# mmigas/LiverRenderer

Hardware: AMD Instinct MI355X
Metric: Msamples/s (higher is better)
Workload: dtype f32; 1 GPU; C3 Liver-SingleMesh volpath 1920x1080 512 spp max_depth 12 (homogeneous medium, isotropic phase, envmap); width=1920, height=1080, spp=512, parallelism=1 GPU

## Files before the change

### include/liverrt.h

```cpp
#ifndef LIVERRT_H
#define LIVERRT_H

#include <stdint.h>
#include <stddef.h>

#ifdef __cplusplus
extern "C" {
#endif

#define LRT_API __attribute__((visibility("default")))

typedef enum {
    LRT_OK = 0,
    LRT_ERR_INVALID = 1,
    LRT_ERR_IO = 2,
    LRT_ERR_DEVICE = 3,
    LRT_ERR_UNSUPPORTED = 4
} lrt_status;

enum { LRT_INTEGRATOR_PATH = 0, LRT_INTEGRATOR_VOLPATH = 1, LRT_INTEGRATOR_PRBVOLPATH = 2,
       LRT_INTEGRATOR_VOLPATHMIS = 5,
       LRT_INTEGRATOR_BIOVOLPATH = 3,
       LRT_INTEGRATOR_BIOVOLPATH06 = 4    };
enum { LRT_MEDIUM_HOMOGENEOUS = 0, LRT_MEDIUM_LIVER = 1, LRT_MEDIUM_PARENCHYMA = 2, LRT_MEDIUM_GLISSON = 3,
// ... 71 lines not shown
    int32_t type;
    float   radiance[3];
    int32_t shape;
    float   scale;
    float   to_world[16];
    int32_t width, height;
    const float *data;
} lrt_emitter_desc;

enum { LRT_SAMPLER_INDEPENDENT = 0, LRT_SAMPLER_LD = 1 };

typedef struct {
    float   to_world[16];
    float   fov_x;
    float   near_clip, far_clip;
    int32_t medium;
    float   principal_point_offset_x, principal_point_offset_y;
    int32_t pad;
} lrt_sensor_desc;

typedef struct {
    int32_t width, height;
    int32_t crop_offset_x, crop_offset_y, crop_width, crop_height;
    int32_t has_alpha;
    int32_t rfilter;
    float   rfilter_param;
} lrt_film_desc;

typedef struct {
    int32_t type;
    int32_t max_depth;
    int32_t rr_depth;
    int32_t hide_emitters;
} lrt_integrator_desc;

typedef struct {
    uint32_t n_vertices, n_faces, n_shapes, n_bsdfs, n_textures, n_media, n_emitters;
    const float    *positions;
    const float    *normals;
    const float    *texcoords;
    const uint32_t *faces;
    const uint32_t *face_shape;
    const lrt_shape_desc   *shapes;
    const lrt_bsdf_desc    *bsdfs;
    const lrt_texture_desc *textures;
    const lrt_medium_desc  *media;
    const lrt_emitter_desc *emitters;
    lrt_sensor_desc     sensor;
    lrt_film_desc       film;
    lrt_integrator_desc integrator;
    uint32_t sample_count;
    uint32_t sampler_seed;
    uint32_t sampler_type;
    uint32_t samples_per_pass;
    uint32_t use_spectral_mis;
    uint32_t pad;
} lrt_scene_desc;

typedef struct {
    int32_t  integrator;
    int32_t  max_depth;
    int32_t  rr_depth;
    int32_t  hide_emitters;
    uint32_t spp;
    uint32_t seed;
    uint32_t tile_rank, tile_count;
    int32_t  device;
    int32_t  output_on_device;
    int32_t  grad_medium;
    int32_t  pad;
} lrt_render_opts;

typedef struct {
    uint64_t n_samples;
    uint64_t n_iter;
    uint64_t n_shadow;
    uint64_t n_launches;
    uint64_t n_records;
    double   kernel_ms;
    double   total_ms;
    uint64_t lds_resident;
    uint64_t record_bytes;
    uint64_t n_closed_guard;
} lrt_render_stats;

typedef struct {
    float d_sigma_t[3];
    float d_albedo[3];
    float d_g;
} lrt_param_grads;

typedef struct lrt_scene lrt_scene;

LRT_API const char *lrt_last_error(void);
LRT_API int         lrt_version(void);

LRT_API lrt_status lrt_scene_load_xml(const char *path, const char *const *defines,
                                      int n_defines, lrt_scene **out);
LRT_API lrt_status lrt_scene_load_xml_string(const char *xml, const char *base_dir,
                                             const char *const *defines, int n_defines,
                                             lrt_scene **out);
LRT_API lrt_status lrt_scene_from_desc(const lrt_scene_desc *desc, lrt_scene **out);
LRT_API const lrt_scene_desc *lrt_scene_desc_get(const lrt_scene *scene);
LRT_API void       lrt_scene_free(lrt_scene *scene);

LRT_API lrt_status lrt_render(lrt_scene *scene, const lrt_render_opts *opts,
                              float *film_raw, float *image);
LRT_API lrt_status lrt_render_stats_get(const lrt_scene *scene, lrt_render_stats *out);
LRT_API lrt_status lrt_film_develop(lrt_scene *scene, const float *film_raw, float *image,
                                    int on_device);

LRT_API lrt_status lrt_render_samples(lrt_scene *scene, const lrt_render_opts *opts,
                                      uint64_t lane_begin, uint32_t n, float *out);

LRT_API lrt_status lrt_render_backward(lrt_scene *scene, const lrt_render_opts *opts,
                                       const float *grad_image, lrt_param_grads *out);

LRT_API lrt_status lrt_render_backward_grid(lrt_scene *scene, const lrt_render_opts *opts, const float *grad_image,
                                            lrt_param_grads *out, float *d_grid);

LRT_API lrt_status lrt_render_multi(lrt_scene *scene, const lrt_render_opts *opts, int n_devices, const int *device_ids,
                                    float *film_raw, float *image);
LRT_API lrt_status lrt_render_backward_multi(lrt_scene *scene, const lrt_render_opts *opts, int n_devices, const int *device_ids,
                                             const float *grad_image, lrt_param_grads *out);

LRT_API lrt_status lrt_math_eval(int fn, const float *x, const float *y, uint32_t n, float *out, float *out2, int device);

#define LRT_PROBE_FLOATS 20
LRT_API lrt_status lrt_emitter_probe(lrt_scene *scene, const float *ref_p, const float *sample, uint32_t n, float *out, int device);

LRT_API lrt_status lrt_envmap_probe(lrt_scene *scene, const float *dir, uint32_t n, float *out, int device);

#define LRT_BSDF_PROBE_FLOATS 30
LRT_API lrt_status lrt_bsdf_probe(lrt_scene *scene, const float *o, const float *d, const float *sample, const float *wo_query,
                                  uint32_t n, float *out, int device);

typedef struct { const float *ox, *oy, *oz, *dx, *dy, *dz, *tmax; } lrt_rays_soa;
typedef struct { float *t, *u, *v; uint32_t *prim; } lrt_hits_soa;
LRT_API lrt_status lrt_trace(lrt_scene *scene, const lrt_rays_soa *rays,
                             const lrt_hits_soa *hits, uint32_t n, int any_hit);

LRT_API lrt_status lrt_param_set(lrt_scene *scene, const char *key, const float *v, int n);
LRT_API lrt_status lrt_param_get(const lrt_scene *scene, const char *key, float *v, int n);

LRT_API lrt_status lrt_image_read(const char *path, int *width, int *height, int *channels, float **data);
LRT_API void       lrt_image_free(float *data);
LRT_API lrt_status lrt_image_write_exr(const char *path, int width, int height, int channels, const float *data);
LRT_API lrt_status lrt_image_write_png(const char *path, int width, int height, int channels, const float *data);

#define LRT_AOV_MAX_INTEGRATORS 4
#define LRT_AOV_MAX_AOVS        16
#define LRT_AOV_NAME_LEN        64
enum { LRT_AOV_ALBEDO = 0,
       LRT_AOV_DEPTH = 1,
       LRT_AOV_POSITION = 2,
       LRT_AOV_UV = 3,
       LRT_AOV_GEO_NORMAL = 4,
       LRT_AOV_SH_NORMAL = 5,
       LRT_AOV_DP_DU = 6,
       LRT_AOV_DP_DV = 7,
       LRT_AOV_PRIM_INDEX = 8,
       LRT_AOV_SHAPE_INDEX = 9    };

typedef struct {
    int32_t n_integrators;
    lrt_integrator_desc integrators[LRT_AOV_MAX_INTEGRATORS];
// ... 74 lines not shown
```

### liverrenderer_amd/_lib.py

```python
import ctypes as C
import os

_HERE = os.path.dirname(os.path.abspath(__file__))
LIB_PATH = os.environ.get("LRT_LIBRARY") or os.path.join(_HERE, "libliverrt.so")

OK, INVALID, UNSUPPORTED = 0, 1, 4
INTEGRATOR = {"path": 0, "volpath": 1, "prbvolpath": 2, "biovolpath": 3, "biovolpath06": 4, "volpathmis": 5}
MEDIUM = {"homogeneous": 0, "liver": 1, "parenchyma": 2, "glissonCapsule": 3, "heterogeneous": 4}
EMITTER = {"area": 0, "envmap": 1, "constant": 2}
PROBE_FLOATS = 20
BSDF_PROBE_FLOATS = 30


class ShapeDesc(C.Structure):
    _fields_ = [("kind", C.c_int32), ("first_face", C.c_uint32), ("n_faces", C.c_uint32), ("bsdf", C.c_int32),
                ("emitter", C.c_int32), ("interior_medium", C.c_int32), ("exterior_medium", C.c_int32),
                ("has_normals", C.c_int32), ("has_texcoords", C.c_int32), ("flip_normals", C.c_int32),
                ("to_world", C.c_float * 16)]


class TextureDesc(C.Structure):
    _fields_ = [("type", C.c_int32), ("color0", C.c_float * 3), ("color1", C.c_float * 3), ("to_uv", C.c_float * 9),
                ("width", C.c_int32), ("height", C.c_int32), ("channels", C.c_int32), ("data", C.POINTER(C.c_float))]


class BsdfDesc(C.Structure):
    _fields_ = [("type", C.c_int32), ("reflectance", C.c_int32), ("eta", C.c_float), ("nested", C.c_int32),
                ("texture", C.c_int32), ("scale", C.c_float),
                ("alpha_u", C.c_float), ("alpha_v", C.c_float), ("distribution", C.c_int32), ("sample_visible", C.c_int32),
                ("specular_reflectance", C.c_int32), ("specular_transmittance", C.c_int32)]


class MediumDesc(C.Structure):
    _fields_ = [("sigma_t", C.c_float * 3), ("albedo", C.c_float * 3), ("scale", C.c_float),
                ("has_spectral_extinction", C.c_int32), ("sample_emitters", C.c_int32), ("phase", C.c_int32),
                ("g", C.c_float), ("id", C.c_char * 64),
                ("type", C.c_int32), ("layer_limit", C.c_float * 4), ("sigma_collagen", (C.c_float * 3) * 4),
                ("sigma_elastin", (C.c_float * 3) * 4), ("sigma_blood", C.c_float * 3), ("sigma_bile", C.c_float * 3),
                ("sigma_lipid_water", C.c_float * 3), ("sigma_hepatocity", C.c_float),
                ("grid_res", C.c_int32 * 3), ("grid_to_local", C.c_float * 12), ("grid_bbox_min", C.c_float * 3),
                ("grid_bbox_max", C.c_float * 3), ("grid_max", C.c_float), ("grid_data", C.POINTER(C.c_float))]


class EmitterDesc(C.Structure):
    _fields_ = [("type", C.c_int32), ("radiance", C.c_float * 3), ("shape", C.c_int32), ("scale", C.c_float),
                ("to_world", C.c_float * 16), ("width", C.c_int32), ("height", C.c_int32), ("data", C.POINTER(C.c_float))]


class SensorDesc(C.Structure):
    _fields_ = [("to_world", C.c_float * 16), ("fov_x", C.c_float), ("near_clip", C.c_float), ("far_clip", C.c_float),
                ("medium", C.c_int32), ("principal_point_offset_x", C.c_float), ("principal_point_offset_y", C.c_float), ("pad", C.c_int32)]


class FilmDesc(C.Structure):
    _fields_ = [("width", C.c_int32), ("height", C.c_int32), ("crop_offset_x", C.c_int32), ("crop_offset_y", C.c_int32),
                ("crop_width", C.c_int32), ("crop_height", C.c_int32), ("has_alpha", C.c_int32), ("rfilter", C.c_int32),
                ("rfilter_param", C.c_float)]


class IntegratorDesc(C.Structure):
    _fields_ = [("type", C.c_int32), ("max_depth", C.c_int32), ("rr_depth", C.c_int32), ("hide_emitters", C.c_int32)]


class SceneDesc(C.Structure):
    _fields_ = [("n_vertices", C.c_uint32), ("n_faces", C.c_uint32), ("n_shapes", C.c_uint32), ("n_bsdfs", C.c_uint32),
                ("n_textures", C.c_uint32), ("n_media", C.c_uint32), ("n_emitters", C.c_uint32),
                ("positions", C.POINTER(C.c_float)), ("normals", C.POINTER(C.c_float)), ("texcoords", C.POINTER(C.c_float)),
                ("faces", C.POINTER(C.c_uint32)), ("face_shape", C.POINTER(C.c_uint32)),
                ("shapes", C.POINTER(ShapeDesc)), ("bsdfs", C.POINTER(BsdfDesc)), ("textures", C.POINTER(TextureDesc)),
                ("media", C.POINTER(MediumDesc)), ("emitters", C.POINTER(EmitterDesc)),
                ("sensor", SensorDesc), ("film", FilmDesc), ("integrator", IntegratorDesc),
                ("sample_count", C.c_uint32), ("sampler_seed", C.c_uint32),
                ("sampler_type", C.c_uint32), ("samples_per_pass", C.c_uint32), ("use_spectral_mis", C.c_uint32), ("pad", C.c_uint32)]


AOV_MAX_INTEGRATORS, AOV_MAX_AOVS, AOV_NAME_LEN = 4, 16, 64
AOV_TYPES = {"albedo": 0, "depth": 1, "position": 2, "uv": 3, "geo_normal": 4, "sh_normal": 5, "dp_du": 6, "dp_dv": 7,
             "prim_index": 8, "shape_index": 9}


class AovDesc(C.Structure):
    _fields_ = [("n_integrators", C.c_int32), ("integrators", IntegratorDesc * AOV_MAX_INTEGRATORS),
                ("integrator_names", (C.c_char * AOV_NAME_LEN) * AOV_MAX_INTEGRATORS),
                ("n_aovs", C.c_int32), ("aov_types", C.c_int32 * AOV_MAX_AOVS), ("aov_names", (C.c_char * AOV_NAME_LEN) * AOV_MAX_AOVS),
                ("n_aov_channels", C.c_int32), ("n_channels", C.c_int32)]


class MomentDesc(C.Structure):
    _fields_ = [("integrator", IntegratorDesc), ("name", C.c_char * AOV_NAME_LEN), ("n_channels", C.c_int32), ("n_raw_channels", C.c_int32)]


class RenderOpts(C.Structure):
    _fields_ = [("integrator", C.c_int32), ("max_depth", C.c_int32), ("rr_depth", C.c_int32), ("hide_emitters", C.c_int32),
                ("spp", C.c_uint32), ("seed", C.c_uint32), ("tile_rank", C.c_uint32), ("tile_count", C.c_uint32),
                ("device", C.c_int32), ("output_on_device", C.c_int32), ("grad_medium", C.c_int32), ("pad", C.c_int32)]


class RenderStats(C.Structure):
    _fields_ = [("n_samples", C.c_uint64), ("n_iter", C.c_uint64), ("n_shadow", C.c_uint64), ("n_launches", C.c_uint64),
                ("n_records", C.c_uint64), ("kernel_ms", C.c_double), ("total_ms", C.c_double), ("lds_resident", C.c_uint64),
                ("record_bytes", C.c_uint64), ("n_closed_guard", C.c_uint64)]


class ParamGrads(C.Structure):
    _fields_ = [("d_sigma_t", C.c_float * 3), ("d_albedo", C.c_float * 3), ("d_g", C.c_float)]


class DenoiseParams(C.Structure):
    _fields_ = [("iterations", C.c_int32), ("sigma_color", C.c_float), ("sigma_normal", C.c_float), ("sigma_albedo", C.c_float), ("eps_a", C.c_float)]


class RaysSoA(C.Structure):
    _fields_ = [(n, C.POINTER(C.c_float)) for n in ("ox", "oy", "oz", "dx", "dy", "dz", "tmax")]


class HitsSoA(C.Structure):
    _fields_ = [("t", C.POINTER(C.c_float)), ("u", C.POINTER(C.c_float)), ("v", C.POINTER(C.c_float)), ("prim", C.POINTER(C.c_uint32))]


def make_opts(integrator=None, max_depth=None, rr_depth=None, hide_emitters=None, spp=0, seed=0,
              tile_rank=0, tile_count=1, device=0, output_on_device=False, grad_medium=0):
    o = RenderOpts()
    o.integrator = -1 if integrator is None else (INTEGRATOR[integrator] if isinstance(integrator, str) else int(integrator))
    o.max_depth = -2 if max_depth is None else int(max_depth)
    o.rr_depth = -1 if rr_depth is None else int(rr_depth)
    o.hide_emitters = -1 if hide_emitters is None else int(bool(hide_emitters))
    o.spp, o.seed, o.tile_rank, o.tile_count = int(spp), int(seed) & 0xffffffff, int(tile_rank), int(tile_count)
    o.device, o.output_on_device = int(device), int(bool(output_on_device))
    o.grad_medium = int(grad_medium)
    return o


_lib = None


def _pytorch_context_first():
    import importlib.util
    import sys
    if os.environ.get("LRT_NO_TORCH_INIT"):
        return "skipped"
    if "torch" not in sys.modules and importlib.util.find_spec("torch") is None:
        return "no torch"
    import torch
    if not torch.cuda.is_available():
        return "no device"
    if not torch.cuda.is_initialized():
        lr = os.environ.get("LOCAL_RANK")
        if lr is not None and lr.isdigit() and torch.cuda.device_count() > 0:
            torch.cuda.set_device(int(lr) % torch.cuda.device_count())
        torch.zeros(1, device="cuda")
    if not torch.cuda.is_initialized():
        raise RuntimeError("PyTorch is importable but its HIP context could not be created before libliverrt.so was loaded; "
                           "set LRT_NO_TORCH_INIT=1 if this process does not use PyTorch")
    return "initialised"


def lib():
    global _lib
    if _lib is not None:
        return _lib
    _pytorch_context_first()
    if not os.path.exists(LIB_PATH):
        raise RuntimeError(f"{LIB_PATH} is missing: build it with `python -c 'import __graft_entry__ as g; g.build()'` "
                           "(the hip_ad_rgb back-end has no CPU fallback)")
    L = C.CDLL(LIB_PATH)
    P = C.POINTER
    L.lrt_last_error.restype = C.c_char_p
    L.lrt_version.restype = C.c_int
    L.lrt_scene_load_xml.argtypes = [C.c_char_p, P(C.c_char_p), C.c_int, P(C.c_void_p)]
    L.lrt_scene_load_xml_string.argtypes = [C.c_char_p, C.c_char_p, P(C.c_char_p), C.c_int, P(C.c_void_p)]
    L.lrt_scene_from_desc.argtypes = [P(SceneDesc), P(C.c_void_p)]
    L.lrt_scene_desc_get.argtypes = [C.c_void_p]
    L.lrt_scene_desc_get.restype = P(SceneDesc)
    L.lrt_scene_free.argtypes = [C.c_void_p]
    L.lrt_scene_free.restype = None
    L.lrt_render.argtypes = [C.c_void_p, P(RenderOpts), C.c_void_p, C.c_void_p]
    L.lrt_render_multi.argtypes = [C.c_void_p, P(RenderOpts), C.c_int, P(C.c_int), C.c_void_p, C.c_void_p]
    L.lrt_render_backward_multi.argtypes = [C.c_void_p, P(RenderOpts), C.c_int, P(C.c_int), C.c_void_p, P(ParamGrads)]
    L.lrt_math_eval.argtypes = [C.c_int, P(C.c_float), P(C.c_float), C.c_uint32, P(C.c_float), P(C.c_float), C.c_int]
    L.lrt_render_stats_get.argtypes = [C.c_void_p, P(RenderStats)]
    L.lrt_film_develop.argtypes = [C.c_void_p, C.c_void_p, C.c_void_p, C.c_int]
    L.lrt_render_samples.argtypes = [C.c_void_p, P(RenderOpts), C.c_uint64, C.c_uint32, C.c_void_p]
    L.lrt_render_backward.argtypes = [C.c_void_p, P(RenderOpts), C.c_void_p, P(ParamGrads)]
    L.lrt_render_backward_grid.argtypes = [C.c_void_p, P(RenderOpts), C.c_void_p, P(ParamGrads), C.c_void_p]
# ... 63 lines not shown
```

### liverrenderer_amd/csrc/capi.cpp

```cpp
#include "host_scene.h"
#include "device_scene.h"
#include "image_io.h"
#include <algorithm>
#include <cmath>
#include <cstring>
#include <cstdio>
#include <fstream>
#include <sstream>
#include <stdexcept>

using namespace lrt;

static thread_local std::string g_error;
static lrt_status fail(lrt_status st, const std::string &msg) { g_error = msg; return st; }

#define LRT_TRY try {
#define LRT_CATCH } catch (const std::exception &e) { \
        std::string m = e.what(); \
        lrt_status st = LRT_ERR_INVALID; \
        if (m.find("hip") != std::string::npos || m.find("HIP") != std::string::npos) st = LRT_ERR_DEVICE; \
        if (m.find("cannot open") != std::string::npos || m.find("file not found") != std::string::npos) st = LRT_ERR_IO; \
        if (m.find("unsupported") != std::string::npos || m.find("not supported") != std::string::npos) st = LRT_ERR_UNSUPPORTED; \
        return fail(st, m); \
    } catch (...) { return fail(LRT_ERR_INVALID, "unknown error"); }

extern "C" {

const char *lrt_last_error(void) { return g_error.c_str(); }
int lrt_version(void) { return 114; }

static std::vector<std::pair<std::string, std::string>> parse_defines(const char *const *defines, int n) {
    std::vector<std::pair<std::string, std::string>> r;
    for (int i = 0; i < n; ++i) {
        std::string s = defines[i]; size_t eq = s.find('=');
        if (eq == std::string::npos) throw std::runtime_error("define \"" + s + "\" must have the form key=value");
        r.emplace_back(s.substr(0, eq), s.substr(eq + 1));
    }
    return r;
}

lrt_status lrt_scene_load_xml_string(const char *xml, const char *base_dir, const char *const *defines, int n_defines, lrt_scene **out) {
    if (!xml || !out) return fail(LRT_ERR_INVALID, "lrt_scene_load_xml_string: null argument");
    *out = nullptr;
    LRT_TRY
        std::unique_ptr<lrt_scene> s(new lrt_scene());
        load_scene_xml(xml, base_dir ? base_dir : "", parse_defines(defines, n_defines), s->st);
        *out = s.release();
        return LRT_OK;
    LRT_CATCH
}

lrt_status lrt_scene_load_xml(const char *path, const char *const *defines, int n_defines, lrt_scene **out) {
    if (!path || !out) return fail(LRT_ERR_INVALID, "lrt_scene_load_xml: null argument");
    *out = nullptr;
    std::ifstream f(path, std::ios::binary);
    if (!f) return fail(LRT_ERR_IO, std::string("cannot open \"") + path + "\"");
    std::stringstream ss; ss << f.rdbuf();
    std::string p = path, dir; size_t sl = p.rfind('/'); dir = sl == std::string::npos ? "." : p.substr(0, sl);
    return lrt_scene_load_xml_string(ss.str().c_str(), dir.c_str(), defines, n_defines, out);
}

static void validate_desc(const lrt_scene_desc &d) {
    auto bad = [](const std::string &m) { throw std::runtime_error("lrt_scene_from_desc: " + m); };
    if ((d.n_vertices && (!d.positions || !d.normals || !d.texcoords)) || (d.n_faces && (!d.faces || !d.face_shape))) bad("null geometry array");
    if ((d.n_shapes && !d.shapes) || (d.n_bsdfs && !d.bsdfs) || (d.n_textures && !d.textures) || (d.n_media && !d.media) || (d.n_emitters && !d.emitters)) bad("null object array");
    for (uint32_t f = 0; f < 3 * d.n_faces; ++f) if (d.faces[f] >= d.n_vertices) bad("face references an invalid vertex");
    for (uint32_t f = 0; f < d.n_faces; ++f) if (d.face_shape[f] >= d.n_shapes) bad("face references an invalid shape");
    for (uint32_t i = 0; i < d.n_textures; ++i) {
        const lrt_texture_desc &T = d.textures[i];
        if (T.type < LRT_TEX_RGB || T.type > LRT_TEX_BITMAP) bad("invalid texture type");
        if (T.type == LRT_TEX_BITMAP && (!T.data || T.width < 1 || T.height < 1 || (T.channels != 1 && T.channels != 3))) bad("bitmap texture without texels or with invalid dimensions");
    }
    for (uint32_t i = 0; i < d.n_bsdfs; ++i) {
        const lrt_bsdf_desc &B = d.bsdfs[i];
        if (B.type < LRT_BSDF_DIFFUSE || B.type > LRT_BSDF_ROUGHDIELECTRIC) bad("invalid bsdf type");
        if (B.type == LRT_BSDF_DIFFUSE) {
            if (B.reflectance < 0 || (uint32_t) B.reflectance >= d.n_textures) bad("diffuse bsdf references an invalid texture");
            if (d.textures[B.reflectance].type == LRT_TEX_BITMAP) throw std::runtime_error("unsupported: a bitmap texture as diffuse reflectance (bitmaps are supported as bump-map heights only)");
        }
        if (B.type == LRT_BSDF_BUMPMAP) {
            if (B.nested < 0 || (uint32_t) B.nested >= d.n_bsdfs || d.bsdfs[B.nested].type == LRT_BSDF_BUMPMAP) bad("bumpmap references an invalid nested bsdf");
            if (B.texture < 0 || (uint32_t) B.texture >= d.n_textures) bad("bumpmap references an invalid texture");
        }
        if (B.type == LRT_BSDF_DIELECTRIC && !(B.eta > 0.f)) bad("dielectric with a non-positive relative index of refraction");
        if (B.type == LRT_BSDF_ROUGHDIELECTRIC) {
            if (!(B.eta > 0.f) || B.eta == 1.f) bad("roughdielectric: the interior and exterior indices of refraction must be positive and differ");
            if (!(B.alpha_u >= 0.f) || !(B.alpha_v >= 0.f) || !std::isfinite(B.alpha_u) || !std::isfinite(B.alpha_v)) bad("roughdielectric with an invalid roughness");
            if (B.distribution != 0 && B.distribution != 1) bad("roughdielectric with an invalid distribution (0: beckmann, 1: ggx)");
            for (int32_t t : { B.specular_reflectance, B.specular_transmittance }) {
                if (t < -1 || t >= (int32_t) d.n_textures) bad("roughdielectric references an invalid texture");
                if (t >= 0 && d.textures[t].type == LRT_TEX_BITMAP) throw std::runtime_error("unsupported: a bitmap texture as roughdielectric specular_reflectance / specular_transmittance");
            }
        }
    }
    for (uint32_t i = 0; i < d.n_media; ++i) {
        const lrt_medium_desc &M = d.media[i];
        if (M.type < LRT_MEDIUM_HOMOGENEOUS || M.type > LRT_MEDIUM_HETEROGENEOUS) bad("invalid medium type");
        if (M.type == LRT_MEDIUM_HETEROGENEOUS && (!M.grid_data || M.grid_res[0] < 1 || M.grid_res[1] < 1 || M.grid_res[2] < 1)) bad("heterogeneous medium without grid data");
        if (M.phase != LRT_PHASE_ISOTROPIC && M.phase != LRT_PHASE_HG) bad("invalid phase function");
        if (M.phase == LRT_PHASE_HG && !(M.g > -1.f && M.g < 1.f)) bad("The asymmetry parameter must lie in the interval (-1, 1)!");
    }
    for (uint32_t i = 0; i < d.n_shapes; ++i) {
        const lrt_shape_desc &s = d.shapes[i];
        if (s.bsdf < 0 || (uint32_t) s.bsdf >= d.n_bsdfs) bad("shape references an invalid bsdf");
        if (s.emitter < -1 || s.emitter >= (int) d.n_emitters || s.interior_medium < -1 || s.interior_medium >= (int) d.n_media || s.exterior_medium < -1 || s.exterior_medium >= (int) d.n_media)
            bad("shape references an invalid emitter/medium");
        if ((uint64_t) s.first_face + s.n_faces > d.n_faces) bad("shape face range exceeds the face array");
        if (s.kind < LRT_SHAPE_MESH || s.kind > LRT_SHAPE_SPHERE) bad("invalid shape kind");
        if (s.kind == LRT_SHAPE_SPHERE && s.n_faces != 0) bad("a sphere shape has no faces");
        if (s.emitter >= 0 && (d.emitters[s.emitter].type != LRT_EMITTER_AREA || d.emitters[s.emitter].shape != (int) i)) bad("shape and area emitter do not reference each other");
    }
    uint32_t n_env = 0;
// ... 488 lines not shown
```

### liverrenderer_amd/csrc/device.hip

```cpp
#include "host_scene.h"
#include "device_scene.h"
#include "kernels_prb.h"
#include "kernels_vae.h"
#include "kernels_aov.h"
#include "kernels_denoise.h"
#include "kernels_moment.h"
#include <functional>
#include "scene_prep.h"
#include <cmath>
#include <array>
#include <cstring>
#include <algorithm>
#include <stdexcept>
#include <string>
#include <cstdio>
#include <cstdlib>
#include <thread>
#include <chrono>
#include <exception>
#include <dlfcn.h>
#include <rccl/rccl.h>

namespace lrt {

#define HIP_CHECK(expr) do { hipError_t e_ = (expr); if (e_ != hipSuccess) throw std::runtime_error(std::string(#expr) + ": " + hipGetErrorString(e_)); } while (0)

template <typename T> static T *dev_upload(const T *src, size_t n, hipStream_t st) {
    T *p = nullptr; size_t bytes = std::max<size_t>(n, 1) * sizeof(T);
    HIP_CHECK(hipMalloc((void **) &p, bytes));
    if (n) HIP_CHECK(hipMemcpyAsync(p, src, n * sizeof(T), hipMemcpyHostToDevice, st));
    return p;
}

struct DevTmp {
    float *p = nullptr;
    DevTmp() = default;
    explicit DevTmp(size_t floats) { alloc(floats); }
    DevTmp(const DevTmp &) = delete; DevTmp &operator=(const DevTmp &) = delete;
    void alloc(size_t floats) { HIP_CHECK(hipMalloc((void **) &p, std::max<size_t>(floats, 1) * sizeof(float))); }
    void upload(const float *src, size_t floats, hipStream_t st) { alloc(floats); HIP_CHECK(hipMemcpyAsync(p, src, floats * sizeof(float), hipMemcpyHostToDevice, st)); }
    ~DevTmp() { if (p) (void) hipFree(p); }
};

static void select_device(int device) {
    int count = 0;
    if (hipGetDeviceCount(&count) != hipSuccess || count == 0) throw std::runtime_error("no HIP device available: the hip_ad_rgb back-end has no CPU fallback");
    if (device < 0 || device >= count) throw std::runtime_error("invalid HIP device ordinal " + std::to_string(device));
    HIP_CHECK(hipSetDevice(device));
}

static lrt_render_opts default_opts() { return lrt_render_opts{ -1, -2, -1, -1, 0, 0, 0, 1, 0, 0, 0, 0 }; }

static void add_stats(lrt_render_stats &total, const lrt_render_stats &s) {
    total.n_samples += s.n_samples; total.n_iter += s.n_iter; total.n_shadow += s.n_shadow; total.n_launches += s.n_launches;
    total.n_records += s.n_records; total.kernel_ms += s.kernel_ms; total.total_ms += s.total_ms;
    total.record_bytes = s.record_bytes; total.n_closed_guard += s.n_closed_guard;
}

#define LRT_LAUNCH_SLOTS 64
#define LRT_WIDE_BLOCK 768

struct DeviceScene {
    int device = 0;
    hipStream_t stream = nullptr;
    DScene sc{};
    DScene *d_sc = nullptr;
    DLaunch *d_launch = nullptr, *h_launch = nullptr; uint32_t launch_next = 0;
    std::vector<void *> allocs;
    uint32_t capacity = 0;
    DPathStreams q[2]{};
    float4 *dl[2] = { nullptr, nullptr }; size_t dl_records[2] = { 0, 0 }; float4 *L_buf = nullptr; size_t l_buf_lanes = 0;
    double *d_grads = nullptr; float *wfilm = nullptr; size_t wfilm_floats = 0; float *grad_image = nullptr; size_t grad_floats = 0;
    DCounters *counters = nullptr;
    DCounters *h_counters = nullptr;
    float *film = nullptr; size_t film_floats = 0;
    float *image = nullptr; size_t image_floats = 0;
    unsigned long long *pass_state[2] = { nullptr, nullptr }; size_t pass_state_lanes[2] = { 0, 0 };
    const unsigned long long *cur_pass_in = nullptr; unsigned long long *cur_pass_out = nullptr;
    uint32_t *pixel_slot = nullptr;
    uint32_t *pixel_list = nullptr; uint32_t pixel_list_rank = 0xffffffffu, pixel_list_count = 0, n_owned_pixels = 0;
    uint32_t *halo_list = nullptr; uint32_t halo_rank = 0xffffffffu, halo_count = 0, halo_width = 0, n_halo_pixels = 0;
    std::vector<hipEvent_t> ev_pool;
    std::vector<DMedium> h_media; DMedium *d_media = nullptr;
    std::vector<DBioMedium> h_bio; DBioMedium *d_bio = nullptr;
    std::vector<DHetMedium> h_het; DHetMedium *d_het = nullptr; std::vector<float *> het_data; bool has_het = false, has_non_bio = false, need_mis = false; uint32_t ws_layouts = 0;
    bool ext = false;
    bool has_area_emitter = false;
    float *dgrid = nullptr; size_t dgrid_floats = 0;
    bool prb_null = false;
    DLdsInfo lds{}; bool use_lds = false; int n_cus = 256; int bvh_leaf = 4;
    DAovSpec *d_aov_spec = nullptr; uint32_t *d_first_face = nullptr;
    float *aov_film = nullptr; size_t aov_film_floats = 0; float *aov_image = nullptr; size_t aov_image_floats = 0; float *aov_inner = nullptr; size_t aov_inner_floats = 0;

    template <typename T> T *track(T *p) { allocs.push_back((void *) p); return p; }
    void release(void *p) {
        if (!p) return;
        for (auto it = allocs.begin(); it != allocs.end(); ++it) if (*it == p) { allocs.erase(it); break; }
        (void) hipFree(p);
    }
    template <typename T> T *grow(T *&p, size_t &have, size_t want) {
        if (have >= want) return p;
        HIP_CHECK(hipStreamSynchronize(stream));
        release(p); p = nullptr; have = 0;
        HIP_CHECK(hipMalloc((void **) &p, std::max<size_t>(want, 1) * sizeof(T))); track(p);
        have = want;
        return p;
    }
    ~DeviceScene() {
        for (void *p : allocs) (void) hipFree(p);
        for (auto e : ev_pool) (void) hipEventDestroy(e);
        if (h_counters) (void) hipHostFree(h_counters);
        if (h_launch) (void) hipHostFree(h_launch);
        if (stream) (void) hipStreamDestroy(stream);
    }
};

void device_scene_destroy(DeviceScene *d) { delete d; }

static_assert(PREP_F_DELTA == F_DELTA && PREP_F_SMOOTH == F_SMOOTH && PREP_F_NULL == F_NULL, "scene_prep.h restates the BSDF leaf flags of dshade.h");

__global__ void k_bio_prepare(DBioMedium *bio, uint32_t n) {
    const uint32_t i = blockIdx.x * blockDim.x + threadIdx.x;
    if (i < n) bio[i].log10_hep = m_log2(bio[i].hepatocity + 1.f) / m_log2(10.f);
}

__global__ void k_medium_prepare(DMedium *media, uint32_t n) {
    const uint32_t i = blockIdx.x * blockDim.x + threadIdx.x;
    if (i >= n) return;
    DMedium &M = media[i];
    const V3 st(M.sigma_t[0], M.sigma_t[1], M.sigma_t[2]), ss = st * V3(M.albedo[0], M.albedo[1], M.albedo[2]);
    const V3 ws = ss / mean3(st / st), wp = ss / st;
    M.w_spec[0] = ws.x; M.w_spec[1] = ws.y; M.w_spec[2] = ws.z; M.w_plain[0] = wp.x; M.w_plain[1] = wp.y; M.w_plain[2] = wp.z;
}

static void upload_media(DeviceScene *D, const lrt_scene_desc &d) {
    prepare_media(d, D->sc.env.bsphere_r, D->h_media, D->h_bio, D->h_het);
    for (size_t i = 0; i < D->h_het.size(); ++i) D->h_het[i].data = D->het_data[i];
    HIP_CHECK(hipMemcpyAsync(D->d_bio, D->h_bio.data(), D->h_bio.size() * sizeof(DBioMedium), hipMemcpyHostToDevice, D->stream));
    k_bio_prepare<<<1, 64, 0, D->stream>>>(D->d_bio, (uint32_t) std::min<size_t>(D->h_bio.size(), 64));
// ... 59 lines not shown
typedef void (*AovFn)(ScenePtr, LaunchPtr, AovSpecPtr);
static AovFn aov_kernel(bool lds, bool ld, bool ext) {
    static const AovFn t[2][2][2] = { { { k_aov<false, false, false>, k_aov<false, false, true> }, { k_aov<false, true, false>, k_aov<false, true, true> } },
                                      { { k_aov<true, false, false>, k_aov<true, false, true> }, { k_aov<true, true, false>, k_aov<true, true, true> } } };
    return t[lds][ld][ext];
}
typedef decltype(&k_trace<false, false>) TraceFn;
typedef decltype(&k_trace_lds<false, false>) TraceLdsFn;
static TraceFn trace_kernel(bool any_hit, bool ext) {
    static const TraceFn t[2][2] = { { k_trace<false, false>, k_trace<false, true> }, { k_trace<true, false>, k_trace<true, true> } };
    return t[any_hit][ext];
}
static TraceLdsFn trace_lds_kernel(bool any_hit, bool ext) {
    static const TraceLdsFn t[2][2] = { { k_trace_lds<false, false>, k_trace_lds<false, true> }, { k_trace_lds<true, false>, k_trace_lds<true, true> } };
    return t[any_hit][ext];
}
static RenderFn moment_splat_kernel(bool wide, bool alpha) {
    static const RenderFn t[2][2] = { { k_moment_splat<false, false>, k_moment_splat<false, true> }, { k_moment_splat<true, false>, k_moment_splat<true, true> } };
    return t[wide][alpha];
}

DeviceScene *device_scene_create(const lrt_scene_desc &d, int device) {
    select_device(device);
    std::unique_ptr<DeviceScene> D(new DeviceScene());
    D->device = device;
    HIP_CHECK(hipStreamCreateWithFlags(&D->stream, hipStreamNonBlocking));
    hipStream_t st = D->stream;
    PrepOptions opt = PrepOptions::from_env();
    hipDeviceProp_t prop; HIP_CHECK(hipGetDeviceProperties(&prop, device)); opt.n_cus = prop.multiProcessorCount > 0 ? prop.multiProcessorCount : 256;
    int optin = 0; if (hipDeviceGetAttribute(&optin, hipDeviceAttributeSharedMemPerBlockOptin, device) != hipSuccess || optin <= 0) optin = (int) prop.sharedMemPerBlock;
    (void) hipGetLastError();
    opt.lds_limit = std::min<size_t>((size_t) std::max(optin, 0), 160 * 1024) - 512;
    PreparedScene P; DScene &sc = P.sc;
    prepare_geometry(d, opt, P);
    D->n_cus = opt.n_cus; D->bvh_leaf = P.bvh_leaf; D->ext = P.ext;
    auto up = [&](const auto &v) { return D->track(dev_upload(v.data(), v.size(), st)); };
    sc.spheres = P.spheres.empty() ? nullptr : up(P.spheres);
    sc.nodes = (const float4 *) up(P.bvh.nodes);
    sc.tris = (const float4 *) up(P.bvh.tris);
    if (P.use_lds) {
        D->lds = P.lds; D->lds.blob = (const uint4 *) up(P.lds_blob);
        const size_t lds_limit = opt.lds_limit;
        auto raise_lds = [&](const void *k) { if (k) HIP_CHECK(hipFuncSetAttribute(k, hipFuncAttributeMaxDynamicSharedMemorySize, (int) lds_limit)); };
        const KernelTable &K = kernels();
        for (const RenderRow &r : K.render) if (r.lds && (!r.ext || D->ext)) raise_lds((const void *) r.fn);
        for (const auto &adjoint : K.prb) for (const auto &ld : adjoint[1]) for (RenderFn fn : ld) raise_lds((const void *) fn);
        for (RenderFn fn : K.prb_grid[1]) raise_lds((const void *) fn);
        for (int i = 0; i < 2; ++i) for (int ext = 0; ext <= (D->ext ? 1 : 0); ++ext) {
            raise_lds((const void *) aov_kernel(true, i, ext)); raise_lds((const void *) trace_lds_kernel(i, ext));
        }
        D->use_lds = true;
    }
    if (sc.grid.enabled) {
        const size_t n_cells = (size_t) sc.grid.n[0] * sc.grid.n[1] * sc.grid.n[2];
        uint16_t *buf = nullptr; HIP_CHECK(hipMalloc((void **) &buf, n_cells * sizeof(uint16_t))); D->track(buf);
        k_build_dist_grid<<<(uint32_t) ((n_cells + LRT_BLOCK - 1) / LRT_BLOCK), LRT_BLOCK, 0, st>>>(sc.tris, d.n_faces ? (uint32_t) (P.bvh.tris.size() / 12) : 0u, sc.grid, buf, P.grid_abs_margin,
                                                                                             sc.spheres, sc.n_spheres);
        HIP_CHECK(hipGetLastError());
        sc.grid.d = buf;
    }
    prepare_shading(d, opt, P);
    D->has_area_emitter = P.has_area_emitter; D->has_het = P.has_het; D->has_non_bio = P.has_non_bio; D->prb_null = P.prb_null;
    sc.positions = D->track(dev_upload(d.positions, 3 * (size_t) d.n_vertices, st));
    sc.vattr = (const float4 *) up(P.vattr);
    sc.faces = D->track(dev_upload(d.faces, 3 * (size_t) d.n_faces, st));
    sc.face_shape = D->track(dev_upload(d.face_shape, d.n_faces, st));
    sc.shapes = up(P.shapes);
    sc.textures = up(P.textures);
    sc.tex_data = up(P.tex_data);
    sc.bsdfs = up(P.bsdfs);
    HIP_CHECK(hipMalloc((void **) &D->d_media, std::max<uint32_t>(d.n_media, 1) * sizeof(DMedium))); D->track(D->d_media);
    HIP_CHECK(hipMalloc((void **) &D->d_bio, std::max<uint32_t>(d.n_media, 1) * sizeof(DBioMedium))); D->track(D->d_bio);
    HIP_CHECK(hipMalloc((void **) &D->d_het, std::max<uint32_t>(d.n_media, 1) * sizeof(DHetMedium))); D->track(D->d_het);
    D->het_data.assign(std::max<uint32_t>(d.n_media, 1), nullptr);
    for (uint32_t i = 0; i < d.n_media; ++i) {
        const lrt_medium_desc &M = d.media[i];
        if (M.type == LRT_MEDIUM_HETEROGENEOUS) D->het_data[i] = D->track(dev_upload(M.grid_data, (size_t) M.grid_res[0] * M.grid_res[1] * M.grid_res[2], st));
    }
    D->sc = sc;
    upload_media(D.get(), d); sc.media = D->d_media; sc.bio = D->d_bio; sc.het = D->d_het;
    sc.emitters = up(P.emitters);
    sc.mesh_emitters = up(P.mesh_emitters);
    sc.mesh_emitter_tab = up(P.mesh_emitter_tab);
    sc.env_data = (const float4 *) up(P.env_data);
    sc.env_hier = up(P.env_hier);
    HIP_CHECK(hipMalloc((void **) &D->d_sc, sizeof(DScene))); D->track(D->d_sc);
    D->sc = sc;
    HIP_CHECK(hipMemcpyAsync(D->d_sc, &D->sc, sizeof(DScene), hipMemcpyHostToDevice, st));
    HIP_CHECK(hipMalloc((void **) &D->d_launch, LRT_LAUNCH_SLOTS * sizeof(DLaunch))); D->track(D->d_launch);
    HIP_CHECK(hipHostMalloc((void **) &D->h_launch, LRT_LAUNCH_SLOTS * sizeof(DLaunch)));
    HIP_CHECK(hipMalloc((void **) &D->counters, sizeof(DCounters))); D->track(D->counters);
    HIP_CHECK(hipHostMalloc((void **) &D->h_counters, sizeof(DCounters)));
    HIP_CHECK(hipStreamSynchronize(st));
    return D.release();
}

void device_scene_update_params(DeviceScene *D, const lrt_scene_desc &d, bool grids) {
    HIP_CHECK(hipSetDevice(D->device));
    if (grids) for (uint32_t i = 0; i < d.n_media; ++i) {
        const lrt_medium_desc &M = d.media[i];
        if (M.type == LRT_MEDIUM_HETEROGENEOUS && D->het_data[i])
            HIP_CHECK(hipMemcpyAsync(D->het_data[i], M.grid_data, (size_t) M.grid_res[0] * M.grid_res[1] * M.grid_res[2] * sizeof(float), hipMemcpyHostToDevice, D->stream));
    }
    upload_media(D, d);
    HIP_CHECK(hipStreamSynchronize(D->stream));
}

static void ensure_workspace(DeviceScene *D, uint32_t capacity) {
    const uint32_t layouts = workspace_layouts(D->has_het, D->need_mis);
    if (D->capacity >= capacity && D->ws_layouts == layouts) return;
    HIP_CHECK(hipStreamSynchronize(D->stream));
    D->capacity = 0;
    auto get = [](const DPathStreams *q, const RecordStream &r) { void *p; memcpy(&p, (const char *) q + r.member, sizeof p); return p; };
    auto set = [](DPathStreams *q, const RecordStream &r, void *p) { memcpy((char *) q + r.member, &p, sizeof p); };
    for (DPathStreams *q : { &D->q[0], &D->q[1] })
        for (const RecordStream &r : kRecordStreams) if (r.member != kNoMember) { D->release(get(q, r)); set(q, r, nullptr); }
    for (DPathStreams *q : { &D->q[0], &D->q[1] })
        for (size_t k = 0; k < std::size(kRecordStreams); ++k) if (const uint32_t bytes = workspace_stream_bytes(k, layouts)) {
            void *p = nullptr; HIP_CHECK(hipMalloc(&p, (size_t) capacity * bytes)); D->track(p); set(q, kRecordStreams[k], p);
        }
    D->capacity = capacity; D->ws_layouts = layouts;
}

static hipEvent_t get_event(DeviceScene *D, size_t i) {
    while (D->ev_pool.size() <= i) { hipEvent_t e; HIP_CHECK(hipEventCreate(&e)); D->ev_pool.push_back(e); }
    return D->ev_pool[i];
}

static void ensure_pixel_list(DeviceScene *D, const ResolvedOpts &O) {
    const DFilm &F = D->sc.film;
    if (O.tile_count == 1) { D->n_owned_pixels = (uint32_t) F.width * F.height; return; }
    if (D->pixel_list && D->pixel_list_rank == O.tile_rank && D->pixel_list_count == O.tile_count) return;
    const TilePixels T = tile_pixel_list(F, O.tile_rank, O.tile_count);
    D->release(D->pixel_list); D->release(D->pixel_slot); D->pixel_list = nullptr; D->pixel_slot = nullptr;
    D->pixel_list = D->track(dev_upload(T.list.data(), T.list.size(), D->stream));
    D->pixel_slot = D->track(dev_upload(T.slot.data(), T.slot.size(), D->stream));
    D->pixel_list_rank = O.tile_rank; D->pixel_list_count = O.tile_count; D->n_owned_pixels = (uint32_t) T.list.size();
}

static void ensure_halo_list(DeviceScene *D, const ResolvedOpts &O, uint32_t halo) {
    const DFilm &F = D->sc.film;
    if (D->halo_list && D->halo_rank == O.tile_rank && D->halo_count == O.tile_count && D->halo_width == halo) return;
    const std::vector<uint32_t> px = halo_pixel_list(F, O.tile_rank, O.tile_count, halo);
    D->release(D->halo_list); D->halo_list = nullptr;
    D->halo_list = D->track(dev_upload(px.data(), px.size(), D->stream));
    D->halo_rank = O.tile_rank; D->halo_count = O.tile_count; D->halo_width = halo; D->n_halo_pixels = (uint32_t) px.size();
}

static void ensure_prb_workspace(DeviceScene *D, uint32_t records, uint64_t l_buf_lanes) {
    for (int k = 0; k < 2; ++k) D->grow(D->dl[k], D->dl_records[k], records);
    D->grow(D->L_buf, D->l_buf_lanes, l_buf_lanes);
    if (!D->d_grads) { HIP_CHECK(hipMalloc((void **) &D->d_grads, 7 * sizeof(double))); D->track(D->d_grads); }
}

static DRenderParams make_params(const lrt_scene_desc &d, const ResolvedOpts &O, uint64_t n_lanes) {
    DRenderParams rp{};
    rp.integrator = O.integrator; rp.max_depth = O.max_depth; rp.rr_depth = O.rr_depth; rp.hide_emitters = O.hide_emitters;
    rp.spp = O.spp; rp.log2_spp = ((O.spp & (O.spp - 1)) == 0) ? (uint32_t) __builtin_ctz(O.spp) : 0xffffffffu;
    rp.profile = getenv("LRT_DEBUG_LAUNCH") ? 1u : 0u;
#ifdef LRT_EXPERIMENT
    if (getenv("LRT_EXP")) rp.profile |= (uint32_t) atoi(getenv("LRT_EXP"));
    if (getenv("LRT_PRB_DEBUG_LANE")) rp.pad1 = (uint32_t) atoi(getenv("LRT_PRB_DEBUG_LANE")) + 1u;
#endif
    rp.seed_value = d.sampler_seed + O.seed; rp.base_seed = d.sampler_seed; rp.seed = O.seed;
    rp.ld_count = d.sampler_type == LRT_SAMPLER_LD ? O.spp_total : 0u; rp.pass_index = O.pass; rp.spp_total = O.spp_total; rp.tile_rank = O.tile_rank; rp.tile_count = O.tile_count; rp.n_lanes = n_lanes;
    return rp;
// ... 49 lines not shown
    HIP_CHECK(hipMemcpyAsync(&D->d_launch[slot], &D->h_launch[slot], sizeof(DLaunch), hipMemcpyHostToDevice, D->stream));
    return (LaunchPtr) &D->d_launch[slot];
}

template <bool ADJOINT>
static void launch_prb(DeviceScene *D, const DRenderParams &rp, const PoolGeometry &g, const uint32_t *pixel_list, uint64_t lane_begin,
                       float4 *L_buf, const float *grad_image, double *grads, float *film, float *sample_out, float *dgrid = nullptr) {
    hipStream_t st = D->stream;
    HIP_CHECK(hipMemsetAsync(&D->counters->next_lane, 0, sizeof(unsigned long long), st));
    DLaunch a{}; a.rp = rp; a.li = D->lds; a.q0 = D->q[0]; a.q1 = D->q[1]; a.dl0 = D->dl[0]; a.dl1 = D->dl[1]; a.P = g.P; a.cnt = D->counters;
    a.pixel_list = pixel_list; a.lane_begin = lane_begin; a.n = rp.n_lanes; a.L_buf = L_buf; a.grad_image = grad_image; a.wfilm = D->wfilm; a.grads = grads;
    a.film = film; a.sample_out = sample_out; a.sample_base = lane_begin; a.dgrid = dgrid;
    const LaunchPtr lp = push_launch(D, a);
    const bool ld = rp.ld_count != 0;
    const RenderFn fn = (ADJOINT && dgrid) ? kernels().prb_grid[D->use_lds][ld] : kernels().prb[ADJOINT][D->use_lds][ld][D->prb_null];
    if (!fn) throw std::runtime_error("developer build: volpath only");
    fn<<<g.n_wg, D->use_lds ? 1024 : LRT_BLOCK, g.smem, st>>>((ScenePtr) D->d_sc, lp);
    HIP_CHECK(hipGetLastError());
}

static void check_integrator_media(DeviceScene *D, int integrator) {
    if ((integrator == LRT_INTEGRATOR_BIOVOLPATH || integrator == LRT_INTEGRATOR_BIOVOLPATH06) && D->has_non_bio)
        throw std::runtime_error("NotImplementedError: sample_interaction (the bio integrators need liver / parenchyma / glissonCapsule media)");
    if (integrator == LRT_INTEGRATOR_PRBVOLPATH && D->ext)
        throw std::runtime_error("unsupported: prbvolpath on a scene with sphere shapes, point emitters, area emitters on meshes or a roughdielectric BSDF (its adjoint is built for triangles, rectangle / infinite emitters and the diffuse / dielectric / null BSDFs)");
    if (integrator == LRT_INTEGRATOR_VOLPATHMIS) D->need_mis = true;
}

static const RenderRow &select_render_kernel(int integrator, bool has_het, bool spectral_mis, bool lds, bool ld, bool ext, bool compact, bool closed) {
    int mode;
    switch (integrator) {
        case LRT_INTEGRATOR_PATH: case LRT_INTEGRATOR_BIOVOLPATH: case LRT_INTEGRATOR_BIOVOLPATH06: mode = integrator; break;
        case LRT_INTEGRATOR_VOLPATHMIS: mode = spectral_mis ? LRT_INTEGRATOR_VOLPATHMIS : LRT_INTEGRATOR_VOLPATHMIS_PLAIN; break;
        default: mode = closed ? LRT_INTEGRATOR_VOLPATH_CLOSED : (has_het ? LRT_INTEGRATOR_VOLPATH_HET : LRT_INTEGRATOR_VOLPATH);
    }
    for (const RenderRow &r : kernels().render) if (r.mode == mode && r.lds == lds && r.ld == ld && r.compact == compact && r.ext == ext) return r;
    throw std::runtime_error("no render-kernel instance for mode " + std::to_string(mode) + (lds ? ", LDS BVH" : ", global BVH") + (ld ? ", ld sampler" : ", independent sampler") +
                             (compact ? ", compact records" : ", wide records") + (ext ? ", EXT" : ""));
}

static void run_wavefront(DeviceScene *D, const lrt_scene_desc &d, const ResolvedOpts &O, uint64_t lane_begin, uint64_t n_lanes,
                          const uint32_t *pixel_list, float *film, float *sample_out, lrt_render_stats &stats) {
    hipStream_t st = D->stream;
    DRenderParams rp = make_params(d, O, n_lanes);
    rp.pixel_slot = pixel_list ? D->pixel_slot : nullptr;
    rp.pass_in = D->cur_pass_in; rp.pass_out = D->cur_pass_out;
    const bool prb = O.integrator == LRT_INTEGRATOR_PRBVOLPATH;
    check_integrator_media(D, O.integrator);
    PoolGeometry g = pool_geometry(D, n_lanes);
    const uint32_t records = (uint32_t) std::min<uint64_t>((uint64_t) g.n_wg * 2u * g.P, 0xffffffffull);
    ensure_workspace(D, records);
    if (prb) ensure_prb_workspace(D, records, 0);
    HIP_CHECK(hipMemsetAsync(D->counters, 0, sizeof(DCounters), st));
    LaunchLog log;
    hipEvent_t e_begin = get_event(D, log.ev++), e_end = get_event(D, log.ev++);
    HIP_CHECK(hipEventRecord(e_begin, st));
    const bool count_iter = !(O.integrator == LRT_INTEGRATOR_PATH && O.max_depth == 0);
    hipEvent_t a = get_event(D, log.ev++), b = get_event(D, log.ev++);
    HIP_CHECK(hipEventRecord(a, st));
    if (prb) { stats.record_bytes = 0; launch_prb<false>(D, rp, g, pixel_list, lane_begin, nullptr, nullptr, nullptr, film, sample_out); }
    else {
        DLaunch a{}; a.rp = rp; a.li = D->lds; a.q0 = D->q[0]; a.q1 = D->q[1]; a.P = g.P; a.cnt = D->counters; a.pixel_list = pixel_list;
        a.lane_begin = lane_begin; a.n = n_lanes; a.film = film; a.sample_out = sample_out; a.sample_base = lane_begin;
        const bool compact = D->use_lds && !D->has_area_emitter && !D->ext && !getenv("LRT_WIDE_RECORDS") && O.integrator != LRT_INTEGRATOR_VOLPATHMIS && !(O.integrator == LRT_INTEGRATOR_VOLPATH && D->has_het);
        const bool closed = compact && O.integrator == LRT_INTEGRATOR_VOLPATH && closed_records(d, D->sc.cam.medium) && !getenv("LRT_NO_CLOSED_RECORDS");
#ifdef LRT_DEV_VOLPATH_ONLY
        if (D->ext) throw std::runtime_error("developer build: no EXT instances (spheres / point emitters)");
        if (!(D->use_lds && (O.integrator == LRT_DEV_INTEGRATOR || (LRT_DEV_INTEGRATOR == LRT_INTEGRATOR_VOLPATH_HET && D->has_het)) && (rp.ld_count != 0) == LRT_DEV_LD)) throw std::runtime_error("developer build: one integrator / sampler / LDS BVH only");
#endif
        const RenderRow &row = select_render_kernel(O.integrator, D->has_het, d.use_spectral_mis != 0, D->use_lds, rp.ld_count != 0, D->ext, compact, closed);
        stats.record_bytes = row.record_bytes;
        const LaunchPtr lp = push_launch(D, a);
        row.fn<<<g.n_wg, row.block, g.smem, st>>>((ScenePtr) D->d_sc, lp);
        HIP_CHECK(hipGetLastError());
    }
    HIP_CHECK(hipEventRecord(b, st));
    log.launches.emplace_back(a, b); log.sizes.push_back(0);
    HIP_CHECK(hipMemcpyAsync(D->h_counters, D->counters, sizeof(DCounters), hipMemcpyDeviceToHost, st));
    HIP_CHECK(hipStreamSynchronize(st));
    log.n_iter = count_iter ? D->h_counters->n_iter : 0;
    log.n_records = D->h_counters->n_records;
    finish_stats(D, log, e_begin, e_end, n_lanes, stats);
    stats.n_closed_guard = D->h_counters->n_closed_guard;
    if (stats.n_closed_guard)
        throw std::runtime_error("64-byte path records: " + std::to_string(stats.n_closed_guard) + " trips broke the premise of the layout (radiance before a path's last trip, "
                                 "or an emitter hit that needs its MIS weight); the scene test in closed_records() is wrong for this scene: LRT_NO_CLOSED_RECORDS=1 renders it with 80-byte records");
}

static void render_passes(DeviceScene *D, const lrt_scene_desc &d, const lrt_render_opts *opts, float *film_raw, float *image, lrt_render_stats &stats,
                          const std::function<void(const ResolvedOpts &)> &after_pass, bool moment = false);

void device_render(DeviceScene *D, const lrt_scene_desc &d, const lrt_render_opts *opts, float *film_raw, float *image, lrt_render_stats &stats) {
    render_passes(D, d, opts, film_raw, image, stats, nullptr);
}

static void develop_and_download(DeviceScene *D, const float *film, float *film_raw, float *image, size_t film_floats, size_t image_floats, bool on_device, bool moment = false) {
    const DFilm &F = D->sc.film; const size_t np = (size_t) F.width * F.height;
    if (image) {
        float *img = on_device ? image : D->grow(D->image, D->image_floats, image_floats);
        if (!moment) k_develop<<<(uint32_t) ((np + 255) / 256), 256, 0, D->stream>>>(F, film, img, (uint32_t) np);
        else if (F.has_alpha) k_moment_develop<true><<<(uint32_t) ((np + 255) / 256), 256, 0, D->stream>>>(film, img, (uint32_t) np);
        else k_moment_develop<false><<<(uint32_t) ((np + 255) / 256), 256, 0, D->stream>>>(film, img, (uint32_t) np);
        if (!on_device) HIP_CHECK(hipMemcpyAsync(image, img, image_floats * 4, hipMemcpyDeviceToHost, D->stream));
    }
    if (film_raw && !on_device) HIP_CHECK(hipMemcpyAsync(film_raw, film, film_floats * 4, hipMemcpyDeviceToHost, D->stream));
    HIP_CHECK(hipStreamSynchronize(D->stream));
    HIP_CHECK(hipGetLastError());
}

static void render_passes(DeviceScene *D, const lrt_scene_desc &d, const lrt_render_opts *opts, float *film_raw, float *image, lrt_render_stats &stats,
                          const std::function<void(const ResolvedOpts &)> &after_pass, bool moment) {
    HIP_CHECK(hipSetDevice(D->device));
    ResolvedOpts O = resolve(d, opts);
    const DFilm &F = D->sc.film;
    bool on_device = opts && opts->output_on_device;
    const size_t film_channels = moment ? (F.has_alpha ? 11 : 10) : (size_t) F.channels, image_channels = moment ? film_channels - 1 : (F.has_alpha ? 4 : 3);
    size_t np = (size_t) F.width * F.height, film_floats = np * film_channels, image_floats = np * image_channels;
    ensure_pixel_list(D, O);
    const uint64_t n_lanes = (uint64_t) D->n_owned_pixels * O.spp;
    float *film = (on_device && film_raw) ? film_raw : D->grow(D->film, D->film_floats, film_floats);
    HIP_CHECK(hipMemsetAsync(film, 0, film_floats * 4, D->stream));
    const uint32_t *pixel_list = O.tile_count > 1 ? D->pixel_list : nullptr;
    const bool carry = O.n_passes > 1 && d.sampler_type != LRT_SAMPLER_LD;
    if (carry) for (int k = 0; k < 2; ++k) D->grow(D->pass_state[k], D->pass_state_lanes[k], n_lanes);
    const bool lane_splat = moment || (F.rfilter != LRT_RFILTER_BOX && (O.n_passes > 1 || !getenv("LRT_NO_LANE_SPLAT")));
    lrt_render_stats total{};
    for (uint32_t pass = 0; pass < O.n_passes; ++pass) {
        O.pass = pass;
        D->cur_pass_in = carry ? D->pass_state[pass & 1] : nullptr;
        D->cur_pass_out = (carry && pass + 1 < O.n_passes) ? D->pass_state[(pass & 1) ^ 1] : nullptr;
        if (!lane_splat) {
            lrt_render_stats st1{};
            run_wavefront(D, d, O, 0, n_lanes, pixel_list, film, nullptr, st1);
            add_stats(total, st1);
            if (after_pass) after_pass(O);
            continue;
        }
        const uint64_t chunk = std::min<uint64_t>(std::max<uint64_t>(n_lanes, 1), 1ull << 28);
        ensure_prb_workspace(D, 0, chunk);
        for (uint64_t base = 0; base < n_lanes; base += chunk) {
            const uint64_t n = std::min<uint64_t>(chunk, n_lanes - base);
            lrt_render_stats st1{};
            run_wavefront(D, d, O, base, n, pixel_list, nullptr, reinterpret_cast<float *>(D->L_buf), st1);
            DRenderParams rp = make_params(d, O, n); rp.pass_in = D->cur_pass_in;
            DLaunch a{}; a.rp = rp; a.L_buf = D->L_buf; a.pixel_list = pixel_list; a.lane_begin = base; a.n = n; a.film = film;
            const uint32_t grid = (uint32_t) ((n + LRT_BLOCK - 1) / LRT_BLOCK);
            const LaunchPtr lp = push_launch(D, a);
            if (!moment) k_splat_lanes<false><<<grid, LRT_BLOCK, 0, D->stream>>>((ScenePtr) D->d_sc, lp);
            else moment_splat_kernel(F.rfilter != LRT_RFILTER_BOX, F.has_alpha != 0)<<<grid, LRT_BLOCK, 0, D->stream>>>((ScenePtr) D->d_sc, lp);
            HIP_CHECK(hipGetLastError());
            add_stats(total, st1);
        }
        if (after_pass) after_pass(O);
    }
    D->cur_pass_in = nullptr; D->cur_pass_out = nullptr;
    total.lds_resident = D->use_lds ? 1 : 0;
    stats = total;
    develop_and_download(D, film, film_raw, image, film_floats, image_floats, on_device, moment);
}

void device_render_moment(DeviceScene *D, const lrt_scene_desc &d, const lrt_render_opts *opts, float *film_raw, float *image, lrt_render_stats &stats) {
    render_passes(D, d, opts, film_raw, image, stats, nullptr, true);
}

void device_render_moment_samples(DeviceScene *D, const lrt_scene_desc &d, const lrt_render_opts *opts, uint64_t lane_begin, uint32_t n, float *out, lrt_render_stats &stats) {
    HIP_CHECK(hipSetDevice(D->device));
// ... 295 lines not shown
        for (const char *name : { env ? env : "/opt/rocm/lib/librccl.so", "librccl.so.1", "librccl.so" }) { h = dlopen(name, RTLD_NOW | RTLD_LOCAL); if (h) break; }
        if (!h) throw std::runtime_error(std::string("hip: cannot load librccl.so (") + (dlerror() ? dlerror() : "?") + "); lrt_render_multi on distinct devices needs RCCL");
        auto sym = [&](const char *n) { void *p = dlsym(h, n); if (!p) throw std::runtime_error(std::string("hip: librccl.so lacks ") + n); return p; };
        CommInitAll = (decltype(CommInitAll)) sym("ncclCommInitAll"); AllReduce = (decltype(AllReduce)) sym("ncclAllReduce");
        GroupStart = (decltype(GroupStart)) sym("ncclGroupStart"); GroupEnd = (decltype(GroupEnd)) sym("ncclGroupEnd");
        CommDestroy = (decltype(CommDestroy)) sym("ncclCommDestroy"); GetErrorString = (decltype(GetErrorString)) sym("ncclGetErrorString");
    }
    void check(ncclResult_t r, const char *what) { if (r != ncclSuccess) throw std::runtime_error(std::string("hip: rccl ") + what + ": " + (GetErrorString ? GetErrorString(r) : "error")); }
};
static Rccl g_rccl;

struct MultiContext {
    std::vector<int> devices; std::vector<ncclComm_t> comms;
    ~MultiContext() { for (auto c : comms) if (c && g_rccl.CommDestroy) (void) g_rccl.CommDestroy(c); }
};
void multi_context_destroy(MultiContext *m) { delete m; }

__global__ void k_film_add(float *__restrict__ dst, const float *__restrict__ src, size_t n) {
    const size_t i = (size_t) blockIdx.x * blockDim.x + threadIdx.x;
    if (i < n) dst[i] += src[i];
}

template <typename T>
static void reduce_across(std::vector<DeviceScene *> &devs, MultiContext *&ctx, std::vector<T *> &buf, size_t count) {
    const int N = (int) devs.size();
    bool distinct = true;
    for (int i = 0; i < N; ++i) for (int j = 0; j < i; ++j) if (devs[i]->device == devs[j]->device) distinct = false;
    for (auto *D : devs) { HIP_CHECK(hipSetDevice(D->device)); HIP_CHECK(hipStreamSynchronize(D->stream)); }
    if (distinct) {
        g_rccl.load();
        std::vector<int> ids; for (auto *D : devs) ids.push_back(D->device);
        if (!ctx || ctx->devices != ids) {
            delete ctx; ctx = new MultiContext(); ctx->devices = ids; ctx->comms.assign(N, nullptr);
            g_rccl.check(g_rccl.CommInitAll(ctx->comms.data(), N, ids.data()), "ncclCommInitAll");
        }
        g_rccl.check(g_rccl.GroupStart(), "ncclGroupStart");
        for (int i = 0; i < N; ++i) {
            HIP_CHECK(hipSetDevice(devs[i]->device));
            g_rccl.check(g_rccl.AllReduce(buf[i], buf[i], count, sizeof(T) == 8 ? ncclDouble : ncclFloat, ncclSum, ctx->comms[i], devs[i]->stream), "ncclAllReduce");
        }
        g_rccl.check(g_rccl.GroupEnd(), "ncclGroupEnd");
        for (auto *D : devs) { HIP_CHECK(hipSetDevice(D->device)); HIP_CHECK(hipStreamSynchronize(D->stream)); }
    } else {
        for (int i = 1; i < N; ++i) if (devs[i]->device != devs[0]->device) throw std::runtime_error("lrt_render_multi: a device list is either all distinct or one device repeated");
        static_assert(sizeof(T) == 4 || sizeof(T) == 8, "float or double");
        HIP_CHECK(hipSetDevice(devs[0]->device));
        for (int i = 1; i < N; ++i) {
            if (sizeof(T) == 4) k_film_add<<<(uint32_t) ((count + 255) / 256), 256, 0, devs[0]->stream>>>((float *) buf[0], (const float *) buf[i], count);
            else { std::vector<double> a(count), b(count); HIP_CHECK(hipMemcpy(a.data(), buf[0], count * 8, hipMemcpyDeviceToHost)); HIP_CHECK(hipMemcpy(b.data(), buf[i], count * 8, hipMemcpyDeviceToHost));
                   for (size_t k = 0; k < count; ++k) a[k] += b[k]; HIP_CHECK(hipMemcpy(buf[0], a.data(), count * 8, hipMemcpyHostToDevice)); }
        }
        HIP_CHECK(hipGetLastError()); HIP_CHECK(hipStreamSynchronize(devs[0]->stream));
    }
}

template <typename F> static void on_every_device(size_t n, F fn) {
    std::vector<std::exception_ptr> err(n);
    std::vector<std::thread> th;
    for (size_t i = 0; i < n; ++i) th.emplace_back([&, i]() { try { fn(i); } catch (...) { err[i] = std::current_exception(); } });
    for (auto &t : th) t.join();
    for (auto &e : err) if (e) std::rethrow_exception(e);
}

void device_render_multi(std::vector<DeviceScene *> &devs, MultiContext *&ctx, const lrt_scene_desc &d, const lrt_render_opts *opts, float *film_raw, float *image, lrt_render_stats &stats) {
    const int N = (int) devs.size();
    const DFilm &F = devs[0]->sc.film;
    const size_t np = (size_t) F.width * F.height, film_floats = np * F.channels, image_floats = np * (F.has_alpha ? 4 : 3);
    const bool on_device = opts && opts->output_on_device;
    std::vector<float *> films(N); std::vector<lrt_render_stats> st(N);
    const auto t0 = std::chrono::steady_clock::now();
    on_every_device(N, [&](size_t i) {
        HIP_CHECK(hipSetDevice(devs[i]->device));
        films[i] = (i == 0 && on_device && film_raw) ? film_raw : devs[i]->grow(devs[i]->film, devs[i]->film_floats, film_floats);
        lrt_render_opts o = opts ? *opts : default_opts();
        o.tile_rank = (uint32_t) i; o.tile_count = (uint32_t) N; o.device = devs[i]->device; o.output_on_device = 1;
        device_render(devs[i], d, &o, films[i], nullptr, st[i]);
    });
    if (N > 1 || getenv("LRT_MULTI_ALWAYS_REDUCE")) reduce_across(devs, ctx, films, film_floats);
    DeviceScene *D0 = devs[0];
    HIP_CHECK(hipSetDevice(D0->device));
    develop_and_download(D0, films[0], film_raw, image, film_floats, image_floats, on_device);
    lrt_render_stats total{};
    for (auto &x : st) { total.n_samples += x.n_samples; total.n_iter += x.n_iter; total.n_shadow += x.n_shadow; total.n_launches += x.n_launches; total.n_records += x.n_records;
                         total.kernel_ms = std::max(total.kernel_ms, x.kernel_ms); total.lds_resident = x.lds_resident; total.record_bytes = x.record_bytes; total.n_closed_guard += x.n_closed_guard; }
    total.total_ms = std::chrono::duration<double, std::milli>(std::chrono::steady_clock::now() - t0).count();
    stats = total;
}

void device_render_backward_multi(std::vector<DeviceScene *> &devs, MultiContext *&ctx, const lrt_scene_desc &d, const lrt_render_opts *opts, const float *grad_image, lrt_param_grads *out, lrt_render_stats &stats) {
    const int N = (int) devs.size();
    if (opts && opts->output_on_device) throw std::runtime_error("lrt_render_backward_multi: grad_image is a host buffer (every device takes its own copy)");
    std::vector<lrt_param_grads> g(N); std::vector<lrt_render_stats> st(N);
    on_every_device(N, [&](size_t i) {
        lrt_render_opts o = opts ? *opts : default_opts();
        o.tile_rank = (uint32_t) i; o.tile_count = (uint32_t) N; o.device = devs[i]->device; o.output_on_device = 0;
        device_render_backward(devs[i], d, &o, grad_image, &g[i], st[i]);
    });
    std::vector<double *> bufs; for (auto *D : devs) bufs.push_back(D->d_grads);
    if (N > 1) reduce_across(devs, ctx, bufs, 7);
    double h[7]; HIP_CHECK(hipSetDevice(devs[0]->device)); HIP_CHECK(hipMemcpy(h, devs[0]->d_grads, sizeof(h), hipMemcpyDeviceToHost));
    for (int k = 0; k < 3; ++k) { out->d_sigma_t[k] = (float) h[k]; out->d_albedo[k] = (float) h[3 + k]; }
    out->d_g = (float) h[6];
    lrt_render_stats total{};
    for (auto &x : st) { total.n_samples += x.n_samples; total.n_iter += x.n_iter; total.n_shadow += x.n_shadow; total.n_launches += x.n_launches; total.n_records += x.n_records;
                         total.kernel_ms = std::max(total.kernel_ms, x.kernel_ms); total.total_ms = std::max(total.total_ms, x.total_ms); total.lds_resident = x.lds_resident; }
    stats = total;
}

void device_emitter_probe(DeviceScene *D, const float *ref_p, const float *sample, uint32_t n, float *out) {
    HIP_CHECK(hipSetDevice(D->device));
    if (!n) return;
    hipStream_t st = D->stream;
    DevTmp dr, ds, dout((size_t) n * LRT_PROBE_FLOATS);
    dr.upload(ref_p, (size_t) n * 3, st); ds.upload(sample, (size_t) n * 2, st);
    k_emitter_probe<<<(n + LRT_BLOCK - 1) / LRT_BLOCK, LRT_BLOCK, 0, st>>>((ScenePtr) D->d_sc, dr.p, ds.p, n, dout.p);
    HIP_CHECK(hipGetLastError());
    HIP_CHECK(hipMemcpyAsync(out, dout.p, (size_t) n * LRT_PROBE_FLOATS * 4, hipMemcpyDeviceToHost, st));
    HIP_CHECK(hipStreamSynchronize(st));
}

void device_envmap_probe(DeviceScene *D, const float *dir, uint32_t n, float *out) {
    HIP_CHECK(hipSetDevice(D->device));
    if (D->sc.env.emitter < 0) throw std::runtime_error("lrt_envmap_probe: the scene has no environment emitter");
    if (!n) return;
    hipStream_t st = D->stream;
    DevTmp dd, dout((size_t) n * 4);
    dd.upload(dir, (size_t) n * 3, st);
    k_envmap_probe<<<(n + LRT_BLOCK - 1) / LRT_BLOCK, LRT_BLOCK, 0, st>>>((ScenePtr) D->d_sc, dd.p, n, dout.p);
    HIP_CHECK(hipGetLastError());
    HIP_CHECK(hipMemcpyAsync(out, dout.p, (size_t) n * 4 * 4, hipMemcpyDeviceToHost, st));
    HIP_CHECK(hipStreamSynchronize(st));
}

void device_bsdf_probe(DeviceScene *D, const float *o, const float *d, const float *sample, const float *wo_query, uint32_t n, float *out) {
    HIP_CHECK(hipSetDevice(D->device));
    if (!n) return;
    hipStream_t st = D->stream;
    DevTmp in[4], dout((size_t) n * LRT_BSDF_PROBE_FLOATS);
    const float *src[4] = { o, d, sample, wo_query };
    for (int k = 0; k < 4; ++k) in[k].upload(src[k], (size_t) n * 3, st);
    k_bsdf_probe<<<(n + LRT_BLOCK - 1) / LRT_BLOCK, LRT_BLOCK, 0, st>>>((ScenePtr) D->d_sc, in[0].p, in[1].p, in[2].p, in[3].p, n, dout.p);
    HIP_CHECK(hipGetLastError());
    HIP_CHECK(hipMemcpyAsync(out, dout.p, (size_t) n * LRT_BSDF_PROBE_FLOATS * 4, hipMemcpyDeviceToHost, st));
    HIP_CHECK(hipStreamSynchronize(st));
}

__global__ void k_math_eval(int fn, const float *__restrict__ x, const float *__restrict__ y, uint32_t n, float *__restrict__ out, float *__restrict__ out2) {
    const uint32_t i = blockIdx.x * blockDim.x + threadIdx.x;
    if (i >= n) return;
    float a = 0.f, b = 0.f;
    switch (fn) {
        case 0: a = m_log(x[i]); break;
        case 1: a = m_exp(x[i]); break;
        case 2: m_sincos(x[i], &a, &b); break;
        case 3: a = m_atan2(y[i], x[i]); break;
        case 4: a = m_acos(x[i]); break;
        case 5: a = m_log2(x[i]); break;
        case 6: a = x[i] / y[i]; break;
        case 7: a = __builtin_sqrtf(x[i]); break;
        case 8: a = rcp(x[i]); break;
        case 9: a = m_erf(x[i]); break;
        case 10: a = m_erfinv(x[i]); break;
        default: break;
    }
    out[i] = a; out2[i] = b;
}
void device_math_eval(int fn, const float *x, const float *y, uint32_t n, float *out, float *out2, int device) {
// ... 85 lines not shown
```

### liverrenderer_amd/csrc/device_types.h

```cpp
#pragma once
#include <stdint.h>
#include <hip/hip_vector_types.h>

namespace lrt {

struct DShape {
    int32_t bsdf, emitter, interior_medium, exterior_medium;
    int32_t has_normals, has_texcoords, flip_normals, kind;
};

#define LRT_MICRO_GGX 1
#define LRT_MICRO_VISIBLE 2
struct DBsdf {
    int32_t type;
    union { int32_t reflectance; int32_t specular_reflectance; };
    union { int32_t nested; int32_t micro; };
    union { int32_t texture; int32_t specular_transmittance; };
    float eta;
    union { float scale; float alpha_u; };
    int32_t flags;
    union { int32_t pad; float alpha_v; };
};
static_assert(sizeof(DBsdf) == 32, "DBsdf stride");

// ... 36 lines not shown
    int32_t type, shape; float radiance[3]; float scale;
    float n[3]; float inv_area;
    float to_world[12];
};

struct DSphere {
    float center[3], radius;
    float to_world[9];
    float to_object[12];
    uint32_t shape; int32_t flip_normals;
    float pad[2];
};

struct DMeshEmitter {
    uint32_t first_face, n_faces, pmf_offset, cdf_offset;
    float sum, normalization;
    int32_t has_normals, flip_normals;
    int32_t mesh, pad[3];
};

#define LRT_MAX_HIER_LEVELS 16

struct DCamera {
    float s2c[16];
    float to_world[12];
    float near_clip, far_clip;
    int32_t medium, pad;
    float ppo_x, ppo_y;
};

struct DFilm {
    int32_t width, height;
    int32_t crop_offset_x, crop_offset_y;
    float scale_x, scale_y, offset_x, offset_y;
    int32_t channels, has_alpha, rfilter, fcount;
    float rf_radius, rf_inv_radius; int32_t fn, pad;
    float rf_coeff[10];
    int32_t pad2[2];
};

struct DEnv {
    int32_t type;
    int32_t emitter;
    uint32_t w, h;
    float scale;
    float bsphere_c[3]; float bsphere_r;
    float to_world[9];
    float to_local[9];
    float patch_size[2], inv_patch_size[2];
    uint32_t max_patch[2];
    int32_t n_levels;
    uint32_t level_offset[LRT_MAX_HIER_LEVELS];
    uint32_t level_width[LRT_MAX_HIER_LEVELS];
    float radiance[3];
};

struct DDistGrid {
    const uint16_t *d;
    float lo[3]; float cell, inv_cell;
    int32_t n[3]; int32_t enabled;
};

struct DScene {
    const float4 *nodes;
    const float4 *tris;
    const float *positions;
    const float4 *vattr;
    const uint32_t *faces, *face_shape;
    const DShape *shapes; const DBsdf *bsdfs; const DTexture *textures; const DMedium *media; const DBioMedium *bio; const DHetMedium *het; const DEmitter *emitters;
    const float *tex_data;
    const float4 *env_data;
    const float *env_hier;
    uint32_t n_faces, n_emitters;
    int32_t root_is_leaf, has_null_bsdf;
    int32_t nee_fast_reject;
    int32_t one_shape;
    uint32_t root_leaf_first, root_leaf_count;
    DCamera cam; DFilm film; DEnv env;
    DDistGrid grid;
    const DSphere *spheres;
    uint32_t n_spheres, pad_sph;
    const DMeshEmitter *mesh_emitters;
    const float *mesh_emitter_tab;
};

#define LRT_CONST __attribute__((address_space(4)))
typedef const LRT_CONST DScene &SceneRef;
typedef const LRT_CONST DFilm &FilmRef;
typedef const LRT_CONST DEnv &EnvRef;
typedef const LRT_CONST DDistGrid &GridRef;
typedef const LRT_CONST DScene *ScenePtr;

struct DRenderParams {
    int32_t integrator, max_depth, rr_depth, hide_emitters;
    uint32_t spp, log2_spp;
    uint32_t seed_value;
    uint32_t base_seed, seed;
    uint32_t ld_count, pad1;
    uint32_t tile_rank, tile_count;
    int32_t grad_medium;
    uint32_t tiles_x, tiles_y, profile;
    uint32_t pad2;
    uint64_t n_lanes;
    const uint32_t *pixel_slot;
    uint32_t pass_index, spp_total;
    const unsigned long long *pass_in;
    unsigned long long *pass_out;
};

struct DPathStreams {
    float4 *o_maxt;
    float4 *d_eta;
    float4 *tp_pdf;
    float4 *res_flags;
    float4 *lp_lane;
    uint2  *rng;
    float2 *tdepth;
    float4 *hit;
    float4 *w1, *w2, *w3, *w4;
};

#define LRT_INTEGRATOR_VOLPATHMIS_PLAIN 102
#define LRT_INTEGRATOR_VOLPATH_HET 101
#define LRT_INTEGRATOR_VOLPATH_CLOSED 103

#define PF_DEPTH_MASK   0x0000ffffu
#define PF_MEDIUM_SHIFT 16
#define PF_MEDIUM_MASK  0x00ff0000u
#define PF_CHANNEL_SHIFT 24
#define PF_SPECULAR     (1u << 26)
#define PF_VALID        (1u << 27)
#define PF_NOHIT        (1u << 28)
#define PF_BIO_SCATTERED (1u << 29)
#define PF_LONG_QUERY   (1u << 29)
#define PF_HAVE_SI      (1u << 29)
#define PF_LAST_NULL    (1u << 30)
#define PF_BIO_EMIT     (1u << 30)
#define PF_BIO_FULL     (1u << 31)

struct DCounters {
    uint32_t pad[4];
    unsigned long long n_shadow;
    unsigned long long n_iter;
    unsigned long long next_lane;
    unsigned long long n_records;
    unsigned long long prof_cycles[4], prof_tiles[4];
    unsigned long long prof_wg[6];
    unsigned long long n_closed_guard;
};

struct DLdsInfo {
    const uint4 *blob;
    uint32_t blob_bytes, nodes_off, verts_off, tris_off, stack_off, total_bytes;
};

struct DLaunch {
    DRenderParams rp; DLdsInfo li; DPathStreams q0, q1;
    float4 *dl0, *dl1;
    uint32_t P, pad; DCounters *cnt; const uint32_t *pixel_list; uint64_t lane_begin, n;
    float4 *L_buf; const float *grad_image; const float *wfilm; double *grads;
    float *film; float *sample_out; uint64_t sample_base;
    float *dgrid;
};
typedef const LRT_CONST DRenderParams &RpRef;
typedef const LRT_CONST DLaunch *LaunchPtr;

}
```

### liverrenderer_amd/csrc/dshade.h

```cpp
#pragma once
#include "device_types.h"
#include "dmath.h"
#include "../../include/liverrt.h"

namespace lrt {

#define LRT_BLOCK 256
#define LRT_STACK 32

template <class T> DEV T tab(const T *table, uint32_t i, bool worth_a_look = true) {
    if (!worth_a_look) return table[i];
    const uint32_t i0 = (uint32_t) __builtin_amdgcn_readfirstlane((int) i);
    if (__builtin_amdgcn_ballot_w64(true) != 0ull && __builtin_amdgcn_ballot_w64(i != i0) == 0ull)
    { T out; __builtin_memcpy(&out, reinterpret_cast<const LRT_CONST T *>((uintptr_t) table) + i0, sizeof(T)); return out; }
    return table[i];
}

struct Ray { V3 o, d; float maxt; };
struct Hit { float t, u, v; uint32_t prim; uint32_t slot = 0xffffffffu; };
struct SI { bool valid; float t; V3 p, n; Frame sh; V2 uv; V3 dp_du, dp_dv, wi; uint32_t prim, shape; };

DEV float slab_rcp(float x) { return fmin_(fmax_(__builtin_amdgcn_rcpf(x), -1e20f), 1e20f); }
DEV void test_tri(const float4 *__restrict__ tris, uint32_t slot, V3 o, V3 d, float maxt, Hit &best) {
    float4 a = tris[3 * slot], b = tris[3 * slot + 1], c = tris[3 * slot + 2];
// ... 114 lines not shown
    const f32x2 vix = { ix, ix }, viy = { iy, iy }, viz = { iz, iz }, vox = { ox, ox }, voy = { oy, oy }, voz = { oz, oz };
    const uint32_t DONE = 0x10000u;
    int sp = 0; uint32_t cur = 0;
    for (;;) {
        while (cur < 0x8000u) {
            LRT_TRAV_COUNT(0)
            const float4 *nd = L.nodes + 4 * cur;
            float4 n0 = nd[0], n1 = nd[1], n2 = nd[2], n3 = nd[3];
            float limit = fmin_(best.t, r.maxt);
            const f32x2 vax = pk_fma(f32x2{ n0.x, n0.y }, vix, vox), vay = pk_fma(f32x2{ n0.z, n0.w }, viy, voy), vaz = pk_fma(f32x2{ n2.x, n2.y }, viz, voz);
            const f32x2 vbx = pk_fma(f32x2{ n1.x, n1.y }, vix, vox), vby = pk_fma(f32x2{ n1.z, n1.w }, viy, voy), vbz = pk_fma(f32x2{ n2.z, n2.w }, viz, voz);
            const float ax0 = vax.x, ax1 = vax.y, ay0 = vay.x, ay1 = vay.y, az0 = vaz.x, az1 = vaz.y;
            const float bx0 = vbx.x, bx1 = vbx.y, by0 = vby.x, by1 = vby.y, bz0 = vbz.x, bz1 = vbz.y;
            float tmin0 = fmax_(fmax_(fmin_(ax0, ax1), fmin_(ay0, ay1)), fmax_(fmin_(az0, az1), 0.f));
            float tmax0 = fmin_(fmin_(fmax_(ax0, ax1), fmax_(ay0, ay1)), fmin_(fmax_(az0, az1), limit));
            float tmin1 = fmax_(fmax_(fmin_(bx0, bx1), fmin_(by0, by1)), fmax_(fmin_(bz0, bz1), 0.f));
            float tmax1 = fmin_(fmin_(fmax_(bx0, bx1), fmax_(by0, by1)), fmin_(fmax_(bz0, bz1), limit));
            bool h0 = tmin0 <= tmax0 * 1.000002f, h1 = tmin1 <= tmax1 * 1.000002f;
            const uint32_t c0 = f2u(n3.x), c1 = f2u(n3.y);
            if (h0 && h1) {
                bool swap = tmin1 < tmin0;
                stack[sp * STRIDE] = (uint16_t) (swap ? c0 : c1); ++sp;
                cur = swap ? c1 : c0;
            } else if (h0 || h1) cur = h0 ? c0 : c1;
            else if (sp == 0) cur = DONE;
            else { --sp; cur = stack[sp * STRIDE]; }
        }
        if (cur == DONE) break;
        uint32_t slot = cur & 0x7fffu, last;
        do {
            LRT_TRAV_COUNT(2)
            const uint2 ix = L.tris[slot];
            last = (ix.y >> 16) & 1u;
            test_tri_lds(L, ix, slot, o, d, r.maxt, best);
            ++slot;
        } while (!last);
        if (ANY_HIT && best.prim != 0xffffffffu) return best;
        if (sp == 0) break;
        --sp; cur = stack[sp * STRIDE];
    }
    if (best.prim != 0xffffffffu) { best.slot = best.prim >> 16; best.prim &= 0x7fffu; }
    return best;
}

template <int STRIDE>
struct LdsTracer {
    static constexpr bool kExt = false;
    const LdsScene &L; uint16_t *stack;
    DEV Hit closest(const Ray &r) const { return trace_lds<false, STRIDE>(L, r, stack); }
    DEV Hit any(const Ray &r) const { return trace_lds<true, STRIDE>(L, r, stack); }
    DEV SI surface(SceneRef s, const Ray &r, const Hit &h) const;
};

DEV float dist_grid_lower_bound(GridRef g, V3 p) {
    float fx = (p.x - g.lo[0]) * g.inv_cell, fy = (p.y - g.lo[1]) * g.inv_cell, fz = (p.z - g.lo[2]) * g.inv_cell;
    int ix = min(max((int) fx, 0), g.n[0] - 1), iy = min(max((int) fy, 0), g.n[1] - 1), iz = min(max((int) fz, 0), g.n[2] - 1);
    union { uint16_t u; _Float16 h; } cv; cv.u = g.d[(uint32_t) ((iz * g.n[1] + iy) * g.n[0] + ix)];
    float D = (float) cv.h;
    float cx = fx - ((float) ix + .5f), cy = fy - ((float) iy + .5f), cz = fz - ((float) iz + .5f);
    return D - __builtin_amdgcn_sqrtf(cx * cx + cy * cy + cz * cz) * (g.cell * 1.001f);
}

#ifndef LRT_GRID_STEPS
#define LRT_GRID_STEPS 3
#endif
template <int STEPS = LRT_GRID_STEPS>
DEV bool segment_proven_empty(GridRef g, V3 o, V3 d, float maxt) {
    if (!g.enabled || !(maxt < 1e30f)) return false;
    float len = __builtin_amdgcn_sqrtf(dot(d, d));
    float remaining = maxt * len * 1.01f, inv_len = __builtin_amdgcn_rcpf(len);
    V3 p = o;
    for (int k = 0; k < STEPS; ++k) {
        float lb = dist_grid_lower_bound(g, p);
        if (remaining < lb) return true;
        if (!(lb > .5f * g.cell)) return false;
        float adv = lb * .99f;
        p = p + d * (adv * inv_len);
        remaining -= adv * .995f;
    }
    return false;
}

template <int K>
DEV bool segment_covered_by_balls(GridRef g, V3 o, V3 d, float maxt) {
    if (!g.enabled || !(maxt < 1e30f)) return false;
    const float len = __builtin_amdgcn_sqrtf(dot(d, d));
    const float L = maxt * len * 1.01f;
#define LRT_FRAC(k) (((float) (k) + .5f) / (float) K)
    float lb[K];
#pragma unroll
    for (int k = 0; k < K; ++k) lb[k] = dist_grid_lower_bound(g, fma3(d, maxt * LRT_FRAC(k), o)) * .995f;
    float covered = 0.f; bool ok = true;
#pragma unroll
    for (int k = 0; k < K; ++k) {
        const float c = L * LRT_FRAC(k);
        ok = ok && (lb[k] > 0.f) && (c - lb[k] <= covered);
        covered = fmax_(covered, c + lb[k]);
    }
    return ok && covered >= L;
#undef LRT_FRAC
}

DEV bool segment_free_of_surfaces(GridRef g, V3 o, V3 d, float maxt) {
#ifdef LRT_SPHERE_TRACE
    return segment_proven_empty(g, o, d, maxt);
#else
    return segment_covered_by_balls<2>(g, o, d, maxt);
#endif
}

DEV SI compute_si(SceneRef sc, const Ray &r, const Hit &h, const LdsScene *L = nullptr) {
    const bool valid = h.prim != 0xffffffffu;
    float t = kInf; V3 p(0.f), n(0.f), shn(0.f), shs(0.f), sht(0.f), dp_du(0.f), dp_dv(0.f), wi = -r.d;
    V2 uv = { 0.f, 0.f }; uint32_t f = 0xffffffffu, shp = 0xffffffffu;
    if (valid) {
        f = h.prim; shp = 0u; if (!sc.one_shape) shp = sc.face_shape[f];
        const DShape sd = tab(sc.shapes, shp, sc.one_shape);
        uint32_t i0, i1, i2; V3 p0, p1, p2;
        if (L && h.slot != 0xffffffffu) {
            const uint2 ix = L->tris[h.slot];
            i0 = ix.x & 0xffffu; i1 = ix.x >> 16; i2 = ix.y & 0xffffu;
            const float4 a = L->verts[i0], b = L->verts[i1], c = L->verts[i2];
            p0 = V3(a.x, a.y, a.z); p1 = V3(b.x, b.y, b.z); p2 = V3(c.x, c.y, c.z);
        } else {
            i0 = sc.faces[3 * f]; i1 = sc.faces[3 * f + 1]; i2 = sc.faces[3 * f + 2];
            p0 = V3(sc.positions[3 * i0], sc.positions[3 * i0 + 1], sc.positions[3 * i0 + 2]);
            p1 = V3(sc.positions[3 * i1], sc.positions[3 * i1 + 1], sc.positions[3 * i1 + 2]);
            p2 = V3(sc.positions[3 * i2], sc.positions[3 * i2 + 1], sc.positions[3 * i2 + 2]);
        }
        float b1 = h.u, b2 = h.v, b0 = 1.f - b1 - b2;
        t = h.t;
        p = V3(fma_(p0.x, b0, fma_(p1.x, b1, p2.x * b2)), fma_(p0.y, b0, fma_(p1.y, b1, p2.y * b2)), fma_(p0.z, b0, fma_(p1.z, b1, p2.z * b2)));
        V3 dp0 = p1 - p0, dp1 = p2 - p0;
        n = normalize(cross(dp0, dp1));
        uv = { b1, b2 };
        Basis bs = coordinate_system(n);
        dp_du = bs.s; dp_dv = bs.t;
        if (sd.has_texcoords) {
            const float2 t0 = *reinterpret_cast<const float2 *>(sc.vattr + 2 * (size_t) i0 + 1), t1 = *reinterpret_cast<const float2 *>(sc.vattr + 2 * (size_t) i1 + 1),
                         t2 = *reinterpret_cast<const float2 *>(sc.vattr + 2 * (size_t) i2 + 1);
            V2 uv0 = { t0.x, t0.y }, uv1 = { t1.x, t1.y }, uv2 = { t2.x, t2.y };
            uv = { fma_(uv2.x, b2, fma_(uv1.x, b1, uv0.x * b0)), fma_(uv2.y, b2, fma_(uv1.y, b1, uv0.y * b0)) };
            V2 duv0 = { uv1.x - uv0.x, uv1.y - uv0.y }, duv1 = { uv2.x - uv0.x, uv2.y - uv0.y };
            float det = fma_(duv0.x, duv1.y, -(duv0.y * duv1.x)), inv_det = rcp(det);
            if (det != 0.f) {
                dp_du = V3(fma_(duv1.y, dp0.x, -(duv0.y * dp1.x)), fma_(duv1.y, dp0.y, -(duv0.y * dp1.y)), fma_(duv1.y, dp0.z, -(duv0.y * dp1.z))) * inv_det;
                dp_dv = V3(fma_(-duv1.x, dp0.x, duv0.x * dp1.x), fma_(-duv1.x, dp0.y, duv0.x * dp1.y), fma_(-duv1.x, dp0.z, duv0.x * dp1.z)) * inv_det;
            }
        }
        if (sd.has_normals) {
            const float4 a0 = sc.vattr[2 * (size_t) i0], a1 = sc.vattr[2 * (size_t) i1], a2 = sc.vattr[2 * (size_t) i2];
            V3 n0(a0.x, a0.y, a0.z), n1(a1.x, a1.y, a1.z), n2(a2.x, a2.y, a2.z);
            V3 ni(fma_(n2.x, b2, fma_(n1.x, b1, n0.x * b0)), fma_(n2.y, b2, fma_(n1.y, b1, n0.y * b0)), fma_(n2.z, b2, fma_(n1.z, b1, n0.z * b0)));
            float il = rsqrt_(squared_norm(ni));
            shn = ni * il;
        } else shn = n;
        if (sd.flip_normals) { n = V3(-n.x, -n.y, -n.z); shn = V3(-shn.x, -shn.y, -shn.z); }
        shs = normalize(fma3(shn, -dot(shn, dp_du), dp_du));
        if (dp_du.x == 0.f && dp_du.y == 0.f && dp_du.z == 0.f) shs = coordinate_system(shn).s;
        sht = cross(shn, shs);
        V3 md(-r.d.x, -r.d.y, -r.d.z);
        wi = V3(dot(md, shs), dot(md, sht), dot(md, shn));
    }
    SI si;
    si.valid = valid; si.t = t; si.p = p; si.n = n; si.sh.s = shs; si.sh.t = sht; si.sh.n = shn; si.uv = uv;
    si.dp_du = dp_du; si.dp_dv = dp_dv; si.wi = wi; si.prim = f; si.shape = shp;
    return si;
}

DEV SI GlobalTracer::surface(SceneRef s, const Ray &r, const Hit &h) const { return compute_si(s, r, h); }
template <int STRIDE> DEV SI LdsTracer<STRIDE>::surface(SceneRef s, const Ray &r, const Hit &h) const { return compute_si(s, r, h, &L); }


DEV bool solve_quadratic(float a, float b, float c, float &x0, float &x1) {
    const bool linear_case = a == 0.f, valid_linear = linear_case && b != 0.f;
    x0 = x1 = -c / b;
    const float discrim = fma_(b, b, -(4.f * a * c));
    const bool valid_quadratic = !linear_case && discrim >= 0.f;
    const float sqrt_discrim = __builtin_sqrtf(discrim);
    const float temp = -0.5f * (b + __builtin_copysignf(sqrt_discrim, b));
    const float x0p = temp / a, x1p = c / temp;
    const float x0m = fmin_(x0p, x1p), x1m = fmax_(x0p, x1p);
    if (!linear_case) { x0 = x0m; x1 = x1m; }
    return valid_linear || valid_quadratic;
}
DEV float sphere_intersect(V3 center, float radius, const Ray &r) {
    const V3 l = r.o - center, d = r.d;
    const float plane_t = dot(-l, d) / norm(d);
    const V3 o = fma3(d, plane_t, r.o) - center;
    const float A = squared_norm(d), B = 2.f * dot(o, d), C = squared_norm(o) - sqr(radius);
    float near_t, far_t;
// ... 866 lines not shown
```

### liverrenderer_amd/csrc/kernels.h

```cpp
#pragma once
#include "dshade.h"
#include "record.h"

namespace lrt {

#ifndef LRT_STAMP_KIND
#define LRT_STAMP_KIND 0
#endif
struct StampClock {
    unsigned long long *acc; unsigned long long t; bool on;
    DEV void start(unsigned long long *a, bool enable) { acc = a; on = enable; t = on ? __builtin_amdgcn_s_memtime() : 0ull; }
    DEV void at(int k) { if (on) { const unsigned long long now = __builtin_amdgcn_s_memtime(); if ((threadIdx.x & 63u) == 0) atomicAdd(&acc[k], now - t); t = now; } }
};

template <bool LD>
DEV uint64_t lane_rng_inc(RpRef rp, uint32_t lane) {
    if (LD) {
        const uint32_t pixel = (rp.log2_spp != 0xffffffffu) ? (lane >> rp.log2_spp) : (lane / rp.spp);
        uint32_t v0, v1; tea32(rp.base_seed, rp.spp * pixel + rp.seed, &v0, &v1);
        return (uint64_t) v0 | ((uint64_t) (rp.pass_index * rp.spp + (lane - pixel * rp.spp)) << 32);
    }
    uint32_t v0, v1; tea32(rp.seed_value, lane, &v0, &v1);
    return ((uint64_t) v1 << 1) | 1u;
}
// ... 124 lines not shown
                else { si.valid = false; si.t = kInf; }
            }
            if (si.t < mei.t) mei.t = kInf;
            needs_intersection = false;
            bool spectral = M.has_spectral_extinction;
            if (spectral) {
                float t = fmin_(remaining_dist, fmin_(mei.t, si.t)) - mei.mint;
                V3 tr = exp_neg(t, mei.combined);
                V3 ffp = (si.t < mei.t || mei.t > remaining_dist) ? tr : tr * mei.combined;
                float tr_pdf = idx3(ffp, channel);
                transmittance = transmittance * ((tr_pdf > 0.f) ? div_uniform(tr, tr_pdf) : V3(0.f));
            }
            if ((mei.t > remaining_dist) && mei.valid()) total_dist = ds.dist;
            if (mei.t > remaining_dist) mei.t = kInf;
            escaped_medium = !mei.valid();
            active_medium = mei.valid();
            if (active_medium) {
                total_dist += mei.t;
                ray.o = mei.p;
                si.t = si.t - mei.t;
                if (spectral) transmittance = transmittance * mei.sigma_n;
                else transmittance = transmittance * (mei.sigma_n / mei.combined);
            }
        }
        bool intersect = active_surface && needs_intersection;
        if (intersect) { n_shadow++; Hit h = tr.closest(ray); si = tr.surface(sc, ray, h); needs_intersection = false; }
        active_surface = active_surface || escaped_medium;
        if (active_surface) total_dist += si.t;
        active_surface = active_surface && si.valid && !active_medium;
        if (active_surface) {
            transmittance = transmittance * bsdf_null_transmission(sc, tab(sc.shapes, si.shape, sc.one_shape).bsdf);
            ray = spawn_ray(si.p, si.n, ray.d);
        }
        ray.maxt = remaining_dist;
        needs_intersection = needs_intersection || active_surface;
        active = (active_medium || active_surface) && any_nonzero(transmittance);
        if (active_surface) { const DShape sd = tab(sc.shapes, si.shape, sc.one_shape); if (is_medium_transition(sd)) medium = target_medium(sd, ray.d, si.n); }
    }
    return transmittance * emitter_val;
}

struct WaveCount {
    unsigned long long *c;
    DEV void operator++(int) {
        const unsigned long long m = __ballot(true);
        if ((threadIdx.x & 63u) == (uint32_t) (__ffsll((long long) m) - 1)) atomicAdd(c, (unsigned long long) __popcll(m));
    }
};

template <bool HET, bool CLOSED = false, typename SMP, typename TR, typename CNT>
DEV bool volpath_iteration(SceneRef sc, RpRef rp, PathState &s, SMP &rng, const TR &tr, CNT &n_shadow, CNT &n_extra, bool fresh = false, StampClock *clk = nullptr,
                           unsigned long long *guard = nullptr) {
    constexpr bool PRE = !HET;
    uint32_t depth = s.flags & PF_DEPTH_MASK;
    bool proven_empty = (s.flags & PF_NOHIT) != 0;
    float ff_t = s.ff_t;
    const bool needs_intersection = !(HET && (s.flags & PF_HAVE_SI));
    bool act_null_scatter = false;
    Hit hkeep; hkeep.t = s.hit.x; hkeep.u = s.hit.y; hkeep.v = s.hit.z; hkeep.prim = f2u(s.hit.w);
    if (PRE) { hkeep.t = kInf; hkeep.u = hkeep.v = 0.f; hkeep.prim = 0xffffffffu; }
    int medium = (int) ((s.flags & PF_MEDIUM_MASK) >> PF_MEDIUM_SHIFT) - 1;
    const uint32_t channel = (s.flags >> PF_CHANNEL_SHIFT) & 3u;
    bool specular_chain = (s.flags & PF_SPECULAR) != 0, valid_ray = (s.flags & PF_VALID) != 0;
    const uint32_t max_depth = (uint32_t) rp.max_depth;
    V3 throughput = s.tp, result = CLOSED ? V3(0.f) : s.res;
    bool broken = false;
    float eta = s.eta;
    Ray ray; ray.o = s.o; ray.d = s.d; ray.maxt = s.maxt;
    auto commit = [&]() {
        s.tp = throughput; s.res = result; s.eta = eta; s.o = ray.o; s.d = ray.d; s.maxt = ray.maxt;
        s.flags = (depth & PF_DEPTH_MASK) | ((uint32_t) (medium + 1) << PF_MEDIUM_SHIFT) | (channel << PF_CHANNEL_SHIFT) |
                  (specular_chain ? PF_SPECULAR : 0u) | (valid_ray ? PF_VALID : 0u);
    };
    auto termination_stage = [&]() -> bool {
        bool a = any_nonzero(throughput);
        const float q = fmin_(max3(throughput) * sqr(eta), .95f);
        const bool perform_rr = depth > (uint32_t) rp.rr_depth;
        if (a) { const float u = rng.next(); a = (u < q) || !perform_rr; }
        if (perform_rr) throughput = throughput * rcp(q);
        return a && depth < max_depth;
    };
    uint32_t nohit = 0;
    float cache_t = u2f(0x7fc00000u);
    auto free_flight_stage = [&]() {
        if (medium < 0) return;
        const DMedium M = tab(sc.media, medium);
        cache_t = medium_sampled_t(M, rng.next(), channel);
        if (sc.grid.enabled) { const MI m2 = medium_interaction_at(M, ray, cache_t); if (m2.valid() && segment_free_of_surfaces(sc.grid, ray.o, ray.d, m2.t)) nohit = PF_NOHIT; }
    };
    bool active = true;
    if (!PRE) active = termination_stage();
    else if (fresh) { active = termination_stage(); if (active) { free_flight_stage(); ff_t = cache_t; proven_empty = nohit != 0; nohit = 0; cache_t = u2f(0x7fc00000u); } }
    if (!active) { commit(); return false; }

    bool active_medium = medium >= 0, active_surface = !active_medium;
    bool act_medium_scatter = false, escaped_medium = false;
    MI mei; mei.t = kInf;
    SI si; si.valid = false; si.t = kInf;
    if (!active_medium) rng.skip(2);
    if (active_medium) {
        const DMedium M = tab(sc.media, medium);
        const bool het = HET && M.het;
        if (PRE) mei = medium_interaction_at(M, ray, ff_t);
        else { const float sample = rng.next(); mei = het ? het_sample_interaction(M, tab(sc.het, medium), ray, sample) : medium_sample_interaction(M, ray, sample, channel); }
        if (mei.valid() && !het) ray.maxt = mei.t;
        if (!needs_intersection) si = surface_of(tr, sc, ray, hkeep);
        else if (!proven_empty) {
            hkeep = tr.closest(ray);
            if (PRE) { si.valid = hkeep.prim != 0xffffffffu; si.t = si.valid ? hkeep.t : kInf; }
            else si = tr.surface(sc, ray, hkeep);
        }
        if (si.t < mei.t) mei.t = kInf;
        if (M.has_spectral_extinction) {
            float t = fmin_(mei.t, si.t) - mei.mint;
            V3 tr = exp_neg(t, mei.combined);
            V3 pdf = (si.t < mei.t) ? tr : tr * mei.combined;
            float tr_pdf = idx3(pdf, channel);
            throughput = throughput * ((tr_pdf > 0.f) ? div_uniform(tr, tr_pdf) : V3(0.f));
        }
        escaped_medium = !mei.valid();
        active_medium = mei.valid();
        if (!active_medium) rng.skip(1);
        if (active_medium) {
            const float u_null = rng.next();
            if (HET) {
                const float null_scatter_prob = mean3(mei.sigma_n / mei.combined);
                act_null_scatter = u_null < null_scatter_prob;
                if (M.has_spectral_extinction && act_null_scatter) throughput = throughput * (mei.sigma_n / null_scatter_prob);
            }
            act_medium_scatter = !act_null_scatter;
            if (act_medium_scatter) { depth += 1; s.lp = mei.p; }
        }
    }
    active = active && depth < max_depth;
    act_medium_scatter = act_medium_scatter && active;
    if (HET && act_null_scatter) { ray.o = mei.p; hkeep.t = si.t - mei.t; }
    if (clk) clk->at(2);
    if (!act_medium_scatter) rng.skip(3);
    if (act_medium_scatter) {
        const DMedium M = tab(sc.media, medium);
        if (HET && M.het) {
            if (M.has_spectral_extinction) throughput = throughput * (mei.sigma_s / mean3(mei.sigma_t / mei.combined));
            else throughput = throughput * (mei.sigma_s / mei.sigma_t);
        } else if (M.has_spectral_extinction) throughput = throughput * V3(M.w_spec[0], M.w_spec[1], M.w_spec[2]);
        else throughput = throughput * V3(M.w_plain[0], M.w_plain[1], M.w_plain[2]);
        bool sample_emitters = M.sample_emitters != 0;
        valid_ray = true;
        specular_chain = !sample_emitters;
        if (!sample_emitters) rng.skip(1);
        if (sample_emitters) {
            bool rejected = false;
            if (sc.nee_fast_reject) {
                SMP saved = rng;
                float sx, sy; rng.next2(sx, sy);
                float u3 = rng.next();
                const float lo = 9.5367431640625e-7f, hi = 1.f - 9.5367431640625e-7f;
                bool interior = sc.env.type == LRT_EMITTER_CONSTANT || (sx > lo && sx < hi && sy > lo && sy < hi);
                rejected = interior;
                if (!(1.f - u3 >= idx3(V3(M.nee_vmin[0], M.nee_vmin[1], M.nee_vmin[2]), channel))) {
                    float sampled_t = 0.f + (-m_log(1.f - u3) / idx3(V3(M.sigma_t[0], M.sigma_t[1], M.sigma_t[2]), channel));
                    V3 cc(sc.env.bsphere_c[0], sc.env.bsphere_c[1], sc.env.bsphere_c[2]);
                    float dist = 2.f * fmax_(sc.env.bsphere_r, norm(mei.p - cc));
                    rejected = interior && sampled_t <= dist * 0.998f - 1e-3f;
                }
                if (!rejected) rng = saved;
            }
            if (!rejected && CLOSED) {
                float sx, sy; rng.next2(sx, sy);
                DirSample ds; (void) sample_emitter_direction<TR::kExt>(sc, mei.p, sx, sy, &ds);
                if (ds.pdf != 0.f) {
                    const Ray r2 = spawn_ray_to(mei.p, V3(0.f), ds.p);
                    if (!(r2.maxt > 0.f)) rng.skip(1);
                    else { const MI m2 = medium_sample_interaction(M, r2, rng.next(), channel); if (!m2.valid()) n_shadow++; }
                }
            } else if (!rejected) {
                DirSample ds;
                V3 emitted = volpath_sample_emitter<HET>(sc, rng, mei.p, V3(0.f), false, 0, V3(0.f), medium, channel, &ds, tr, n_shadow);
                float phase_val = phase_eval(M, mei.wi, ds.d);
                V3 c = throughput * phase_val * emitted * mis_weight(ds.pdf, ds.delta ? 0.f : phase_val);
                result = result + c;
            }
        }
        (void) rng.next();
        float s2x, s2y; rng.next2(s2x, s2y);
        V3 wo; float phase_pdf; phase_sample(M, mei.wi, s2x, s2y, &wo, &phase_pdf);
        if (phase_pdf > 0.f) {
            ray = spawn_ray(mei.p, V3(0.f), wo);
            s.last_pdf = phase_pdf;
        }
    }
    active_surface = active_surface || escaped_medium;
    bool intersect = active_surface && !escaped_medium;
    if (PRE) {
        Hit h = hkeep;
        if (intersect) h = tr.closest(ray);
        if (active_surface) si = tr.surface(sc, ray, h);
    } else if (intersect) { Hit h = tr.closest(ray); si = tr.surface(sc, ray, h); }
    if (active_surface) {
        if (!CLOSED && rp.hide_emitters && depth == 0 && intersect) {
            bool skip = si.valid && tab(sc.shapes, si.shape, sc.one_shape).emitter >= 0;
            if (skip) {
                Ray r2 = spawn_ray(si.p, si.n, ray.d);
                bool a = true; Hit h; h.prim = 0xffffffffu; h.t = kInf; h.u = h.v = 0.f;
                while (a) {
                    h = tr.closest(r2);
                    a = hit_on_emitter(tr, sc, h);
                    if (a) { SI s2 = surface_of(tr, sc, r2, h); r2 = spawn_ray(s2.p, s2.n, r2.d); }
                }
                si = surface_of(tr, sc, r2, h);
            }
        }
        bool count_direct = (depth == 0) || specular_chain;
        int emitter = CLOSED ? (si.valid ? -1 : sc.env.emitter) : si_emitter(sc, si);
        bool active_e = emitter >= 0 && !(depth == 0 && rp.hide_emitters);
        if (active_e) {
            if (CLOSED) { broken = broken || !count_direct; result = result + throughput * emitter_eval_env(sc, -si.wi); }
            else {
                float emitter_pdf = 1.f;
                if (!count_direct) emitter_pdf = pdf_emitter_direction<TR::kExt>(sc, s.lp, si, emitter);
                V3 emitted = emitter_eval(sc, emitter, si);
                V3 contrib = count_direct ? throughput * emitted : throughput * mis_weight(s.last_pdf, emitter_pdf) * emitted;
                result = result + contrib;
            }
        }
    }
    active_surface = active_surface && si.valid;
    if (!active_surface) rng.skip(3);
    if (active_surface) {
        const DShape sd = tab(sc.shapes, si.shape, sc.one_shape);
        int b = sd.bsdf;
        int flags = tab(sc.bsdfs, b, sc.one_shape).flags;
        bool active_e = !CLOSED && (flags & F_SMOOTH) && (depth + 1 < max_depth);
        if (!active_e) rng.skip(1);
        if (active_e) {
            DirSample ds;
            V3 emitted = volpath_sample_emitter<HET>(sc, rng, si.p, si.n, true, si.shape, si.n, medium, channel, &ds, tr, n_shadow);
            V3 wo = si.sh.to_local(ds.d);
            V3 bsdf_val = bsdf_eval<TR::kExt>(sc, b, si, wo);
            float bpdf = bsdf_pdf<TR::kExt>(sc, b, si, wo);
            V3 c = throughput * bsdf_val * mis_weight(ds.pdf, ds.delta ? 0.f : bpdf) * emitted;
            result = result + c;
        }
        float s1 = rng.next(), s2x, s2y; rng.next2(s2x, s2y);
        const BSDFSample bs = bsdf_sample<CLOSED, TR::kExt>(sc, b, si, s1, s2x, s2y);
        throughput = throughput * bs.weight;
        eta *= bs.eta;
        ray = spawn_ray(si.p, si.n, si.sh.to_world(bs.wo));
        bool non_null = !(bs.type & F_NULL);
        if (non_null) { depth += 1; s.lp = si.p; s.last_pdf = bs.pdf; valid_ray = true; }
        specular_chain = specular_chain || (non_null && (bs.type & F_DELTA));
        specular_chain = specular_chain && !(bs.type & F_SMOOTH);
        if (is_medium_transition(sd)) medium = target_medium(sd, ray.d, si.n);
    }
    active = active && (active_surface || active_medium);
    if (clk) clk->at(3);
    if (PRE) {
        if (active) { if (!termination_stage()) { active = false; n_extra++; } else free_flight_stage(); }
        if (clk) clk->at(4);
    } else if (active) {
        SMP pk = rng;
        bool a2 = any_nonzero(throughput);
        float q2 = fmin_(max3(throughput) * sqr(eta), .95f);
        if (a2) { float u = pk.next(); a2 = (u < q2) || !(depth > (uint32_t) rp.rr_depth); }
        a2 = a2 && depth < max_depth;
        if (!a2) { active = false; n_extra++; rng = pk; }
        else if (medium >= 0 && sc.grid.enabled && !(HET && act_null_scatter)) {
            const DMedium M = tab(sc.media, medium);
            if (!(HET && M.het)) {
                const float t2 = medium_sampled_t(M, pk.next(), channel);
                const MI m2 = medium_interaction_at(M, ray, t2);
                if (m2.valid() && segment_free_of_surfaces(sc.grid, ray.o, ray.d, m2.t)) nohit = PF_NOHIT;
            }
        }
    }
    commit();
    s.flags |= nohit; s.ff_t = cache_t;
#ifndef LRT_CLOSED_NO_GUARD
    if (CLOSED && (broken || (active && !(result.x == 0.f && result.y == 0.f && result.z == 0.f)))) atomicAdd(guard, 1ull);
#endif
    if (HET && act_null_scatter && active) { s.flags |= PF_HAVE_SI; s.hit = make_float4(hkeep.t, hkeep.u, hkeep.v, u2f(hkeep.prim)); }
    return active;
}

template <typename SMP, typename TR>
DEV bool path_iteration(SceneRef sc, RpRef rp, PathState &s, SMP &rng, const TR &tr, uint32_t &n_shadow) {
    uint32_t depth = s.flags & PF_DEPTH_MASK;
    bool prev_bsdf_delta = (s.flags & PF_SPECULAR) != 0, valid_ray = (s.flags & PF_VALID) != 0;
    const uint32_t max_depth = (uint32_t) rp.max_depth;
    V3 throughput = s.tp, result = s.res;
    float eta = s.eta;
    Ray ray; ray.o = s.o; ray.d = s.d; ray.maxt = s.maxt;
    auto commit = [&]() {
        s.tp = throughput; s.res = result; s.eta = eta; s.o = ray.o; s.d = ray.d; s.maxt = ray.maxt;
        s.flags = (depth & PF_DEPTH_MASK) | (prev_bsdf_delta ? PF_SPECULAR : 0u) | (valid_ray ? PF_VALID : 0u);
    };
    if (max_depth == 0) { commit(); return false; }
    Hit pi = tr.closest(ray);
    if (rp.hide_emitters && depth == 0) {
        bool skip = hit_on_emitter(tr, sc, pi);
        if (skip) {
            SI s0 = surface_of(tr, sc, ray, pi);
            Ray r2 = spawn_ray(s0.p, s0.n, ray.d);
            bool a = true; Hit h; h.prim = 0xffffffffu; h.t = kInf; h.u = h.v = 0.f;
            while (a) {
                h = tr.closest(r2);
                a = hit_on_emitter(tr, sc, h);
                if (a) { SI s2 = surface_of(tr, sc, r2, h); r2 = spawn_ray(s2.p, s2.n, r2.d); }
            }
            pi = h; ray = r2;
        }
    }
    SI si = surface_of(tr, sc, ray, pi);
    int emitter = si_emitter(sc, si);
    if (emitter >= 0) {
        float em_pdf = 0.f;
        if (!prev_bsdf_delta) em_pdf = pdf_emitter_direction<TR::kExt>(sc, s.lp, si, emitter);
        float mis_bsdf = mis_weight(s.last_pdf, em_pdf);
        V3 em = (s.last_pdf > 0.f) ? emitter_eval(sc, emitter, si) : V3(0.f);
        em = em * mis_bsdf;
        result = V3(fma_(throughput.x, em.x, result.x), fma_(throughput.y, em.y, result.y), fma_(throughput.z, em.z, result.z));
    }
    bool active_next = (depth + 1 < max_depth) && si.valid;
    if (!active_next) {
        float a0, a1; rng.next2(a0, a1); (void) rng.next(); rng.next2(a0, a1); (void) rng.next();
        if (si.valid && !(tab(sc.bsdfs, tab(sc.shapes, si.shape, sc.one_shape).bsdf, sc.one_shape).flags & F_NULL)) valid_ray = true;
        commit(); return false;
    }
    const DShape sd = tab(sc.shapes, si.shape, sc.one_shape);
    int b = sd.bsdf;
    bool active_em = (tab(sc.bsdfs, b, sc.one_shape).flags & F_SMOOTH) != 0;
    DirSample ds; ds.pdf = 0.f; ds.delta = false; ds.d = V3(0.f);
    V3 em_weight(0.f), wo(0.f);
    float sx, sy; rng.next2(sx, sy);
    if (active_em) {
        em_weight = sample_emitter_direction<TR::kExt>(sc, si.p, sx, sy, &ds);
// ... 32 lines not shown
}

}
#include "kernels_bio.h"
#include "kernels_mis.h"
namespace lrt {

template <RecordLayout LAYOUT = RecordLayout::Wide, bool READLANE = true, bool COMPACT = false, bool LONGQ = false>
DEV void retire_and_compact_wave(SceneRef sc, RpRef rp, bool had_path, bool alive, const PathState &s,
                                 float *__restrict__ film, float *__restrict__ sample_out, uint64_t sample_base,
                                 const LRT_CONST DPathStreams &qout, size_t pool, uint32_t P, uint32_t *s_out , StampClock *clk = nullptr) {
    const uint32_t lane_in_wave = threadIdx.x & 63u;
    const int region = !(s.flags & PF_MEDIUM_MASK) ? 2 : ((s.flags & PF_NOHIT) ? 0 : ((LONGQ && (s.flags & PF_LONG_QUERY)) ? 3 : 1));
    const unsigned long long m0 = __ballot(alive && region == 0), m1 = __ballot(alive && region == 1), m2 = __ballot(alive && region == 2);
    const unsigned long long m3 = LONGQ ? __ballot(alive && region == 3) : 0ull;
    uint32_t base = 0;
    if (lane_in_wave < (LONGQ ? 4u : 3u)) {
        const uint32_t c = (uint32_t) __popcll(lane_in_wave == 0 ? m0 : (lane_in_wave == 1 ? m1 : ((!LONGQ || lane_in_wave == 2) ? m2 : m3)));
        if (c) base = atomicAdd(&s_out[lane_in_wave], c);
    }
    uint32_t b;
    if (READLANE) {
        const uint32_t b0 = (uint32_t) __builtin_amdgcn_readlane((int) base, 0), b1 = (uint32_t) __builtin_amdgcn_readlane((int) base, 1), b2 = (uint32_t) __builtin_amdgcn_readlane((int) base, 2);
        b = region == 0 ? b0 : (region == 1 ? b1 : b2);
        if (LONGQ) { const uint32_t b3 = (uint32_t) __builtin_amdgcn_readlane((int) base, 3); if (region == 3) b = b3; }
    } else b = __shfl(base, region);
    if (clk) clk->at(5);
    if (alive) {
        const unsigned long long mine = region == 0 ? m0 : (region == 1 ? m1 : ((!LONGQ || region == 2) ? m2 : m3));
        const uint32_t slot = b + (uint32_t) __popcll(mine & ((1ull << lane_in_wave) - 1ull));
        store_state<LAYOUT, COMPACT>(qout, pool + (region == 0 ? slot : (region == 1 ? P + slot : ((!LONGQ || region == 2) ? 2u * P - 1u - slot : P - 1u - slot))), s);
    }
    if (clk) clk->at(6);
    if (rp.pass_out && had_path && !alive) rp.pass_out[lane_local_index(rp, s.lane)] = s.rng_state;
    finish_paths_wave(sc, rp, film, sample_out, sample_base, had_path && !alive, s.lane, s.res, (s.flags & PF_VALID) != 0);
}

template <int INTEGRATOR, int BLOCK, bool LDS_BVH, bool LD, bool COMPACT = false, bool EXT = false>
__global__ void __launch_bounds__(BLOCK, BLOCK == 512 ? 2 : (BLOCK == 768 ? 3 : 4))
k_render(ScenePtr scp, LaunchPtr lp) {
    SceneRef sc = *scp;
    const LRT_CONST DLaunch &A = *lp;
    RpRef rp = A.rp;
    const LRT_CONST DLdsInfo &li = A.li;
    const uint32_t P = A.P;
    extern __shared__ __align__(16) unsigned char smem[];
    __shared__ uint32_t s_in[4], s_out[4], s_ticket, s_fresh;
    __shared__ unsigned long long s_fresh_base, s_prof[8];
#ifdef LRT_STAMP
    __shared__ unsigned long long s_stamp[16];
    if (threadIdx.x < 16) s_stamp[threadIdx.x] = 0;
#endif
    const uint32_t tid = threadIdx.x, lane_in_wave = tid & 63u;
    constexpr bool READLANE = INTEGRATOR != LRT_INTEGRATOR_PATH && INTEGRATOR != LRT_INTEGRATOR_BIOVOLPATH06;
    constexpr bool LONGQ = INTEGRATOR == LRT_INTEGRATOR_BIOVOLPATH;
    constexpr bool CLOSED = INTEGRATOR == LRT_INTEGRATOR_VOLPATH_CLOSED;
    constexpr RecordLayout LAYOUT = record_layout(INTEGRATOR);
    if (tid < 8) s_prof[tid] = 0;
    const unsigned long long t_wg_start = (rp.profile & 1u) ? wall_clock64() : 0ull;
    unsigned long long t_loop_start = 0ull, t_barrier = 0ull;
    LdsScene L{};
    if (LDS_BVH) {
        const uint4 *src = li.blob; uint4 *dst = reinterpret_cast<uint4 *>(smem);
        for (uint32_t k = tid; k < li.blob_bytes / 16u; k += BLOCK) dst[k] = src[k];
        L.nodes = reinterpret_cast<const float4 *>(smem + li.nodes_off); L.verts = reinterpret_cast<const float4 *>(smem + li.verts_off);
        L.tris = reinterpret_cast<const uint2 *>(smem + li.tris_off);
        L.n_faces = sc.n_faces; L.root_is_leaf = (uint32_t) sc.root_is_leaf; L.root_first = sc.root_leaf_first; L.root_count = sc.root_leaf_count;
    }
    const LdsTracer<BLOCK> tr_lds_tri{ L, reinterpret_cast<uint16_t *>(smem + li.stack_off) + tid };
    const GlobalTracer tr_glb_tri{ sc, reinterpret_cast<int *>(smem) + tid };
    const ExtTracer<LdsTracer<BLOCK>> tr_lds_ext{ tr_lds_tri, sc };
    const ExtTracer<GlobalTracer> tr_glb_ext{ tr_glb_tri, sc };
    const auto &tr_lds = pick<EXT>(tr_lds_tri, tr_lds_ext);
    const auto &tr_glb = pick<EXT>(tr_glb_tri, tr_glb_ext);
    const size_t pool = (size_t) blockIdx.x * 2u * P;
    uint32_t parity = 0;
    if (tid == 0) { s_in[0] = s_in[1] = s_in[2] = 0; if (LONGQ) s_in[3] = 0; }
    bool lanes_left = true;
    constexpr bool VP_LDS_COUNT = INTEGRATOR == LRT_INTEGRATOR_VOLPATH || CLOSED;
    __shared__ unsigned long long s_cnt[2];
    if (VP_LDS_COUNT && tid < 2) s_cnt[tid] = 0;
    WaveCount wc_shadow{ &s_cnt[0] }, wc_extra{ &s_cnt[1] };
    uint32_t n_shadow = 0, n_extra = 0, n_trips = 0, n_loaded = 0;
    if (rp.profile & 1u) t_loop_start = wall_clock64();
    for (;;) {
        if (tid == 0) {
            const uint32_t want = P - (s_in[0] + s_in[1] + s_in[2] + (LONGQ ? s_in[3] : 0u));
            uint32_t got = 0; unsigned long long base = 0;
            if (want && lanes_left) {
                base = atomicAdd(&A.cnt->next_lane, (unsigned long long) want);
                if (base < rp.n_lanes) got = (uint32_t) (rp.n_lanes - base < (unsigned long long) want ? rp.n_lanes - base : (unsigned long long) want);
                lanes_left = base + want < rp.n_lanes;
            }
            s_fresh = got; s_fresh_base = base; s_ticket = 0; s_out[0] = s_out[1] = s_out[2] = 0; if (LONGQ) s_out[3] = 0;
        }
        __syncthreads();
        const uint32_t n_a = s_in[0], n_c = s_in[1], n_b = s_in[2], n_l = LONGQ ? s_in[3] : 0u, fresh = s_fresh;
        const unsigned long long fresh_base = s_fresh_base;
        if (n_a + n_c + n_b + n_l + fresh == 0) break;
        const uint32_t ta = (n_a + 63u) >> 6, tc = (n_c + 63u) >> 6, tb = (n_b + 63u) >> 6, tf = (fresh + 63u) >> 6;
        const uint32_t tcl = tc + (LONGQ ? (n_l + 63u) >> 6 : 0u);
        const uint32_t n_tiles = ta + tcl + tb + tf;
        for (;;) {
            uint32_t t = 0;
            if (lane_in_wave == 0) t = atomicAdd(&s_ticket, 1u);
            t = (uint32_t) __builtin_amdgcn_readfirstlane((int) t);
            if (t >= n_tiles) break;
            const unsigned long long t_begin = (rp.profile & 1u) ? wall_clock64() : 0ull;
#ifdef LRT_STAMP
            StampClock clk; clk.start(s_stamp, LRT_STAMP_KIND == 0 ? t < ta : (LRT_STAMP_KIND == 1 ? (t >= ta && t < ta + tcl) : (LRT_STAMP_KIND == 2 ? (t >= ta + tcl && t < ta + tcl + tb) : t >= ta + tcl + tb)));
#endif
            bool had_path = false, alive = false;
            PathState s; s.flags = 0; s.lane = 0; s.res = V3(0.f);
            if (t < ta + tcl + tb) {
                uint32_t i;
                if (t < ta) { i = (t << 6) + lane_in_wave; had_path = i < n_a; }
                else if (t < ta + tc) { i = ((t - ta) << 6) + lane_in_wave; had_path = i < n_c; i += P; }
                else if (LONGQ && t < ta + tcl) { i = ((t - ta - tc) << 6) + lane_in_wave; had_path = i < n_l; i = P - 1u - i; }
                else { i = ((t - ta - tcl) << 6) + lane_in_wave; had_path = i < n_b; i = 2u * P - 1u - i; }
                if (had_path) { load_state<LAYOUT, COMPACT>(parity ? A.q1 : A.q0, pool + i, s); if (!VP_LDS_COUNT) n_loaded += 1; }
            } else {
                const uint32_t i = ((t - ta - tcl - tb) << 6) + lane_in_wave;
                had_path = i < fresh;
                if (had_path) s = generate_camera_path<LD>(sc, rp, A.pixel_list, A.lane_begin + fresh_base + i);
            }
            if (VP_LDS_COUNT) {
                const uint32_t n_had = (uint32_t) __popcll(__ballot(had_path));
                n_trips += n_had;
                if (t < ta + tcl + tb) n_loaded += n_had;
            }
#ifdef LRT_STAMP
            clk.at(0);
#endif
            if (had_path) {
                SamplerT<LD> rng = COMPACT ? lane_rng_resume_word<LD>(rp, s.lane, s.rng_state, s.rng_word) : lane_rng_resume<LD>(rp, s.lane, s.rng_state);
#ifdef LRT_STAMP
                clk.at(1);
#endif
                if (INTEGRATOR == LRT_INTEGRATOR_PATH) alive = LDS_BVH ? path_iteration(sc, rp, s, rng, tr_lds, n_shadow) : path_iteration(sc, rp, s, rng, tr_glb, n_shadow);
                else if (INTEGRATOR == LRT_INTEGRATOR_BIOVOLPATH) { const bool fresh_tile = t >= ta + tcl + tb; alive = LDS_BVH ? biovolpath_iteration(sc, rp, s, rng, tr_lds, n_shadow, n_extra, fresh_tile) : biovolpath_iteration(sc, rp, s, rng, tr_glb, n_shadow, n_extra, fresh_tile); }
                else if (INTEGRATOR == LRT_INTEGRATOR_BIOVOLPATH06) alive = LDS_BVH ? biovolpath06_iteration(sc, rp, s, rng, tr_lds) : biovolpath06_iteration(sc, rp, s, rng, tr_glb);
                else if (INTEGRATOR == LRT_INTEGRATOR_VOLPATHMIS) alive = LDS_BVH ? volpathmis_iteration<true>(sc, rp, s, rng, tr_lds, n_shadow) : volpathmis_iteration<true>(sc, rp, s, rng, tr_glb, n_shadow);
                else if (INTEGRATOR == LRT_INTEGRATOR_VOLPATHMIS_PLAIN) alive = LDS_BVH ? volpathmis_iteration<false>(sc, rp, s, rng, tr_lds, n_shadow) : volpathmis_iteration<false>(sc, rp, s, rng, tr_glb, n_shadow);
                else if (INTEGRATOR == LRT_INTEGRATOR_VOLPATH_HET) alive = LDS_BVH ? volpath_iteration<true>(sc, rp, s, rng, tr_lds, n_shadow, n_extra) : volpath_iteration<true>(sc, rp, s, rng, tr_glb, n_shadow, n_extra);
                else {
                    const bool fresh_tile = t >= ta + tcl + tb;
#ifdef LRT_STAMP
                    StampClock *const pclk = &clk;
#else
                    StampClock *const pclk = nullptr;
#endif
                    unsigned long long *const guard = CLOSED ? &A.cnt->n_closed_guard : nullptr;
                    alive = LDS_BVH ? volpath_iteration<false, CLOSED>(sc, rp, s, rng, tr_lds, wc_shadow, wc_extra, fresh_tile, pclk, guard) : volpath_iteration<false, CLOSED>(sc, rp, s, rng, tr_glb, wc_shadow, wc_extra, fresh_tile, pclk, guard);
                }
                s.rng_state = rng.state;
                if (!VP_LDS_COUNT) n_trips += 1;
            }
#ifdef LRT_STAMP
            retire_and_compact_wave<LAYOUT, READLANE, COMPACT, LONGQ>(sc, rp, had_path, alive, s, A.film, A.sample_out, A.sample_base, parity ? A.q0 : A.q1, pool, P, s_out, &clk);
            clk.at(7);
            if (clk.on && lane_in_wave == 0) atomicAdd(&s_stamp[15], 1ull);
#else
            retire_and_compact_wave<LAYOUT, READLANE, COMPACT, LONGQ>(sc, rp, had_path, alive, s, A.film, A.sample_out, A.sample_base, parity ? A.q0 : A.q1, pool, P, s_out);
#endif
            if ((rp.profile & 1u) && lane_in_wave == 0) {
                const int region = t < ta ? 0 : (t < ta + tcl ? 1 : (t < ta + tcl + tb ? 2 : 3));
                atomicAdd(&s_prof[region], wall_clock64() - t_begin); atomicAdd(&s_prof[4 + region], 1ull);
            }
        }
        { const unsigned long long tb0 = (rp.profile & 1u) ? wall_clock64() : 0ull;
        __syncthreads();
        if (rp.profile & 1u) t_barrier += wall_clock64() - tb0; }
        if (tid == 0) { s_in[0] = s_out[0]; s_in[1] = s_out[1]; s_in[2] = s_out[2]; if (LONGQ) s_in[3] = s_out[3]; }
        parity ^= 1u;
    }
    if ((rp.profile & 1u) && (tid & 63u) == 0) {
        const unsigned long long t_end = wall_clock64();
        if (tid == 0) { atomicAdd(&A.cnt->prof_wg[0], t_loop_start - t_wg_start); atomicMax(&A.cnt->prof_wg[1], t_end); atomicMax(&A.cnt->prof_wg[2], ~t_wg_start); atomicAdd(&A.cnt->prof_wg[3], t_end - t_wg_start); atomicMax(&A.cnt->prof_wg[5], t_wg_start); }
        atomicAdd(&A.cnt->prof_wg[4], t_barrier);
    }
    if ((rp.profile & 1u) && tid < 8) { if (tid < 4) atomicAdd(&A.cnt->prof_cycles[tid], s_prof[tid]); else atomicAdd(&A.cnt->prof_tiles[tid - 4], s_prof[tid]); }
#ifdef LRT_TRAV_STATS
    if (tid == 0 && blockIdx.x == 0) printf("[trav, so far] closest: node steps %llu (lanes %.1f), leaf steps %llu (lanes %.1f); any-hit: node steps %llu (lanes %.1f), leaf steps %llu (lanes %.1f)\n", g_trav[0], (double) g_trav[1] / g_trav[0], g_trav[2], (double) g_trav[3] / g_trav[2], g_trav[4], (double) g_trav[5] / g_trav[4], g_trav[6], (double) g_trav[7] / g_trav[6]);
#endif
#ifdef LRT_STAMP
    __syncthreads();
    if (tid == 0 && blockIdx.x == 7) printf("[stamp] tiles of kind %d in workgroup 7: %llu; cycles per tile: ticket+load issue %.0f, record wait+TEA %.0f, to the end of the medium interaction / ray query %.0f, scatter + surface %.0f, termination+free flight %.0f, ballots+slots %.0f, stores %.0f, film %.0f\n", LRT_STAMP_KIND, s_stamp[15],
        (double) s_stamp[0] / s_stamp[15], (double) s_stamp[1] / s_stamp[15], (double) s_stamp[2] / s_stamp[15], (double) s_stamp[3] / s_stamp[15], (double) s_stamp[4] / s_stamp[15], (double) s_stamp[5] / s_stamp[15], (double) s_stamp[6] / s_stamp[15], (double) s_stamp[7] / s_stamp[15]);
#endif
    if (!VP_LDS_COUNT) {
        n_trips += n_extra;
        for (int off = 32; off > 0; off >>= 1) {
            n_shadow += __shfl_down(n_shadow, off); n_trips += __shfl_down(n_trips, off); n_loaded += __shfl_down(n_loaded, off);
        }
    }
    if (lane_in_wave == 0) {
        if (!VP_LDS_COUNT && n_shadow) atomicAdd(&A.cnt->n_shadow, (unsigned long long) n_shadow);
        if (n_trips) atomicAdd(&A.cnt->n_iter, (unsigned long long) n_trips);
        if (n_loaded) atomicAdd(&A.cnt->n_records, (unsigned long long) n_loaded);
    }
    if (VP_LDS_COUNT) {
        __syncthreads();
        if (tid == 0) {
            if (s_cnt[0]) atomicAdd(&A.cnt->n_shadow, s_cnt[0]);
            if (s_cnt[1]) atomicAdd(&A.cnt->n_iter, s_cnt[1]);
        }
    }
}

DEV float point_triangle_dist2(V3 p, V3 a, V3 ab, V3 ac) {
    V3 ap = p - a;
    float d1 = dot(ab, ap), d2 = dot(ac, ap);
    if (d1 <= 0.f && d2 <= 0.f) return dot(ap, ap);
    V3 bp = ap - ab;
    float d3 = dot(ab, bp), d4 = dot(ac, bp);
    if (d3 >= 0.f && d4 <= d3) return dot(bp, bp);
    float vc = d1 * d4 - d3 * d2;
    if (vc <= 0.f && d1 >= 0.f && d3 <= 0.f) { V3 r = ap - ab * (d1 / (d1 - d3)); return dot(r, r); }
    V3 cp = ap - ac;
    float d5 = dot(ab, cp), d6 = dot(ac, cp);
    if (d6 >= 0.f && d5 <= d6) return dot(cp, cp);
    float vb = d5 * d2 - d1 * d6;
    if (vb <= 0.f && d2 >= 0.f && d6 <= 0.f) { V3 r = ap - ac * (d2 / (d2 - d6)); return dot(r, r); }
    float va = d3 * d6 - d5 * d4;
    if (va <= 0.f && (d4 - d3) >= 0.f && (d5 - d6) >= 0.f) { V3 r = bp - (ac - ab) * ((d4 - d3) / ((d4 - d3) + (d5 - d6))); return dot(r, r); }
    float denom = 1.f / (va + vb + vc);
    V3 r = ap - ab * (vb * denom) - ac * (vc * denom);
    return dot(r, r);
}

__global__ void __launch_bounds__(LRT_BLOCK)
k_build_dist_grid(const float4 *__restrict__ tris, uint32_t n_slots, DDistGrid g, uint16_t *__restrict__ out, float abs_margin,
                  const DSphere *__restrict__ spheres, uint32_t n_spheres) {
    const size_t n_cells = (size_t) g.n[0] * g.n[1] * g.n[2];
    const size_t c = (size_t) blockIdx.x * LRT_BLOCK + threadIdx.x;
    if (c >= n_cells) return;
    const int ix = (int) (c % g.n[0]), iy = (int) ((c / g.n[0]) % g.n[1]), iz = (int) (c / ((size_t) g.n[0] * g.n[1]));
    const V3 p(g.lo[0] + ((float) ix + .5f) * g.cell, g.lo[1] + ((float) iy + .5f) * g.cell, g.lo[2] + ((float) iz + .5f) * g.cell);
    float best = kInf;
    for (uint32_t sl = 0; sl < n_slots; ++sl) {
        const float4 a = tris[3 * sl], b = tris[3 * sl + 1], cc = tris[3 * sl + 2];
        float d2 = point_triangle_dist2(p, V3(a.x, a.y, a.z), V3(b.x, b.y, b.z), V3(cc.x, cc.y, cc.z));
        if (!(d2 >= 0.f)) d2 = 0.f;
        best = fmin_(best, d2);
    }
    for (uint32_t k = 0; k < n_spheres; ++k) {
        const DSphere &S = spheres[k];
        const float ds = __builtin_fabsf(norm(p - V3(S.center[0], S.center[1], S.center[2])) - S.radius);
        best = fmin_(best, ds * ds);
    }
    float d = __builtin_sqrtf(best) * .999f - abs_margin;
    d = d > 0.f ? fmin_(d, 60000.f) : 0.f;
    union { uint16_t u; _Float16 h; } cv; cv.h = (_Float16) d;
    if ((float) cv.h > d) cv.u -= 1;
    out[c] = cv.u;
}

template <bool WEIGHTS_ONLY>
__global__ void __launch_bounds__(LRT_BLOCK)
k_splat_lanes(ScenePtr scp, LaunchPtr lp) {
    RpRef rp = lp->rp;
    const float4 *__restrict__ lane_L = lp->L_buf; const uint32_t *__restrict__ pixel_list = lp->pixel_list;
    const uint64_t slot_base = lp->lane_begin, n = lp->n;
    float *__restrict__ film = lp->film;
    SceneRef sc = *scp;
    FilmRef F = sc.film;
    const uint64_t i = (uint64_t) blockIdx.x * LRT_BLOCK + threadIdx.x;
    const uint32_t me = threadIdx.x & 63u;
    const bool have = i < n;
    V3 L(0.f); float alpha = 0.f; FilmFootprint fp{}; uint32_t key = 0xffffffffu;
    if (have) {
        const uint64_t j = slot_base + i;
        const uint32_t lane = slot_to_lane(rp, pixel_list, j);
        if (!WEIGHTS_ONLY) {
            const float4 v = lane_L[i];
            L = V3(v.x, v.y, v.z); alpha = v.w;
            if (rp.integrator == LRT_INTEGRATOR_PATH && alpha == 0.f) L = V3(0.f);
        }
        int px, py; lane_to_pixel(sc, rp, lane, &px, &py);
        float jx, jy; lane_jitter(rp, lane, j, jx, jy);
        fp = film_footprint(F, px, py, jx, jy);
        key = fp.key();
// ... 160 lines not shown
```

### liverrenderer_amd/csrc/scene_prep.cpp

```cpp
#include "scene_prep.h"
#include <cmath>
#include <cstring>
#include <cstdlib>
#include <algorithm>
#include <stdexcept>
#include <string>

namespace lrt {

PrepOptions PrepOptions::from_env() {
    PrepOptions o;
    if (getenv("LRT_BVH_LEAF")) o.bvh_leaf = std::max(1, atoi(getenv("LRT_BVH_LEAF")));
    o.no_lds_bvh = getenv("LRT_NO_LDS_BVH") != nullptr;
    o.no_dist_grid = getenv("LRT_NO_DIST_GRID") != nullptr;
    if (getenv("LRT_DIST_GRID_RES")) o.dist_grid_res = std::max(8, std::min(256, atoi(getenv("LRT_DIST_GRID_RES"))));
    o.no_nee_reject = getenv("LRT_NO_NEE_REJECT") != nullptr;
    return o;
}

static void m4_mul(const float *a, const float *b, float *r) {
    for (int i = 0; i < 4; ++i) for (int j = 0; j < 4; ++j) { float s = a[4 * i] * b[j]; for (int k = 1; k < 4; ++k) s = fmaf(a[4 * i + k], b[4 * k + j], s); r[4 * i + j] = s; }
}
static void m4_ident(float *m) { for (int i = 0; i < 16; ++i) m[i] = (i % 5 == 0) ? 1.f : 0.f; }

static void build_camera(const lrt_scene_desc &d, DCamera &cam, DFilm &film) {
    const lrt_film_desc &F = d.film; const lrt_sensor_desc &C = d.sensor;
    float fw = (float) F.width, fh = (float) F.height;
    float rsx = (float) F.crop_width / fw, rsy = (float) F.crop_height / fh, rox = (float) F.crop_offset_x / fw, roy = (float) F.crop_offset_y / fh;
    float aspect = fw / fh, recip = 1.f / (C.far_clip - C.near_clip);
    float tn = (float) tan((double) (C.fov_x * .5f) * (3.14159265358979323846 / 180.0));
    (void) recip;
    float S1i[16], T1i[16], S2i[16], T2i[16], Pit[16], t0[16], t1[16], t2[16], it[16];
    m4_ident(S1i); S1i[0] = 1.f / (1.f / rsx); S1i[5] = 1.f / (1.f / rsy); S1i[10] = 1.f / 1.f;
    m4_ident(T1i); T1i[12] = rox; T1i[13] = roy; T1i[14] = -0.f;
    m4_ident(S2i); S2i[0] = 1.f / -0.5f; S2i[5] = 1.f / (-0.5f * aspect); S2i[10] = 1.f;
    m4_ident(T2i); T2i[12] = 1.f; T2i[13] = 1.f / aspect; T2i[14] = -0.f;
    float Pinv[16]; m4_ident(Pinv); Pinv[0] = tn; Pinv[5] = tn; Pinv[10] = 0.f; Pinv[15] = 1.f / C.near_clip; Pinv[11] = 1.f;
    Pinv[14] = (C.near_clip - C.far_clip) / (C.far_clip * C.near_clip);
    for (int i = 0; i < 4; ++i) for (int j = 0; j < 4; ++j) Pit[4 * i + j] = Pinv[4 * j + i];
    m4_mul(S1i, T1i, t0); m4_mul(t0, S2i, t1); m4_mul(t1, T2i, t2); m4_mul(t2, Pit, it);
    for (int i = 0; i < 4; ++i) for (int j = 0; j < 4; ++j) cam.s2c[4 * i + j] = it[4 * j + i];
    memcpy(cam.to_world, C.to_world, sizeof(float) * 12);
    cam.near_clip = C.near_clip; cam.far_clip = C.far_clip; cam.medium = C.medium;
    cam.ppo_x = fw * C.principal_point_offset_x / (float) F.crop_width; cam.ppo_y = fh * C.principal_point_offset_y / (float) F.crop_height;

    film.width = F.crop_width; film.height = F.crop_height; film.crop_offset_x = F.crop_offset_x; film.crop_offset_y = F.crop_offset_y;
    film.scale_x = 1.f / (float) F.crop_width; film.scale_y = 1.f / (float) F.crop_height;
    film.offset_x = -(float) F.crop_offset_x * film.scale_x; film.offset_y = -(float) F.crop_offset_y * film.scale_y;
    film.has_alpha = F.has_alpha; film.channels = F.has_alpha ? 5 : 4; film.rfilter = F.rfilter;
    film.rf_radius = 0.5f; film.rf_inv_radius = 1.f;
    if (F.rfilter == LRT_RFILTER_GAUSSIAN) {
        float stddev = F.rfilter_param; film.rf_radius = 4.f * stddev;
        static const double coeff[10] = { 9.992604880e-1, -4.977025247e-1, 1.222248550e-1, -1.932406282e-2, 2.136713061e-3,
                                          -1.679873860e-4, 9.202145248e-6, -3.329417433e-7, 7.128382794e-9, -6.821193280e-11 };
        double sc = 1; for (int i = 0; i < 10; ++i) { film.rf_coeff[i] = (float) (coeff[i] * sc); sc /= (double) stddev * (double) stddev; }
        float x = film.rf_radius * film.rf_radius, x2 = x * x, x4 = x2 * x2, x8 = x4 * x4; const float *c = film.rf_coeff;
        float a0 = fmaf(x, c[1], c[0]), a1 = fmaf(x, c[3], c[2]), a2 = fmaf(x, c[5], c[4]), a3 = fmaf(x, c[7], c[6]), a4 = fmaf(x, c[9], c[8]);
        float b0 = fmaf(x2, a1, a0), b1 = fmaf(x2, a3, a2), c0 = fmaf(x4, b1, b0);
        film.rf_coeff[0] -= fmaf(x8, a4, c0);
    } else if (F.rfilter == LRT_RFILTER_TENT) { film.rf_radius = F.rfilter_param; film.rf_inv_radius = 1.f / film.rf_radius; }
    film.fn = (int) ceilf(film.rf_radius - .5f); film.fcount = 2 * film.fn + 1;
}

static void inverse3(const float *m16, float *out9) {
    double m[3][3]; for (int i = 0; i < 3; ++i) for (int j = 0; j < 3; ++j) m[i][j] = m16[4 * i + j];
    double det = m[0][0] * (m[1][1] * m[2][2] - m[1][2] * m[2][1]) - m[0][1] * (m[1][0] * m[2][2] - m[1][2] * m[2][0]) + m[0][2] * (m[1][0] * m[2][1] - m[1][1] * m[2][0]);
    double id = 1.0 / det;
    out9[0] = (float) ((m[1][1] * m[2][2] - m[1][2] * m[2][1]) * id); out9[1] = (float) ((m[0][2] * m[2][1] - m[0][1] * m[2][2]) * id); out9[2] = (float) ((m[0][1] * m[1][2] - m[0][2] * m[1][1]) * id);
    out9[3] = (float) ((m[1][2] * m[2][0] - m[1][0] * m[2][2]) * id); out9[4] = (float) ((m[0][0] * m[2][2] - m[0][2] * m[2][0]) * id); out9[5] = (float) ((m[0][2] * m[1][0] - m[0][0] * m[1][2]) * id);
    out9[6] = (float) ((m[1][0] * m[2][1] - m[1][1] * m[2][0]) * id); out9[7] = (float) ((m[0][1] * m[2][0] - m[0][0] * m[2][1]) * id); out9[8] = (float) ((m[0][0] * m[1][1] - m[0][1] * m[1][0]) * id);
}

static uint32_t log2i_ceil(uint32_t v) { uint32_t r = 0; while ((1u << r) < v) ++r; return r; }

static void build_hierarchy(const std::vector<float> &lum, uint32_t w, uint32_t h, DEnv &E, std::vector<float> &out) {
    uint32_t npx = w - 1, npy = h - 1;
    E.patch_size[0] = 1.f / (float) npx; E.patch_size[1] = 1.f / (float) npy;
    E.inv_patch_size[0] = (float) npx; E.inv_patch_size[1] = (float) npy;
    E.max_patch[0] = npx - 1; E.max_patch[1] = npy - 1;
    uint32_t max_level = log2i_ceil(std::max(npx, npy));
    struct L { uint32_t w, h, off; };
    std::vector<L> lv; uint32_t total = 0;
    auto add = [&](uint32_t lw, uint32_t lh) { lv.push_back({ lw, lh, total }); total += (lw * lh + 3u) & ~3u; };
    add(w, h);
    uint32_t lx = npx, ly = npy;
    for (int level = (int) max_level; level >= 0; --level) { lx += lx & 1u; ly += ly & 1u; add(lx, ly); lx >>= 1; ly >>= 1; }
    if (lv.size() > LRT_MAX_HIER_LEVELS) throw std::runtime_error("environment map too large for the sampling hierarchy");
    out.assign(total, 0.f);
    auto index = [](uint32_t x, uint32_t y, uint32_t width) { return ((x & 1u) | (((x & ~1u) | (y & 1u)) << 1)) + ((y & ~1u) * width); };
    float *l0 = &out[lv[0].off], *l1 = &out[lv[1].off];
    const float *in = lum.data(); double sum = 0.0;
    for (uint32_t y = 0; y < npy; ++y) { for (uint32_t x = 0; x < npx; ++x) { float avg = .25f * (in[0] + in[1] + in[w] + in[w + 1]); sum += (double) avg; l1[index(x, y, lv[1].w)] = avg; ++in; } ++in; }
    float scale = (float) ((double) (npx * npy) / sum);
    for (uint32_t i = 0; i < w * h; ++i) l0[i] = lum[i] * scale;
    for (uint32_t i = 0; i < lv[1].w * lv[1].h; ++i) l1[i] *= scale;
    lx = npx; ly = npy;
    for (uint32_t level = 2; level <= max_level + 1; ++level) {
        const float *a = &out[lv[level - 1].off]; float *b = &out[lv[level].off];
        lx = (lx + 1u) >> 1; ly = (ly + 1u) >> 1;
        for (uint32_t y = 0; y < ly; ++y) for (uint32_t x = 0; x < lx; ++x) { const float *d0 = a + index(x * 2, y * 2, lv[level - 1].w); b[index(x, y, lv[level].w)] = d0[0] + d0[1] + d0[2] + d0[3]; }
    }
    E.n_levels = (int) lv.size();
    for (size_t i = 0; i < lv.size(); ++i) { E.level_offset[i] = lv[i].off; E.level_width[i] = lv[i].w; }
}

struct LdsLayout {
    size_t nodes_b, verts_b, tris_b, stacks_b;
    size_t blob() const { return nodes_b + verts_b + tris_b; }
    size_t total() const { return blob() + stacks_b; }
};
static LdsLayout lds_layout(const HostBVH &b, uint32_t n_vertices) {
    return { b.nodes.size() / 16 * 64, ((size_t) n_vertices * 16 + 15) & ~size_t(15), (b.tris.size() / 12 * 8 + 15) & ~size_t(15), (size_t) 2 * (b.max_depth + 2) * 1024 };
}
size_t lds_image_bytes(const HostBVH &b, uint32_t n_vertices) { return lds_layout(b, n_vertices).total(); }

static bool lds_possible(const lrt_scene_desc &d, const PrepOptions &opt) { return d.n_faces > 0 && d.n_faces <= 32767 && d.n_vertices <= 65535 && !opt.no_lds_bvh; }
bool lds_image_fits(const lrt_scene_desc &d, const HostBVH &b, const PrepOptions &opt) {
    return lds_possible(d, opt) && b.nodes.size() / 16 <= 32767 && b.tris.size() / 12 <= 32767 && lds_image_bytes(b, d.n_vertices) <= opt.lds_limit;
}

static void build_lds_image(const lrt_scene_desc &d, const HostBVH &bvh, PreparedScene &P) {
    const LdsLayout lay = lds_layout(bvh, d.n_vertices);
    const size_t n_nodes = bvh.nodes.size() / 16, n_slots = bvh.tris.size() / 12, n_verts = d.n_vertices;
    const size_t nodes_b = lay.nodes_b, verts_b = lay.verts_b;
    std::vector<unsigned char> &blob = P.lds_blob; blob.assign(lay.blob(), 0);
    memcpy(blob.data(), bvh.nodes.data(), nodes_b);
    float *v = reinterpret_cast<float *>(blob.data() + nodes_b);
    for (size_t i = 0; i < n_verts; ++i) { v[4 * i] = d.positions[3 * i]; v[4 * i + 1] = d.positions[3 * i + 1]; v[4 * i + 2] = d.positions[3 * i + 2]; v[4 * i + 3] = 0.f; }
    uint16_t *t = reinterpret_cast<uint16_t *>(blob.data() + nodes_b + verts_b);
    for (size_t sl = 0; sl < n_slots; ++sl) {
        uint32_t f; memcpy(&f, &bvh.tris[12 * sl + 3], 4);
        for (int k = 0; k < 3; ++k) t[4 * sl + k] = (uint16_t) d.faces[3 * (size_t) f + k];
        t[4 * sl + 3] = (uint16_t) (f << 1);
    }
    for (size_t n = 0; n < n_nodes; ++n) {
        int32_t refs[4]; memcpy(refs, &bvh.nodes[16 * n + 12], 16);
        for (int c = 0; c < 2; ++c) if (refs[c] < 0 && refs[2 + c] > 0) t[4 * ((size_t) (uint32_t) ~refs[c] + (size_t) refs[2 + c] - 1) + 3] |= 1;
        uint32_t enc[2]; for (int c = 0; c < 2; ++c) enc[c] = refs[c] < 0 ? (0x8000u | (uint32_t) ~refs[c]) : (uint32_t) refs[c];
        memcpy(blob.data() + 64 * n + 48, enc, 8);
    }
    if (bvh.root_is_leaf && bvh.root_count) t[4 * ((size_t) bvh.root_first + bvh.root_count - 1) + 3] |= 1;
    P.lds.blob = nullptr; P.lds.blob_bytes = (uint32_t) blob.size(); P.lds.nodes_off = 0; P.lds.verts_off = (uint32_t) nodes_b; P.lds.tris_off = (uint32_t) (nodes_b + verts_b);
    P.lds.stack_off = (uint32_t) blob.size(); P.lds.total_bytes = (uint32_t) lay.total();
}

static void referenced_bounds(const lrt_scene_desc &d, const std::vector<DSphere> &spheres, float lo[3], float hi[3]) {
    for (int a = 0; a < 3; ++a) { lo[a] = INFINITY; hi[a] = -INFINITY; }
    for (uint32_t f = 0; f < 3 * d.n_faces; ++f) for (int a = 0; a < 3; ++a) { float v = d.positions[3 * (size_t) d.faces[f] + a]; lo[a] = std::min(lo[a], v); hi[a] = std::max(hi[a], v); }
    for (const DSphere &o : spheres) for (int a = 0; a < 3; ++a) { lo[a] = std::min(lo[a], o.center[a] - o.radius); hi[a] = std::max(hi[a], o.center[a] + o.radius); }
}
static void vertex_bounds(const lrt_scene_desc &d, const std::vector<DSphere> &spheres, float lo[3], float hi[3]) {
    for (int a = 0; a < 3; ++a) { lo[a] = INFINITY; hi[a] = -INFINITY; }
    for (uint32_t i = 0; i < d.n_vertices; ++i) for (int a = 0; a < 3; ++a) { lo[a] = fminf(lo[a], d.positions[3 * i + a]); hi[a] = fmaxf(hi[a], d.positions[3 * i + a]); }
    for (const DSphere &o : spheres) for (int a = 0; a < 3; ++a) { lo[a] = fminf(lo[a], o.center[a] - o.radius); hi[a] = fmaxf(hi[a], o.center[a] + o.radius); }
}

void prepare_geometry(const lrt_scene_desc &d, const PrepOptions &opt, PreparedScene &P) {
    DScene &sc = P.sc;
    memset(&sc, 0, sizeof(sc));
    std::vector<DSphere> &spheres = P.spheres;
    for (uint32_t i = 0; i < d.n_shapes; ++i) {
        const lrt_shape_desc &s = d.shapes[i];
        if (s.kind != LRT_SHAPE_SPHERE) continue;
        DSphere o; memset(&o, 0, sizeof(o));
        const float *m = s.to_world;
        for (int a = 0; a < 3; ++a) o.center[a] = m[4 * a + 3];
        o.radius = sqrtf(fmaf(m[8], m[8], fmaf(m[4], m[4], m[0] * m[0])));
        for (int a = 0; a < 3; ++a) for (int b = 0; b < 3; ++b) o.to_world[3 * a + b] = m[4 * a + b];
        double md[16]; for (int k = 0; k < 16; ++k) md[k] = m[k];
        const double c00 = md[5] * md[10] - md[6] * md[9], c01 = md[6] * md[8] - md[4] * md[10], c02 = md[4] * md[9] - md[5] * md[8];
        const double id = 1.0 / (md[0] * c00 + md[1] * c01 + md[2] * c02);
        double inv[12] = { c00 * id, (md[2] * md[9] - md[1] * md[10]) * id, (md[1] * md[6] - md[2] * md[5]) * id, 0,
                           c01 * id, (md[0] * md[10] - md[2] * md[8]) * id, (md[2] * md[4] - md[0] * md[6]) * id, 0,
                           c02 * id, (md[1] * md[8] - md[0] * md[9]) * id, (md[0] * md[5] - md[1] * md[4]) * id, 0 };
        for (int a = 0; a < 3; ++a) inv[4 * a + 3] = -(inv[4 * a] * md[3] + inv[4 * a + 1] * md[7] + inv[4 * a + 2] * md[11]);
        for (int k = 0; k < 12; ++k) o.to_object[k] = (float) inv[k];
        o.shape = i; o.flip_normals = s.flip_normals;
        if (!(o.radius > 0.f) || !std::isfinite(o.radius)) throw std::runtime_error("sphere with a zero or invalid radius");
        spheres.push_back(o);
    }
    sc.n_spheres = (uint32_t) spheres.size();
    for (uint32_t i = 0; i < d.n_emitters; ++i) {
        const lrt_emitter_desc &e = d.emitters[i];
        if (e.type == LRT_EMITTER_POINT || (e.type == LRT_EMITTER_AREA && e.shape >= 0 && (uint32_t) e.shape < d.n_shapes && d.shapes[e.shape].kind == LRT_SHAPE_MESH)) P.ext = true;
    }
    if (!spheres.empty()) P.ext = true;
    for (uint32_t i = 0; i < d.n_shapes; ++i) {
        const int32_t b = d.shapes[i].bsdf;
        if (b < 0 || (uint32_t) b >= d.n_bsdfs) continue;
        const lrt_bsdf_desc &B = d.bsdfs[b];
        if (B.type == LRT_BSDF_ROUGHDIELECTRIC || (B.type == LRT_BSDF_BUMPMAP && B.nested >= 0 && (uint32_t) B.nested < d.n_bsdfs && d.bsdfs[B.nested].type == LRT_BSDF_ROUGHDIELECTRIC)) P.ext = true;
    }
    HostBVH &bvh = P.bvh;
    {
        const int forced = opt.bvh_leaf;
        int chosen = forced ? forced : 4;
        bool done = false;
        if (!forced && lds_possible(d, opt)) {
            for (int leaf : { 2, 3, 4, 6, 8, 12, 16 }) {
                HostBVH b2; build_bvh(d.positions, d.faces, d.n_faces, b2, leaf);
                if (lds_image_fits(d, b2, opt)) { bvh = std::move(b2); chosen = leaf; done = true; break; }
            }
        }
        if (!done) build_bvh(d.positions, d.faces, d.n_faces, bvh, chosen);
        P.bvh_leaf = chosen;
    }
    sc.root_is_leaf = bvh.root_is_leaf; sc.root_leaf_first = bvh.root_first; sc.root_leaf_count = bvh.root_count;
    sc.n_faces = d.n_faces; sc.n_emitters = d.n_emitters; sc.one_shape = d.n_shapes == 1;
    if (lds_image_fits(d, bvh, opt)) { build_lds_image(d, bvh, P); P.use_lds = true; }
    sc.grid = DDistGrid{};
    if (d.n_media > 0 && (d.n_faces > 0 || !spheres.empty()) && d.n_faces <= (1u << 17) && !opt.no_dist_grid) {
        float lo[3], hi[3]; referenced_bounds(d, spheres, lo, hi);
        const float ext = std::max(hi[0] - lo[0], std::max(hi[1] - lo[1], hi[2] - lo[2]));
        const int res = opt.dist_grid_res ? opt.dist_grid_res : (d.n_faces <= (1u << 14) ? 192 : 64);
        if (ext > 0.f && std::isfinite(ext)) {
            DDistGrid g{};
            g.cell = ext / (float) res; g.inv_cell = 1.f / g.cell;
            for (int a = 0; a < 3; ++a) { g.lo[a] = lo[a]; g.n[a] = std::max(1, std::min(res, (int) std::ceil((hi[a] - lo[a]) / g.cell))); }
            float diag = std::sqrt((hi[0] - lo[0]) * (hi[0] - lo[0]) + (hi[1] - lo[1]) * (hi[1] - lo[1]) + (hi[2] - lo[2]) * (hi[2] - lo[2]));
            float amax = 0.f; for (int a = 0; a < 3; ++a) amax = std::max(amax, std::max(std::fabs(lo[a]), std::fabs(hi[a])));
            P.grid_abs_margin = 1e-4f * diag + 1e-5f * amax;
            g.enabled = 1; sc.grid = g;
        }
    }
}

void prepare_shading(const lrt_scene_desc &d, const PrepOptions &opt, PreparedScene &P) {
    DScene &sc = P.sc; const std::vector<DSphere> &spheres = P.spheres;
    {
        P.vattr.assign(8 * (size_t) d.n_vertices, 0.f); std::vector<float> &va = P.vattr;
        for (size_t v = 0; v < d.n_vertices; ++v) {
            if (d.normals) for (int a = 0; a < 3; ++a) va[8 * v + a] = d.normals[3 * v + a];
            if (d.texcoords) for (int a = 0; a < 2; ++a) va[8 * v + 4 + a] = d.texcoords[2 * v + a];
        }
    }
    std::vector<DShape> &shapes = P.shapes; shapes.resize(d.n_shapes);
    for (uint32_t i = 0; i < d.n_shapes; ++i) { const lrt_shape_desc &s = d.shapes[i]; shapes[i] = { s.bsdf, s.emitter, s.interior_medium, s.exterior_medium, s.has_normals, s.has_texcoords, s.flip_normals, s.kind }; }
    std::vector<DTexture> &tex = P.textures; tex.resize(d.n_textures); std::vector<float> &tex_data = P.tex_data;
    for (uint32_t i = 0; i < d.n_textures; ++i) {
        const lrt_texture_desc &T = d.textures[i]; DTexture &o = tex[i]; memset(&o, 0, sizeof(o));
        o.type = T.type; o.width = T.width; o.height = T.height; o.channels = T.channels;
        for (int k = 0; k < 3; ++k) { o.color0[k] = T.color0[k]; o.color1[k] = T.color1[k]; }
        for (int k = 0; k < 6; ++k) o.to_uv[k] = T.to_uv[k];
        if (T.type == LRT_TEX_BITMAP) {
            o.data_offset = (uint32_t) tex_data.size();
            size_t np = (size_t) T.width * T.height;
            for (size_t p = 0; p < np; ++p) {
                const float *px = T.data + p * T.channels;
                tex_data.push_back(T.channels == 1 ? px[0] : px[0] * 0.212671f + px[1] * 0.715160f + px[2] * 0.072169f);
            }
        }
    }
    std::vector<DBsdf> &bsdfs = P.bsdfs; bsdfs.resize(d.n_bsdfs); sc.has_null_bsdf = 0;
    auto leaf_flags = [](int type) { return (type == LRT_BSDF_DIFFUSE || type == LRT_BSDF_ROUGHDIELECTRIC) ? PREP_F_SMOOTH : type == LRT_BSDF_DIELECTRIC ? PREP_F_DELTA : PREP_F_NULL; };
    for (uint32_t i = 0; i < d.n_bsdfs; ++i) {
        const lrt_bsdf_desc &B = d.bsdfs[i];
        DBsdf &o = bsdfs[i]; memset(&o, 0, sizeof(o));
        o.type = B.type; o.reflectance = B.reflectance; o.nested = B.nested; o.texture = B.texture; o.eta = B.eta; o.scale = B.scale;
        if (B.type == LRT_BSDF_BUMPMAP) {
            if (B.nested < 0 || (uint32_t) B.nested >= d.n_bsdfs || d.bsdfs[B.nested].type == LRT_BSDF_BUMPMAP) throw std::runtime_error("bumpmap: invalid nested BSDF");
            bsdfs[i].flags = leaf_flags(d.bsdfs[B.nested].type);
        } else bsdfs[i].flags = leaf_flags(B.type);
        if (B.type == LRT_BSDF_DIFFUSE && (B.reflectance < 0 || (uint32_t) B.reflectance >= d.n_textures || d.textures[B.reflectance].type == LRT_TEX_BITMAP))
            throw std::runtime_error("unsupported: a bitmap texture as diffuse reflectance (bitmaps are supported as bump-map heights only)");
        if (B.type == LRT_BSDF_NULL) sc.has_null_bsdf = 1;
        if (B.type == LRT_BSDF_ROUGHDIELECTRIC) {
            for (int32_t t : { B.specular_reflectance, B.specular_transmittance }) {
                if (t < -1 || t >= (int32_t) d.n_textures) throw std::runtime_error("roughdielectric references an invalid texture");
                if (t >= 0 && d.textures[t].type == LRT_TEX_BITMAP)
                    throw std::runtime_error("unsupported: a bitmap texture as roughdielectric specular_reflectance / specular_transmittance");
            }
            bsdfs[i].specular_reflectance = B.specular_reflectance; bsdfs[i].specular_transmittance = B.specular_transmittance;
            bsdfs[i].alpha_u = std::max(B.alpha_u, 1e-4f); bsdfs[i].alpha_v = std::max(B.alpha_v, 1e-4f);
            bsdfs[i].micro = (B.distribution == 1 ? LRT_MICRO_GGX : 0) | (B.sample_visible ? LRT_MICRO_VISIBLE : 0);
        }
    }
    DEnv &E = sc.env; memset(&E, 0, sizeof(E)); E.type = -1; E.emitter = -1;
    {
        float lo[3], hi[3]; vertex_bounds(d, spheres, lo, hi);
        const float ray_eps = 5.9604644775390625e-8f * 1500.f;
        if (d.n_vertices || !spheres.empty()) {
            float c[3], dd[3]; for (int a = 0; a < 3; ++a) { c[a] = (hi[a] + lo[a]) * 0.5f; dd[a] = c[a] - hi[a]; E.bsphere_c[a] = c[a]; }
            float r = sqrtf(fmaf(dd[2], dd[2], fmaf(dd[1], dd[1], dd[0] * dd[0])));
            E.bsphere_r = fmaxf(ray_eps, r * (1.f + ray_eps));
        } else { E.bsphere_c[0] = E.bsphere_c[1] = E.bsphere_c[2] = 0.f; E.bsphere_r = ray_eps; }
    }
    if (d.n_media > 64) throw std::runtime_error("at most 64 media are supported");
    for (uint32_t i = 0; i < d.n_media; ++i) {
        const lrt_medium_desc &M = d.media[i];
        if (M.type == LRT_MEDIUM_HOMOGENEOUS || M.type == LRT_MEDIUM_HETEROGENEOUS) P.has_non_bio = true;
        if (M.type != LRT_MEDIUM_HETEROGENEOUS) continue;
        if (!M.grid_data || M.grid_res[0] < 1 || M.grid_res[1] < 1 || M.grid_res[2] < 1 || !(M.grid_max > 0.f)) throw std::runtime_error("heterogeneous medium without a valid grid");
        P.has_het = true;
    }
    for (uint32_t i = 0; i < d.n_shapes; ++i) for (int m : { d.shapes[i].interior_medium, d.shapes[i].exterior_medium })
        if (m >= 0 && d.media[m].type == LRT_MEDIUM_HETEROGENEOUS) P.prb_null = true;
    std::vector<DEmitter> &em = P.emitters; em.resize(d.n_emitters); std::vector<float> &env_rgbx = P.env_data, &hier = P.env_hier; bool &env_interior_positive = P.env_interior_positive;
    std::vector<DMeshEmitter> &mesh_em = P.mesh_emitters; mesh_em.resize(d.n_emitters); std::vector<float> &mesh_tab = P.mesh_emitter_tab;
    for (uint32_t i = 0; i < d.n_emitters; ++i) {
        const lrt_emitter_desc &S = d.emitters[i]; DEmitter &o = em[i]; memset(&o, 0, sizeof(o));
        o.type = S.type; o.shape = S.shape; o.scale = S.scale; for (int k = 0; k < 3; ++k) o.radiance[k] = S.radiance[k];
        if (S.type == LRT_EMITTER_AREA) {
            P.has_area_emitter = true;
            const lrt_shape_desc &sd = d.shapes[S.shape];
            if (sd.kind == LRT_SHAPE_SPHERE) throw std::runtime_error("unsupported: an area emitter on a sphere (area emitters are supported on rectangles and triangle meshes)");
            if (sd.kind == LRT_SHAPE_MESH) {
                MeshEmitterTable T; mesh_emitter_table(d.positions, d.faces, sd.first_face, sd.n_faces, "shapes[" + std::to_string(S.shape) + "]", T);
// ... 165 lines not shown
```

### liverrenderer_amd/csrc/scene_prep.h

```cpp
#pragma once
#include "device_types.h"
#include "bvh.h"
#include "host_scene.h"
#include <utility>

namespace lrt {

struct PrepOptions {
    int bvh_leaf = 0;
    bool no_lds_bvh = false;
    bool no_dist_grid = false;
    int dist_grid_res = 0;
    bool no_nee_reject = false;
    size_t lds_limit = 0;
    int n_cus = 256;
    static PrepOptions from_env();
};

enum { PREP_F_DELTA = 1, PREP_F_SMOOTH = 2, PREP_F_NULL = 4 };

struct PreparedScene {
    std::vector<DSphere> spheres;
    HostBVH bvh;
    std::vector<unsigned char> lds_blob; DLdsInfo lds{};
    std::vector<float> vattr;
    std::vector<DShape> shapes;
    std::vector<DTexture> textures; std::vector<float> tex_data;
    std::vector<DBsdf> bsdfs;
    std::vector<DEmitter> emitters;
    std::vector<DMeshEmitter> mesh_emitters; std::vector<float> mesh_emitter_tab;
    std::vector<float> env_data, env_hier;
    DScene sc{};
    float grid_abs_margin = 0.f;
    bool env_interior_positive = false;
    bool ext = false, has_area_emitter = false, has_het = false, has_non_bio = false, prb_null = false, use_lds = false;
    int bvh_leaf = 4;
};
void prepare_geometry(const lrt_scene_desc &d, const PrepOptions &opt, PreparedScene &P);
void prepare_shading(const lrt_scene_desc &d, const PrepOptions &opt, PreparedScene &P);
PreparedScene prepare_scene(const lrt_scene_desc &d, const PrepOptions &opt);

size_t lds_image_bytes(const HostBVH &b, uint32_t n_vertices);
bool lds_image_fits(const lrt_scene_desc &d, const HostBVH &b, const PrepOptions &opt);

inline float medium_sigma_t(const lrt_medium_desc &M, int k) { return M.sigma_t[k] * M.scale; }
void prepare_media(const lrt_scene_desc &d, float bsphere_r, std::vector<DMedium> &media, std::vector<DBioMedium> &bio, std::vector<DHetMedium> &het);

struct ResolvedOpts { int integrator, max_depth, rr_depth, hide_emitters; uint32_t spp, seed, tile_rank, tile_count; uint32_t spp_total = 0, n_passes = 1, pass = 0; };
ResolvedOpts resolve(const lrt_scene_desc &d, const lrt_render_opts *o);

struct TilePixels { std::vector<uint32_t> list, slot; };
TilePixels tile_pixel_list(const DFilm &film, uint32_t rank, uint32_t count);
std::vector<uint32_t> halo_pixel_list(const DFilm &film, uint32_t rank, uint32_t count, uint32_t halo);

bool closed_records(const lrt_scene_desc &d, int sensor_medium);

}
```

Before: 6136 Msamples/s.

## Add per-face cone free-distance table to prove medium segments surface-free

Precomputes on the host, per triangle and per side, a conservative free distance inside four cone angle bins around the normal, stored as fp16. After a surface interaction, the kernel looks up this distance for the outgoing direction and uses it as a head start for the distance-grid ball-covering proof, so more free-flight segments can skip BVH traversal. In the closed-record path, the precomputed free-flight stage at path start is dropped. The cost is an O(n_faces^2) host prepass, an extra 16-byte table load per surface hit, and correctness that depends on the geometric bound being conservative.

```diff
diff --git a/include/liverrt.h b/include/liverrt.h
--- a/include/liverrt.h
+++ b/include/liverrt.h
@@ -177,6 +177,7 @@
     uint64_t lds_resident;
     uint64_t record_bytes;
     uint64_t n_closed_guard;
+    uint64_t n_proven;
 } lrt_render_stats;
 
 typedef struct {
diff --git a/liverrenderer_amd/_lib.py b/liverrenderer_amd/_lib.py
--- a/liverrenderer_amd/_lib.py
+++ b/liverrenderer_amd/_lib.py
@@ -99,7 +99,7 @@
 class RenderStats(C.Structure):
     _fields_ = [("n_samples", C.c_uint64), ("n_iter", C.c_uint64), ("n_shadow", C.c_uint64), ("n_launches", C.c_uint64),
                 ("n_records", C.c_uint64), ("kernel_ms", C.c_double), ("total_ms", C.c_double), ("lds_resident", C.c_uint64),
-                ("record_bytes", C.c_uint64), ("n_closed_guard", C.c_uint64)]
+                ("record_bytes", C.c_uint64), ("n_closed_guard", C.c_uint64), ("n_proven", C.c_uint64)]
 
 
 class ParamGrads(C.Structure):
diff --git a/liverrenderer_amd/csrc/capi.cpp b/liverrenderer_amd/csrc/capi.cpp
--- a/liverrenderer_amd/csrc/capi.cpp
+++ b/liverrenderer_amd/csrc/capi.cpp
@@ -27,7 +27,7 @@
 extern "C" {
 
 const char *lrt_last_error(void) { return g_error.c_str(); }
-int lrt_version(void) { return 114; }
+int lrt_version(void) { return 115; }
 
 static std::vector<std::pair<std::string, std::string>> parse_defines(const char *const *defines, int n) {
     std::vector<std::pair<std::string, std::string>> r;
diff --git a/liverrenderer_amd/csrc/device.hip b/liverrenderer_amd/csrc/device.hip
--- a/liverrenderer_amd/csrc/device.hip
+++ b/liverrenderer_amd/csrc/device.hip
@@ -54,7 +54,7 @@
 static void add_stats(lrt_render_stats &total, const lrt_render_stats &s) {
     total.n_samples += s.n_samples; total.n_iter += s.n_iter; total.n_shadow += s.n_shadow; total.n_launches += s.n_launches;
     total.n_records += s.n_records; total.kernel_ms += s.kernel_ms; total.total_ms += s.total_ms;
-    total.record_bytes = s.record_bytes; total.n_closed_guard += s.n_closed_guard;
+    total.record_bytes = s.record_bytes; total.n_closed_guard += s.n_closed_guard; total.n_proven += s.n_proven;
 }
 
 #define LRT_LAUNCH_SLOTS 64
@@ -280,6 +280,7 @@
     sc.emitters = up(P.emitters);
     sc.mesh_emitters = up(P.mesh_emitters);
     sc.mesh_emitter_tab = up(P.mesh_emitter_tab);
+    sc.cone_tab = P.cone_tab.empty() ? nullptr : (const uint2 *) up(P.cone_tab);
     sc.env_data = (const float4 *) up(P.env_data);
     sc.env_hier = up(P.env_hier);
     HIP_CHECK(hipMalloc((void **) &D->d_sc, sizeof(DScene))); D->track(D->d_sc);
@@ -495,6 +496,7 @@
     log.n_records = D->h_counters->n_records;
     finish_stats(D, log, e_begin, e_end, n_lanes, stats);
     stats.n_closed_guard = D->h_counters->n_closed_guard;
+    stats.n_proven = D->h_counters->n_proven;
     if (stats.n_closed_guard)
         throw std::runtime_error("64-byte path records: " + std::to_string(stats.n_closed_guard) + " trips broke the premise of the layout (radiance before a path's last trip, "
                                  "or an emitter hit that needs its MIS weight); the scene test in closed_records() is wrong for this scene: LRT_NO_CLOSED_RECORDS=1 renders it with 80-byte records");
@@ -956,7 +958,7 @@
     develop_and_download(D0, films[0], film_raw, image, film_floats, image_floats, on_device);
     lrt_render_stats total{};
     for (auto &x : st) { total.n_samples += x.n_samples; total.n_iter += x.n_iter; total.n_shadow += x.n_shadow; total.n_launches += x.n_launches; total.n_records += x.n_records;
-                         total.kernel_ms = std::max(total.kernel_ms, x.kernel_ms); total.lds_resident = x.lds_resident; total.record_bytes = x.record_bytes; total.n_closed_guard += x.n_closed_guard; }
+                         total.kernel_ms = std::max(total.kernel_ms, x.kernel_ms); total.lds_resident = x.lds_resident; total.record_bytes = x.record_bytes; total.n_closed_guard += x.n_closed_guard; total.n_proven += x.n_proven; }
     total.total_ms = std::chrono::duration<double, std::milli>(std::chrono::steady_clock::now() - t0).count();
     stats = total;
 }
diff --git a/liverrenderer_amd/csrc/device_types.h b/liverrenderer_amd/csrc/device_types.h
--- a/liverrenderer_amd/csrc/device_types.h
+++ b/liverrenderer_amd/csrc/device_types.h
@@ -142,7 +142,15 @@
     uint32_t n_spheres, pad_sph;
     const DMeshEmitter *mesh_emitters;
     const float *mesh_emitter_tab;
-};
+    const uint2 *cone_tab;
+    int32_t cone_enabled, pad_cone;
+};
+
+#define LRT_CONE_BINS 4
+#define LRT_CONE_COS0 0.95f
+#define LRT_CONE_COS1 0.85f
+#define LRT_CONE_COS2 0.70f
+#define LRT_CONE_COS3 0.50f
 
 #define LRT_CONST __attribute__((address_space(4)))
 typedef const LRT_CONST DScene &SceneRef;
@@ -207,6 +215,7 @@
     unsigned long long prof_cycles[4], prof_tiles[4];
     unsigned long long prof_wg[6];
     unsigned long long n_closed_guard;
+    unsigned long long n_proven;
 };
 
 struct DLdsInfo {
diff --git a/liverrenderer_amd/csrc/dshade.h b/liverrenderer_amd/csrc/dshade.h
--- a/liverrenderer_amd/csrc/dshade.h
+++ b/liverrenderer_amd/csrc/dshade.h
@@ -220,7 +220,7 @@
 }
 
 template <int K>
-DEV bool segment_covered_by_balls(GridRef g, V3 o, V3 d, float maxt) {
+DEV bool segment_covered_by_balls(GridRef g, V3 o, V3 d, float maxt, float start = 0.f) {
     if (!g.enabled || !(maxt < 1e30f)) return false;
     const float len = __builtin_amdgcn_sqrtf(dot(d, d));
     const float L = maxt * len * 1.01f;
@@ -228,7 +228,7 @@
     float lb[K];
 #pragma unroll
     for (int k = 0; k < K; ++k) lb[k] = dist_grid_lower_bound(g, fma3(d, maxt * LRT_FRAC(k), o)) * .995f;
-    float covered = 0.f; bool ok = true;
+    float covered = start; bool ok = true;
 #pragma unroll
     for (int k = 0; k < K; ++k) {
         const float c = L * LRT_FRAC(k);
@@ -245,6 +245,21 @@
 #else
     return segment_covered_by_balls<2>(g, o, d, maxt);
 #endif
+}
+DEV bool segment_free_of_surfaces_from(GridRef g, V3 o, V3 d, float maxt, float cone) {
+    if (cone < 0.f || !g.enabled || !(maxt < 1e30f)) return false;
+    if (cone > 0.f && cone >= maxt * __builtin_amdgcn_sqrtf(dot(d, d)) * 1.01f) return true;
+    return segment_covered_by_balls<2>(g, o, d, maxt, cone);
+}
+DEV float cone_free_length(uint4 rows, V3 d, V3 n) {
+    const float cs = dot(d, n), c = __builtin_fabsf(cs) * __builtin_amdgcn_rsqf(dot(d, d));
+    const uint32_t lo = cs < 0.f ? rows.z : rows.x, hi = cs < 0.f ? rows.w : rows.y;
+    const uint32_t w = c >= LRT_CONE_COS1 ? lo : hi;
+    uint32_t h = (c >= LRT_CONE_COS0 || (c < LRT_CONE_COS1 && c >= LRT_CONE_COS2)) ? (w & 0xffffu) : (w >> 16);
+    if (!(c >= LRT_CONE_COS3)) h = 0u;
+    union { uint16_t u; _Float16 f; } cv; cv.u = (uint16_t) h;
+    const float r = (float) cv.f;
+    return r > 0.f ? r * 1.01f : -1.f;
 }
 
 DEV SI compute_si(SceneRef sc, const Ray &r, const Hit &h, const LdsScene *L = nullptr) {
diff --git a/liverrenderer_amd/csrc/kernels.h b/liverrenderer_amd/csrc/kernels.h
--- a/liverrenderer_amd/csrc/kernels.h
+++ b/liverrenderer_amd/csrc/kernels.h
@@ -230,15 +230,19 @@
     };
     uint32_t nohit = 0;
     float cache_t = u2f(0x7fc00000u);
+    float cone_free = 0.f;
     auto free_flight_stage = [&]() {
         if (medium < 0) return;
         const DMedium M = tab(sc.media, medium);
         cache_t = medium_sampled_t(M, rng.next(), channel);
-        if (sc.grid.enabled) { const MI m2 = medium_interaction_at(M, ray, cache_t); if (m2.valid() && segment_free_of_surfaces(sc.grid, ray.o, ray.d, m2.t)) nohit = PF_NOHIT; }
+        if (sc.grid.enabled) {
+            const MI m2 = medium_interaction_at(M, ray, cache_t);
+            if (m2.valid() && (CLOSED ? segment_free_of_surfaces_from(sc.grid, ray.o, ray.d, m2.t, cone_free) : segment_free_of_surfaces(sc.grid, ray.o, ray.d, m2.t))) nohit = PF_NOHIT;
+        }
     };
     bool active = true;
     if (!PRE) active = termination_stage();
-    else if (fresh) { active = termination_stage(); if (active) { free_flight_stage(); ff_t = cache_t; proven_empty = nohit != 0; nohit = 0; cache_t = u2f(0x7fc00000u); } }
+    else if (fresh) { active = termination_stage(); if (active && !CLOSED) { free_flight_stage(); ff_t = cache_t; proven_empty = nohit != 0; nohit = 0; cache_t = u2f(0x7fc00000u); } }
     if (!active) { commit(); return false; }
 
     bool active_medium = medium >= 0, active_surface = !active_medium;
@@ -375,6 +379,8 @@
     active_surface = active_surface && si.valid;
     if (!active_surface) rng.skip(3);
     if (active_surface) {
+        uint4 cone_rows = make_uint4(0u, 0u, 0u, 0u);
+        if (CLOSED && sc.cone_enabled) cone_rows = *reinterpret_cast<const uint4 *>(sc.cone_tab + 2u * (size_t) si.prim);
         const DShape sd = tab(sc.shapes, si.shape, sc.one_shape);
         int b = sd.bsdf;
         int flags = tab(sc.bsdfs, b, sc.one_shape).flags;
@@ -399,6 +405,7 @@
         specular_chain = specular_chain || (non_null && (bs.type & F_DELTA));
         specular_chain = specular_chain && !(bs.type & F_SMOOTH);
         if (is_medium_transition(sd)) medium = target_medium(sd, ray.d, si.n);
+        if (CLOSED && sc.cone_enabled) cone_free = cone_free_length(cone_rows, ray.d, si.n);
     }
     active = active && (active_surface || active_medium);
     if (clk) clk->at(3);
@@ -597,6 +604,7 @@
     if (VP_LDS_COUNT && tid < 2) s_cnt[tid] = 0;
     WaveCount wc_shadow{ &s_cnt[0] }, wc_extra{ &s_cnt[1] };
     uint32_t n_shadow = 0, n_extra = 0, n_trips = 0, n_loaded = 0;
+    uint32_t n_proven = 0;
     if (rp.profile & 1u) t_loop_start = wall_clock64();
     for (;;) {
         if (tid == 0) {
@@ -643,6 +651,7 @@
                 const uint32_t n_had = (uint32_t) __popcll(__ballot(had_path));
                 n_trips += n_had;
                 if (t < ta + tcl + tb) n_loaded += n_had;
+                if (CLOSED && t < ta) n_proven += n_had;
             }
 #ifdef LRT_STAMP
             clk.at(0);
@@ -713,6 +722,7 @@
         if (!VP_LDS_COUNT && n_shadow) atomicAdd(&A.cnt->n_shadow, (unsigned long long) n_shadow);
         if (n_trips) atomicAdd(&A.cnt->n_iter, (unsigned long long) n_trips);
         if (n_loaded) atomicAdd(&A.cnt->n_records, (unsigned long long) n_loaded);
+        if (CLOSED && n_proven) atomicAdd(&A.cnt->n_proven, (unsigned long long) n_proven);
     }
     if (VP_LDS_COUNT) {
         __syncthreads();
diff --git a/liverrenderer_amd/csrc/scene_prep.cpp b/liverrenderer_amd/csrc/scene_prep.cpp
--- a/liverrenderer_amd/csrc/scene_prep.cpp
+++ b/liverrenderer_amd/csrc/scene_prep.cpp
@@ -15,6 +15,7 @@
     o.no_dist_grid = getenv("LRT_NO_DIST_GRID") != nullptr;
     if (getenv("LRT_DIST_GRID_RES")) o.dist_grid_res = std::max(8, std::min(256, atoi(getenv("LRT_DIST_GRID_RES"))));
     o.no_nee_reject = getenv("LRT_NO_NEE_REJECT") != nullptr;
+    o.no_cone_proof = getenv("LRT_NO_CONE_PROOF") != nullptr;
     return o;
 }
 
@@ -155,6 +156,167 @@
     for (const DSphere &o : spheres) for (int a = 0; a < 3; ++a) { lo[a] = fminf(lo[a], o.center[a] - o.radius); hi[a] = fmaxf(hi[a], o.center[a] + o.radius); }
 }
 
+namespace {
+struct D3 { double x, y, z; };
+inline D3 operator-(D3 a, D3 b) { return { a.x - b.x, a.y - b.y, a.z - b.z }; }
+inline D3 operator+(D3 a, D3 b) { return { a.x + b.x, a.y + b.y, a.z + b.z }; }
+inline D3 operator*(D3 a, double s) { return { a.x * s, a.y * s, a.z * s }; }
+inline double dot3(D3 a, D3 b) { return a.x * b.x + a.y * b.y + a.z * b.z; }
+inline D3 cross3(D3 a, D3 b) { return { a.y * b.z - a.z * b.y, a.z * b.x - a.x * b.z, a.x * b.y - a.y * b.x }; }
+inline double len3(D3 a) { return std::sqrt(dot3(a, a)); }
+struct ConePlane { D3 n; double c; };
+bool clip_min_height(const D3 *tri, const ConePlane *pl, D3 hn, double &hmin) {
+    D3 a[8], b[8]; int n = 3; for (int i = 0; i < 3; ++i) a[i] = tri[i];
+    for (int p = 0; p < 4 && n > 0; ++p) {
+        int m = 0;
+        for (int i = 0; i < n; ++i) {
+            const D3 u = a[i], v = a[(i + 1) % n];
+            const double su = dot3(pl[p].n, u) - pl[p].c, sv = dot3(pl[p].n, v) - pl[p].c;
+            if (su <= 0.0) b[m++] = u;
+            if ((su <= 0.0) != (sv <= 0.0)) { const double t = su / (su - sv); b[m++] = u + (v - u) * t; }
+        }
+        n = m; for (int i = 0; i < n; ++i) a[i] = b[i];
+    }
+    if (n == 0) return false;
+    hmin = INFINITY; for (int i = 0; i < n; ++i) hmin = std::min(hmin, dot3(hn, a[i]));
+    return true;
+}
+uint16_t half_round_down(double v) {
+    float f = (float) v; if ((double) f > v) f = std::nextafterf(f, 0.f);
+    if (!(f >= 6.103515625e-5f)) return 0;
+    if (f >= 65504.f) return 0x7bff;
+    uint32_t u; memcpy(&u, &f, 4);
+    return (uint16_t) ((((u >> 23) - 112u) << 10) | ((u >> 13) & 0x3ffu));
+}
+}
+float cone_table_value(uint16_t h) {
+    if (!h) return 0.f;
+    const uint32_t u = (((uint32_t) (h >> 10) + 112u) << 23) | ((uint32_t) (h & 0x3ffu) << 13); float f; memcpy(&f, &u, 4); return f;
+}
+
+void build_cone_table(const lrt_scene_desc &d, std::vector<uint16_t> &out) {
+    constexpr int K = LRT_CONE_BINS;
+    const uint32_t nf = d.n_faces;
+    out.assign((size_t) nf * 2 * K, 0);
+    if (!nf) return;
+    for (size_t i = 0; i < 3 * (size_t) d.n_vertices; ++i) if (!std::isfinite(d.positions[i])) return;
+    const double bin_cos[K] = { LRT_CONE_COS0, LRT_CONE_COS1, LRT_CONE_COS2, LRT_CONE_COS3 };
+    double tan_k[K], inv_cos_k[K];
+    for (int k = 0; k < K; ++k) { const double c = bin_cos[k] - 1e-3; tan_k[k] = std::sqrt(1.0 - c * c) / c; inv_cos_k[k] = 1.0 / c; }
+    std::vector<uint32_t> cid(d.n_vertices), order(d.n_vertices);
+    for (uint32_t i = 0; i < d.n_vertices; ++i) order[i] = i;
+    auto pos = [&](uint32_t v, int a) { return d.positions[3 * (size_t) v + a]; };
+    std::sort(order.begin(), order.end(), [&](uint32_t u, uint32_t v) { for (int a = 0; a < 3; ++a) if (pos(u, a) != pos(v, a)) return pos(u, a) < pos(v, a); return false; });
+    for (uint32_t i = 0, id = 0; i < d.n_vertices; ++i) {
+        if (i && (pos(order[i], 0) != pos(order[i - 1], 0) || pos(order[i], 1) != pos(order[i - 1], 1) || pos(order[i], 2) != pos(order[i - 1], 2))) ++id;
+        cid[order[i]] = id;
+    }
+    struct Face { D3 v[3], cen; double rad; uint32_t c[3]; bool dup; };
+    std::vector<Face> F(nf);
+    double lo[3] = { INFINITY, INFINITY, INFINITY }, hi[3] = { -INFINITY, -INFINITY, -INFINITY };
+    for (uint32_t f = 0; f < nf; ++f) {
+        Face &T = F[f];
+        for (int j = 0; j < 3; ++j) {
+            const uint32_t v = d.faces[3 * (size_t) f + j];
+            T.v[j] = { pos(v, 0), pos(v, 1), pos(v, 2) }; T.c[j] = cid[v];
+            const double q[3] = { T.v[j].x, T.v[j].y, T.v[j].z };
+            for (int a = 0; a < 3; ++a) { lo[a] = std::min(lo[a], q[a]); hi[a] = std::max(hi[a], q[a]); }
+        }
+        T.cen = (T.v[0] + T.v[1] + T.v[2]) * (1.0 / 3.0);
+        T.rad = std::max(len3(T.v[0] - T.cen), std::max(len3(T.v[1] - T.cen), len3(T.v[2] - T.cen))) * (1.0 + 1e-12);
+        T.dup = T.c[0] == T.c[1] || T.c[1] == T.c[2] || T.c[0] == T.c[2];
+    }
+    const double cap = 0.125 * std::max(hi[0] - lo[0], std::max(hi[1] - lo[1], hi[2] - lo[2]));
+    const double ray_eps = 1500.0 * 5.9604644775390625e-8;
+    for (uint32_t f = 0; f < nf; ++f) {
+        const Face &T = F[f];
+        if (T.dup) continue;
+        const D3 e1 = T.v[1] - T.v[0], e2 = T.v[2] - T.v[0], N = cross3(e1, e2);
+        const double n2 = len3(N);
+        if (!(n2 > 0.0) || n2 < 2e-3 * len3(e1) * len3(e2)) continue;
+        double amax = 0.0, m_min = 0.0;
+        for (int a = 0; a < 3; ++a) {
+            const double q[3] = { a == 0 ? T.v[0].x : (a == 1 ? T.v[0].y : T.v[0].z), a == 0 ? T.v[1].x : (a == 1 ? T.v[1].y : T.v[1].z), a == 0 ? T.v[2].x : (a == 1 ? T.v[2].y : T.v[2].z) };
+            amax = std::max(amax, std::max(std::fabs(q[0]), std::max(std::fabs(q[1]), std::fabs(q[2]))));
+            const bool one_sign = (q[0] > 0 && q[1] > 0 && q[2] > 0) || (q[0] < 0 && q[1] < 0 && q[2] < 0);
+            if (one_sign) m_min = std::max(m_min, std::min(std::fabs(q[0]), std::min(std::fabs(q[1]), std::fabs(q[2]))));
+        }
+        const double tau = 2e-6 * amax + 1e-9, mag_min = (1.0 + m_min) * ray_eps * (1.0 - 1e-5), mag_max = (1.0 + amax) * ray_eps * (1.0 + 1e-5);
+        const double h_o_max = mag_max + tau;
+        const uint32_t shape = d.face_shape ? d.face_shape[f] : 0u;
+        const bool flip = shape < d.n_shapes && d.shapes[shape].flip_normals;
+        D3 nu[2], ne[2][3]; double R[2][K];
+        for (int s = 0; s < 2; ++s) {
+            nu[s] = N * (((s == 0) != flip ? 1.0 : -1.0) / n2);
+            for (int e = 0; e < 3; ++e) {
+                D3 m = cross3(T.v[(e + 1) % 3] - T.v[e], nu[s]); m = m * (1.0 / len3(m));
+                if (dot3(T.v[(e + 2) % 3] - T.v[e], m) > 0.0) m = m * -1.0;
+                ne[s][e] = m;
+            }
+            for (int k = 0; k < K; ++k) R[s][k] = tau < 0.25 * mag_min * tan_k[k] ? cap : 0.0;
+        }
+        bool dead = false;
+        for (int pass = 0; pass < 2 && !dead; ++pass) {
+        double base[2];
+        for (int s = 0; s < 2; ++s) { double r = 0.0; for (int k = 0; k < K; ++k) r = std::max(r, R[s][k]); base[s] = T.rad + (r + h_o_max + tau) * inv_cos_k[K - 1] + 4.0 * tau; }
+        for (uint32_t g = 0; g < nf; ++g) {
+            if (g == f) continue;
+            const Face &G = F[g];
+            const D3 dc = G.cen - T.cen; const double dist2 = dot3(dc, dc), near = 3.0 * T.rad + G.rad, far = std::max(base[0], base[1]) + G.rad;
+            if ((dist2 <= near * near) != (pass == 0) || dist2 > far * far) continue;
+            int match[3], ns = 0;
+            for (int j = 0; j < 3; ++j) { match[j] = -1; for (int i = 0; i < 3; ++i) if (G.c[j] == T.c[i]) match[j] = i; ns += match[j] >= 0; }
+            if (ns == 3 || (ns > 0 && G.dup)) { for (int s = 0; s < 2; ++s) for (int k = 0; k < K; ++k) R[s][k] = 0.0; dead = true; break; }
+            for (int s = 0; s < 2; ++s) {
+                const D3 hn = nu[s]; const double h_off = dot3(hn, T.v[0]);
+                if (ns == 2) {
+                    int jw = 0, seen = 0; for (int j = 0; j < 3; ++j) { if (match[j] < 0) jw = j; else seen |= 1 << match[j]; }
+                    const int opp = seen == 3 ? 2 : (seen == 6 ? 0 : 1), e = (opp + 1) % 3;
+                    const D3 w = G.v[jw]; const double hw = dot3(hn, w) - h_off, lat = dot3(w - T.v[e], ne[s][e]), slack = 1e-9 * (1.0 + len3(w - T.v[e]));
+                    for (int k = 0; k < K; ++k) if (hw >= -slack && lat - hw * tan_k[k] <= slack) R[s][k] = 0.0;
+                } else if (ns == 1) {
+                    int iv = 0, jv = 0; for (int j = 0; j < 3; ++j) if (match[j] >= 0) { iv = match[j]; jv = j; }
+                    const D3 v = T.v[iv], w1 = G.v[(jv + 1) % 3], w2 = G.v[(jv + 2) % 3];
+                    const int ea = iv, eb = (iv + 2) % 3;
+                    const double slack = 1e-9 * (1.0 + std::max(len3(w1 - v), len3(w2 - v)));
+                    const double h1 = dot3(hn, w1 - v), h2 = dot3(hn, w2 - v);
+                    for (int k = 0; k < K; ++k) {
+                        const double c1[3] = { -h1, dot3(w1 - v, ne[s][ea]) - h1 * tan_k[k], dot3(w1 - v, ne[s][eb]) - h1 * tan_k[k] };
+                        const double c2[3] = { -h2, dot3(w2 - v, ne[s][ea]) - h2 * tan_k[k], dot3(w2 - v, ne[s][eb]) - h2 * tan_k[k] };
+                        double t0 = 0.0, t1 = 1.0;
+                        for (int c = 0; c < 3; ++c) {
+                            const double u0 = c1[c] - slack, du = c2[c] - c1[c];
+                            if (du == 0.0) { if (u0 > 0.0) t1 = -1.0; }
+                            else if (du > 0.0) t1 = std::min(t1, -u0 / du);
+                            else t0 = std::max(t0, -u0 / du);
+                        }
+                        if (t0 <= t1) R[s][k] = 0.0;
+                    }
+                } else {
+                    if (dist2 > (base[s] + G.rad) * (base[s] + G.rad)) continue;
+                    const double hc = dot3(hn, G.cen) - h_off;
+                    if (hc + G.rad < -tau) continue;
+                    double lat[3]; for (int e = 0; e < 3; ++e) lat[e] = dot3(G.cen - T.v[e], ne[s][e]);
+                    for (int k = K - 1; k >= 0; --k) {
+                        if (!(R[s][k] > 0.0) || hc - G.rad - h_o_max - tau >= R[s][k]) continue;
+                        const double tp = tau * (1.0 + tan_k[k]);
+                        bool outside = false;
+                        for (int e = 0; e < 3; ++e) outside = outside || lat[e] - hc * tan_k[k] - G.rad * inv_cos_k[k] > tp;
+                        if (outside) break;
+                        ConePlane pl[4]; pl[0] = { hn * -1.0, tau - h_off };
+                        for (int e = 0; e < 3; ++e) { const D3 n = ne[s][e] - hn * tan_k[k]; pl[1 + e] = { n, tp + dot3(T.v[e], ne[s][e]) - h_off * tan_k[k] }; }
+                        double hmin;
+                        if (!clip_min_height(G.v, pl, hn, hmin)) break;
+                        R[s][k] = std::max(0.0, std::min(R[s][k], hmin - h_off - h_o_max - tau));
+                    }
+                }
+            }
+        }
+        }
+        for (int s = 0; s < 2; ++s) for (int k = 0; k < K; ++k) out[((size_t) 2 * f + s) * K + k] = half_round_down(R[s][k]);
+    }
+}
+
 void prepare_geometry(const lrt_scene_desc &d, const PrepOptions &opt, PreparedScene &P) {
     DScene &sc = P.sc;
     memset(&sc, 0, sizeof(sc));
@@ -223,6 +385,7 @@
             g.enabled = 1; sc.grid = g;
         }
     }
+    if (P.use_lds && !P.ext && sc.grid.enabled && !opt.no_cone_proof && closed_records(d, d.sensor.medium)) { build_cone_table(d, P.cone_tab); sc.cone_enabled = 1; }
 }
 
 void prepare_shading(const lrt_scene_desc &d, const PrepOptions &opt, PreparedScene &P) {
diff --git a/liverrenderer_amd/csrc/scene_prep.h b/liverrenderer_amd/csrc/scene_prep.h
--- a/liverrenderer_amd/csrc/scene_prep.h
+++ b/liverrenderer_amd/csrc/scene_prep.h
@@ -12,6 +12,7 @@
     bool no_dist_grid = false;
     int dist_grid_res = 0;
     bool no_nee_reject = false;
+    bool no_cone_proof = false;
     size_t lds_limit = 0;
     int n_cus = 256;
     static PrepOptions from_env();
@@ -32,6 +33,7 @@
     std::vector<float> env_data, env_hier;
     DScene sc{};
     float grid_abs_margin = 0.f;
+    std::vector<uint16_t> cone_tab;
     bool env_interior_positive = false;
     bool ext = false, has_area_emitter = false, has_het = false, has_non_bio = false, prb_null = false, use_lds = false;
     int bvh_leaf = 4;
@@ -39,6 +41,9 @@
 void prepare_geometry(const lrt_scene_desc &d, const PrepOptions &opt, PreparedScene &P);
 void prepare_shading(const lrt_scene_desc &d, const PrepOptions &opt, PreparedScene &P);
 PreparedScene prepare_scene(const lrt_scene_desc &d, const PrepOptions &opt);
+
+void build_cone_table(const lrt_scene_desc &d, std::vector<uint16_t> &out);
+float cone_table_value(uint16_t h);
 
 size_t lds_image_bytes(const HostBVH &b, uint32_t n_vertices);
 bool lds_image_fits(const lrt_scene_desc &d, const HostBVH &b, const PrepOptions &opt);
```

Result: faster. 6552 Msamples/s (median of 6 runs) (+6.8%).
